# IRMVLab/EfficientLO-Net

Hardware: AMD Instinct MI355X
Metric: frame-pairs/sec (KITTI 64x1800 range image) (higher is better)
Workload: dtype f32 (1x1 convolutions as 3 fp16-MFMA products of hi/lo-split fp32 operands, fp32 accumulate)

## Files before the change

### efficientlo-net_amd/_lib.py

```python
import ctypes
import os

import torch

_PKG = os.path.dirname(os.path.abspath(__file__))
LIB_PATH = os.environ.get("ELO_LIB_PATH") or os.path.join(
    _PKG, "libelo_hip_f32.so" if os.environ.get("ELO_DENSE_F32", "0") == "1" else "libelo_hip.so")

_vp = ctypes.c_void_p


class GroupArgs(ctypes.Structure):
    _fields_ = [("batch", ctypes.c_int), ("H", ctypes.c_int), ("W", ctypes.c_int),
                ("H2", ctypes.c_int), ("W2", ctypes.c_int), ("npoints", ctypes.c_int),
                ("kernel_h", ctypes.c_int), ("kernel_w", ctypes.c_int), ("K", ctypes.c_int),
                ("flag_copy", ctypes.c_int), ("distance", ctypes.c_float),
                ("stride_h", ctypes.c_int), ("stride_w", ctypes.c_int),
                ("xyz1", _vp), ("xyz2", _vp), ("idx_n2", _vp), ("random_hw", _vp),
                ("selected_bhw_idx", _vp), ("valid_idx", _vp), ("valid_in_dis_idx", _vp),
                ("selected_mask", _vp)]


def _struct(name, fields):
    return type(name, (ctypes.Structure,), {"_fields_": fields, "__doc__": "struct %s (include/elo.h)." % name})


_i, _f = ctypes.c_int, ctypes.c_float
GroupConcatArgs = _struct("elo_group_concat_args", [
    ("batch", _i), ("npoints", _i), ("K", _i), ("H2", _i), ("W2", _i), ("C", _i),
    ("centre_xyz", _vp), ("src_xyz", _vp), ("src_feat", _vp), ("idx", _vp), ("mask", _vp), ("out", _vp)])
MaskedMaxpoolArgs = _struct("elo_masked_maxpool_args", [
    ("batch", _i), ("npoints", _i), ("K", _i), ("C", _i), ("x", _vp), ("mask", _vp), ("out", _vp)])
CvEncode1Args = _struct("elo_cv_encode1_args", [
    ("batch", _i), ("npoints", _i), ("K", _i), ("H2", _i), ("W2", _i), ("C", _i),
    ("xyz1", _vp), ("feat1", _vp), ("xyz2", _vp), ("feat2", _vp), ("idx", _vp), ("mask", _vp), ("out", _vp),
    ("dtype", _i)])
CvEncode2Args = _struct("elo_cv_encode2_args", [
    ("batch", _i), ("npoints", _i), ("K", _i), ("H", _i), ("W", _i), ("C", _i), ("Cc", _i),
    ("xyz1", _vp), ("feat1", _vp), ("cost", _vp), ("idx", _vp), ("mask", _vp), ("xyz_cat", _vp), ("rest", _vp),
    ("dtype", _i)])
SoftmaxPoolArgs = _struct("elo_softmax_pool_args", [
    ("batch", _i), ("npoints", _i), ("K", _i), ("C", _i), ("logits", _vp), ("values", _vp),
    ("values_stride", _i), ("mask", _vp), ("out", _vp), ("dtype", _i)])
ELO_F32, ELO_F16 = 0, 1
SoftmaxValidArgs = _struct("elo_softmax_valid_args", [
    ("batch", _i), ("npoints", _i), ("C", _i), ("feature", _vp), ("weight", _vp), ("xyz", _vp), ("out", _vp),
    ("scratch", _vp), ("stats", _vp)])
SV_MAX_PARTS = 512
PermRefreshArgs = _struct("elo_perm_refresh_args", [
    ("pool", _vp), ("versions", _i), ("total", _i), ("cursor", _vp), ("flat", _vp), ("decoded", _vp), ("entry_of", _vp),
    ("table", _vp), ("n_entries", _i)])
PoseHeadArgs = _struct("elo_pose_head_args", [
    ("batch", _i), ("npoints", _i), ("C", _i), ("hidden", _i), ("feature", _vp), ("weight", _vp), ("xyz", _vp),
    ("W_big", _vp), ("b_big", _vp), ("W_q", _vp), ("b_q", _vp), ("W_t", _vp), ("b_t", _vp),
    ("q_coarse", _vp), ("t_coarse", _vp), ("q", _vp), ("t", _vp), ("q_norm", _vp), ("scratch", _vp), ("pose7", _vp),
    ("clear_scratch", _vp), ("clear_xyz", _vp), ("clear_feat", _vp), ("clear_cells", ctypes.c_long), ("clear_C", _i),
    ("feat_dtype", _i), ("pose7_slots", _i), ("pose7_cursor", _vp), ("next_orders", PermRefreshArgs), ("ready_parts", _i)])
WarpProjectArgs = _struct("elo_warp_project_args", [
    ("batch", _i), ("npoints", _i), ("C", _i), ("H", _i), ("W", _i),
    ("az_res", _f), ("vert_res", _f), ("vert_off", _f),
    ("xyz", _vp), ("feat", _vp), ("q", _vp), ("t", _vp), ("warped", _vp), ("out_xyz", _vp), ("out_feat", _vp),
    ("scratch", _vp), ("prepared", _i), ("feat_dtype", _i)])

InputStageArgs = _struct("elo_input_stage_args", [
    ("batch", _i), ("npoints", _i), ("point_stride", _i), ("H", _i), ("W", _i), ("az_res", _f), ("vert_res", _f),
    ("vert_off", _f), ("crop_xy", _f), ("cloud", _vp), ("T_trans", _vp), ("aug_frame", _vp), ("points", _vp),
    ("out_xyz", _vp), ("scratch", _vp)])

GroupConcatBwdArgs = _struct("elo_group_concat_bwd_args", [
    ("batch", _i), ("npoints", _i), ("K", _i), ("H2", _i), ("W2", _i), ("C", _i),
    ("grad_out", _vp), ("idx", _vp), ("mask", _vp), ("grad_centre", _vp), ("grad_src_xyz", _vp), ("grad_src_feat", _vp)])
MaskedMaxpoolBwdArgs = _struct("elo_masked_maxpool_bwd_args", [
    ("batch", _i), ("npoints", _i), ("K", _i), ("C", _i), ("x", _vp), ("mask", _vp), ("grad_out", _vp), ("grad_x", _vp)])
CvEncode1BwdArgs = _struct("elo_cv_encode1_bwd_args", [
    ("batch", _i), ("npoints", _i), ("K", _i), ("H2", _i), ("W2", _i), ("C", _i),
    ("xyz1", _vp), ("xyz2", _vp), ("idx", _vp), ("mask", _vp), ("grad_out", _vp),
    ("grad_xyz1", _vp), ("grad_feat1", _vp), ("grad_xyz2", _vp), ("grad_feat2", _vp)])
CvEncode2BwdArgs = _struct("elo_cv_encode2_bwd_args", [
    ("batch", _i), ("npoints", _i), ("K", _i), ("H", _i), ("W", _i), ("C", _i), ("Cc", _i),
    ("xyz1", _vp), ("idx", _vp), ("mask", _vp), ("grad_xyz_cat", _vp), ("grad_rest", _vp),
    ("grad_xyz1", _vp), ("grad_feat1", _vp), ("grad_cost", _vp)])
SoftmaxPoolBwdArgs = _struct("elo_softmax_pool_bwd_args", [
    ("batch", _i), ("npoints", _i), ("K", _i), ("C", _i), ("logits", _vp), ("values", _vp), ("values_stride", _i),
    ("mask", _vp), ("grad_out", _vp), ("grad_logits", _vp), ("grad_values", _vp)])
SoftmaxValidBwdArgs = _struct("elo_softmax_valid_bwd_args", [
    ("batch", _i), ("npoints", _i), ("C", _i), ("feature", _vp), ("weight", _vp), ("xyz", _vp), ("grad_out", _vp),
    ("grad_feature", _vp), ("grad_weight", _vp), ("out", _vp), ("stats", _vp)])
WarpProjectBwdArgs = _struct("elo_warp_project_bwd_args", [
    ("batch", _i), ("npoints", _i), ("C", _i), ("H", _i), ("W", _i), ("az_res", _f), ("vert_res", _f), ("vert_off", _f),
    ("xyz", _vp), ("q", _vp), ("t", _vp), ("scratch", _vp), ("grad_out_xyz", _vp), ("grad_out_feat", _vp),
    ("grad_warped", _vp), ("grad_xyz", _vp), ("grad_feat", _vp), ("grad_q", _vp), ("grad_t", _vp)])

BnStatsArgs = _struct("elo_bn_stats_args", [
    ("rows", ctypes.c_long), ("C", _i), ("z", _vp), ("scratch", _vp), ("eps", _f), ("momentum", _f), ("mean", _vp), ("invstd", _vp),
    ("running_mean", _vp), ("running_var", _vp), ("groups", _i)])
BnApplyArgs = _struct("elo_bn_apply_args", [
    ("rows", ctypes.c_long), ("C", _i), ("z", _vp), ("mean", _vp), ("invstd", _vp), ("gamma", _vp), ("beta", _vp), ("relu", _i),
    ("y", _vp), ("groups", _i)])
BnBackwardArgs = _struct("elo_bn_backward_args", [
    ("rows", ctypes.c_long), ("C", _i), ("dy", _vp), ("z", _vp), ("mean", _vp), ("invstd", _vp), ("gamma", _vp), ("beta", _vp),
    ("relu", _i), ("scratch", _vp), ("sums", _vp), ("dz", _vp), ("groups", _i)])
AdamFlatArgs = _struct("elo_adam_flat_args", [
    ("n", ctypes.c_long), ("param", _vp), ("grad", _vp), ("exp_avg", _vp), ("exp_avg_sq", _vp), ("hyper", _vp),
    ("beta1", _f), ("beta2", _f), ("one_minus_beta1", _f), ("one_minus_beta2", _f)])
PoseComposeArgs = _struct("elo_pose_compose_args", [
    ("batch", _i), ("q_raw", _vp), ("t_det", _vp), ("q_coarse", _vp), ("t_coarse", _vp), ("q", _vp), ("t", _vp), ("q_norm", _vp),
    ("grad_q", _vp), ("grad_t", _vp), ("grad_q_norm", _vp), ("grad_q_raw", _vp), ("grad_t_det", _vp), ("grad_q_coarse", _vp),
    ("grad_t_coarse", _vp)])
PoseLossArgs = _struct("elo_pose_loss_args", [
    ("batch", _i), ("q", _vp * 4), ("t", _vp * 4), ("q_gt", _vp), ("t_gt", _vp), ("w_x", _vp), ("w_q", _vp), ("loss", _vp),
    ("grad_out", _vp), ("grad_q", _vp * 4), ("grad_t", _vp * 4), ("grad_w_x", _vp), ("grad_w_q", _vp)])
WeightGradArgs = _struct("elo_weight_grad_args", [
    ("rows", ctypes.c_long), ("Cin", _i), ("Cout", _i), ("x", _vp), ("g", _vp), ("dW", _vp), ("db", _vp), ("scratch", _vp)])
DenseRowsArgs = _struct("elo_dense_rows_args", [
    ("rows", ctypes.c_long), ("Cin", _i), ("Cout", _i), ("x", _vp), ("W", _vp), ("transposed", _i), ("bias", _vp), ("out", _vp),
    ("scratch", _vp), ("eps", _f), ("momentum", _f), ("mean", _vp), ("invstd", _vp), ("running_mean", _vp), ("running_var", _vp),
    ("bn_z", _vp), ("bn_mean", _vp), ("bn_invstd", _vp), ("bn_gamma", _vp), ("bn_beta", _vp), ("bn_sums", _vp), ("bn_relu", _i), ("bn_dz", _vp), ("groups", _i)])
Dense = _struct("elo_dense", [("w_packed", _vp), ("bias", _vp), ("K", _i), ("N", _i), ("relu", _i), ("w_plain", _vp),
                              ("products", _i)])
_l = ctypes.c_long
GroupSpec = _struct("elo_group_spec", [
    ("random_hw", _vp), ("kernel_h", _i), ("kernel_w", _i), ("distance", _f), ("stride_h", _i), ("stride_w", _i),
    ("idx_out", _vp), ("mask_out", _vp), ("decoded_hw", _vp)])
SetconvArgs = _struct("elo_setconv_args", [
    ("batch", _i), ("npoints", _i), ("K", _i), ("H", _i), ("W", _i), ("H2", _i), ("W2", _i), ("C", _i),
    ("xyz1_grid", _vp), ("centre_hw", _vp), ("centre_xyz", _vp), ("src_xyz", _vp), ("src_feat", _vp),
    ("idx", _vp), ("mask", _vp), ("n_layers", _i), ("layers", Dense * 3), ("out", _vp), ("new_xyz", _vp), ("group", GroupSpec),
    ("feat_dtype", _i), ("range_counter", _vp)])
MlpArgs = _struct("elo_mlp_args", [
    ("rows", _l), ("n_sources", _i), ("src", _vp * 3), ("src_width", _i * 3), ("n_layers", _i),
    ("layers", Dense * 3), ("out", _vp),
    ("n_layers2", _i), ("layers2", Dense * 3), ("before", _vp), ("w_before", _i), ("after", _vp), ("w_after", _i),
    ("out2", _vp), ("feat_dtype", _i),
    ("clear_scratch", _vp), ("clear_xyz", _vp), ("clear_feat", _vp), ("clear_cells", _l), ("clear_C", _i), ("clear_images", _i),
    ("batch_hint", _i), ("sv_scratch", _vp), ("sv_xyz", _vp), ("sv_feature", _vp), ("sv_npoints", _i),
    ("range_counter", _vp)])
Cv1Args = _struct("elo_cv1_args", [
    ("batch", _i), ("npoints", _i), ("K", _i), ("H2", _i), ("W2", _i), ("C", _i),
    ("xyz1", _vp), ("feat1", _vp), ("xyz2", _vp), ("feat2", _vp), ("idx", _vp), ("mask", _vp),
    ("cv0", Dense), ("cv1", Dense), ("cv2", Dense), ("cv_xyz", Dense), ("sum_cv0", Dense), ("sum_cv1", Dense),
    ("out", _vp), ("group", GroupSpec), ("feat_dtype", _i), ("range_counter", _vp)])
Cv2Args = _struct("elo_cv2_args", [
    ("batch", _i), ("npoints", _i), ("K", _i), ("H", _i), ("W", _i), ("C", _i),
    ("xyz1", _vp), ("feat1", _vp), ("cost", _vp), ("idx", _vp), ("mask", _vp),
    ("xyz_enc", Dense), ("sum_cost0", Dense), ("sum_cost1", Dense), ("out", _vp), ("group", GroupSpec), ("feat_dtype", _i),
    ("range_counter", _vp)])
Tuning = _struct("elo_tuning", [
    ("chain_forms", _i), ("narrow_mfma", _i), ("range_check", _i), ("select_dense_waves", _i), ("random_dense_rows", _i),
    ("setconv_chain_rows", _l), ("mlp_chain_rows", _l), ("small_tile_units", _l), ("pool_wave", _i)])

SYMBOLS = [
    ("elo_abi_version", ctypes.c_int, []),
    ("elo_dense_f32", ctypes.c_int, []),
    ("elo_last_error", ctypes.c_char_p, []),
    ("elo_range_check", ctypes.c_int, [ctypes.c_int]),
    ("elo_range_violations", ctypes.c_int, [ctypes.POINTER(ctypes.c_ulonglong), _vp]),
    ("elo_get_tuning", ctypes.c_int, [ctypes.POINTER(Tuning)]),
    ("elo_set_tuning", ctypes.c_int, [ctypes.POINTER(Tuning)]),
    ("elo_fused_conv_random_k", ctypes.c_int, [ctypes.POINTER(GroupArgs), _vp]),
    ("elo_fused_conv_select_k", ctypes.c_int, [ctypes.POINTER(GroupArgs), _vp]),
    ("elo_fused_conv_random_k_dense", ctypes.c_int, [ctypes.POINTER(GroupArgs), _vp]),
    ("elo_fused_conv_select_k_dense", ctypes.c_int, [ctypes.POINTER(GroupArgs), _vp]),
    ("elo_debug_select_dense_waves", ctypes.c_int, [ctypes.c_int]),
    ("elo_perm_refresh", ctypes.c_int, [ctypes.POINTER(PermRefreshArgs), _vp]),
    ("elo_group_concat", ctypes.c_int, [ctypes.POINTER(GroupConcatArgs), _vp]),
    ("elo_masked_maxpool", ctypes.c_int, [ctypes.POINTER(MaskedMaxpoolArgs), _vp]),
    ("elo_cv_encode1", ctypes.c_int, [ctypes.POINTER(CvEncode1Args), _vp]),
    ("elo_cv_encode2", ctypes.c_int, [ctypes.POINTER(CvEncode2Args), _vp]),
    ("elo_masked_softmax_pool", ctypes.c_int, [ctypes.POINTER(SoftmaxPoolArgs), _vp]),
    ("elo_softmax_valid", ctypes.c_int, [ctypes.POINTER(SoftmaxValidArgs), _vp]),
    ("elo_pose_head", ctypes.c_int, [ctypes.POINTER(PoseHeadArgs), _vp]),
    ("elo_warp_project", ctypes.c_int, [ctypes.POINTER(WarpProjectArgs), _vp]),
    ("elo_input_stage", ctypes.c_int, [ctypes.POINTER(InputStageArgs), _vp]),
    ("elo_pose_head_warp", ctypes.c_int, [ctypes.POINTER(PoseHeadArgs), ctypes.POINTER(WarpProjectArgs), _vp]),
    ("elo_group_concat_backward", ctypes.c_int, [ctypes.POINTER(GroupConcatBwdArgs), _vp]),
    ("elo_masked_maxpool_backward", ctypes.c_int, [ctypes.POINTER(MaskedMaxpoolBwdArgs), _vp]),
    ("elo_cv_encode1_backward", ctypes.c_int, [ctypes.POINTER(CvEncode1BwdArgs), _vp]),
    ("elo_cv_encode2_backward", ctypes.c_int, [ctypes.POINTER(CvEncode2BwdArgs), _vp]),
    ("elo_masked_softmax_pool_backward", ctypes.c_int, [ctypes.POINTER(SoftmaxPoolBwdArgs), _vp]),
    ("elo_softmax_valid_backward", ctypes.c_int, [ctypes.POINTER(SoftmaxValidBwdArgs), _vp]),
    ("elo_warp_project_backward", ctypes.c_int, [ctypes.POINTER(WarpProjectBwdArgs), _vp]),
    ("elo_bn_stats", ctypes.c_int, [ctypes.POINTER(BnStatsArgs), _vp]),
    ("elo_bn_apply", ctypes.c_int, [ctypes.POINTER(BnApplyArgs), _vp]),
    ("elo_bn_backward", ctypes.c_int, [ctypes.POINTER(BnBackwardArgs), _vp]),
    ("elo_dense_weight_grad", ctypes.c_int, [ctypes.POINTER(WeightGradArgs), _vp]),
    ("elo_dense_rows", ctypes.c_int, [ctypes.POINTER(DenseRowsArgs), _vp]),
    ("elo_dense_rows_supported", ctypes.c_int, [ctypes.c_long, ctypes.c_int, ctypes.c_int]),
    ("elo_dense_rows_scratch_floats", ctypes.c_long, [ctypes.c_int, ctypes.c_int]),
    ("elo_bn_scratch_floats", ctypes.c_long, [ctypes.c_int, ctypes.c_int]),
    ("elo_adam_flat", ctypes.c_int, [ctypes.POINTER(AdamFlatArgs), _vp]),
    ("elo_pose_compose", ctypes.c_int, [ctypes.POINTER(PoseComposeArgs), _vp]),
    ("elo_pose_loss", ctypes.c_int, [ctypes.POINTER(PoseLossArgs), _vp]),
    ("elo_weight_grad_slices", ctypes.c_int, [ctypes.c_long, ctypes.c_int, ctypes.c_int]),
    ("elo_setconv_fused", ctypes.c_int, [ctypes.POINTER(SetconvArgs), _vp]),
    ("elo_mlp_fused", ctypes.c_int, [ctypes.POINTER(MlpArgs), _vp]),
    ("elo_setconv_fused2", ctypes.c_int, [ctypes.POINTER(SetconvArgs), ctypes.POINTER(SetconvArgs), _vp]),
    ("elo_mlp_fused2", ctypes.c_int, [ctypes.POINTER(MlpArgs), ctypes.POINTER(MlpArgs), _vp]),
    ("elo_mlp_sv_parts", ctypes.c_int, [ctypes.POINTER(MlpArgs), ctypes.POINTER(MlpArgs)]),
    ("elo_cv_stage1_fused", ctypes.c_int, [ctypes.POINTER(Cv1Args), _vp]),
    ("elo_debug_cv1_rr", ctypes.c_int, [ctypes.c_int]),
    ("elo_debug_rr_rows", ctypes.c_int, [ctypes.c_long, ctypes.c_long]),
    ("elo_debug_rr_launches", ctypes.c_int, [ctypes.POINTER(ctypes.c_ulonglong), ctypes.c_int]),
    ("elo_debug_narrow_mfma", ctypes.c_int, [ctypes.c_int]),
    ("elo_debug_narrow_launches", ctypes.c_int, [ctypes.POINTER(ctypes.c_ulonglong), ctypes.c_int]),
    ("elo_debug_sv_ride_launches", ctypes.c_int, [ctypes.POINTER(ctypes.c_ulonglong), ctypes.c_int]),
    ("elo_get_tuning_base", ctypes.c_int, [ctypes.POINTER(Tuning)]),
    ("elo_graph_submit", ctypes.c_int, [_vp, _vp, _vp, _vp, ctypes.c_ulong, _vp, _vp, ctypes.c_int]),
    ("elo_debug_chain_pair_launches", ctypes.c_int, [ctypes.POINTER(ctypes.c_ulonglong), ctypes.c_int]),
    ("elo_cv_stage1_setconv_chain_form", ctypes.c_int, [ctypes.POINTER(Cv1Args), ctypes.POINTER(SetconvArgs), ctypes.POINTER(SetconvArgs)]),
    ("elo_cv_stage1_setconv_chain", ctypes.c_int, [ctypes.POINTER(Cv1Args), ctypes.POINTER(SetconvArgs), ctypes.POINTER(SetconvArgs), _vp]),
    ("elo_cv_stage2_fused", ctypes.c_int, [ctypes.POINTER(Cv2Args), _vp]),
    ("elo_cv_stage1_setconv_fused", ctypes.c_int, [ctypes.POINTER(Cv1Args), ctypes.POINTER(SetconvArgs), ctypes.POINTER(SetconvArgs), _vp]),
]

_lib = None


class EloError(RuntimeError):
    pass


ABI_VERSION = 26


def lib():
    global _lib
    if _lib is None:
        if not os.path.exists(LIB_PATH):
            raise EloError("libelo_hip.so is not built (%s); run `python -c 'import __graft_entry__ as g; "
                           "g.build()'` -- there is no CPU fallback for the hot path" % LIB_PATH)
        handle = ctypes.CDLL(LIB_PATH)
        for name, restype, argtypes in SYMBOLS:
            fn = getattr(handle, name)
            fn.restype = restype
            fn.argtypes = argtypes
        if handle.elo_abi_version() != ABI_VERSION:
            raise EloError("%s has ABI version %d, this host expects %d: rebuild (python -c 'import __graft_entry__ as g; "
                           "g.build()')" % (LIB_PATH, handle.elo_abi_version(), ABI_VERSION))
        _lib = handle
        from . import tuning
        env = tuning.lib_from_env()
        if env:
            set_tuning(**env)
    return _lib


def get_tuning():
    t = Tuning()
    check(lib().elo_get_tuning(ctypes.byref(t)))
    return {name: int(getattr(t, name)) for name, _ in Tuning._fields_}


def get_tuning_base():
    t = Tuning()
    check(lib().elo_get_tuning_base(ctypes.byref(t)))
    return {name: int(getattr(t, name)) for name, _ in Tuning._fields_}


def set_tuning(**fields):
    t = Tuning()
    check(lib().elo_get_tuning_base(ctypes.byref(t)))
    for name, value in fields.items():
        if not hasattr(t, name):
            raise KeyError("elo_tuning has no field %r" % name)
        setattr(t, name, int(value))
    check(lib().elo_set_tuning(ctypes.byref(t)))
    from . import tuning
    tuning.bump()


def check(rc):
    if rc != 0:
        raise EloError("libelo_hip: %s (status %d)" % (lib().elo_last_error().decode(), rc))


_range_counter = None


def set_range_counter(ptr):
    global _range_counter
    prev, _range_counter = _range_counter, ptr
    return prev


def _stamp(*structs):
    if _range_counter is not None:
        for a in structs:
            if a is not None and hasattr(a, "range_counter"):
                a.range_counter = _range_counter


def call(entry, args, like):
    _stamp(args)
    with torch.cuda.device(like.device):
        check(getattr(lib(), entry)(ctypes.byref(args), stream_ptr(like)))


def call3(entry, a, b, c, like):
    _stamp(a, b, c)
    with torch.cuda.device(like.device):
        check(getattr(lib(), entry)(ctypes.byref(a), ctypes.byref(b), ctypes.byref(c) if c is not None else None, stream_ptr(like)))


def call2(entry, args_a, args_b, like):
    _stamp(args_a, args_b)
    with torch.cuda.device(like.device):
        check(getattr(lib(), entry)(ctypes.byref(args_a), ctypes.byref(args_b), stream_ptr(like)))


def call2n(entry, args_a, args_b, like):
    _stamp(args_a, args_b)
    with torch.cuda.device(like.device):
        check(getattr(lib(), entry)(ctypes.byref(args_a), ctypes.byref(args_b) if args_b is not None else None, stream_ptr(like)))


def stream_ptr(t):
    return ctypes.c_void_p(torch.cuda.current_stream(t.device).cuda_stream)


def require_gpu(*tensors):
    for t in tensors:
        if t is not None and not t.is_cuda:
            raise EloError("the EfficientLO-Net hot path runs on an AMD GPU only (got a %s tensor); "
                           "there is no CPU fallback" % t.device)


def dtype_code(t):
    if t.dtype == torch.float32:
        return ELO_F32
    if t.dtype == torch.float16:
        return ELO_F16
    raise TypeError("feature tensors are float32 or float16 (got %s)" % t.dtype)


def range_check(enable):
    return lib().elo_range_check(1 if enable else 0)


def range_violations(like):
    n = ctypes.c_ulonglong(0)
    with torch.cuda.device(like.device):
        check(lib().elo_range_violations(ctypes.byref(n), stream_ptr(like)))
    return int(n.value)
```

### efficientlo-net_amd/csrc/elo_fused.hip

```cpp
#include "elo_group_device.h"
#include "elo_project_device.h"
#include <atomic>
#include <cstdlib>
#include <type_traits>

namespace elo {
namespace {

typedef float f32x4 __attribute__((ext_vector_type(4)));
typedef _Float16 half4 __attribute__((ext_vector_type(4)));
typedef _Float16 half2v __attribute__((ext_vector_type(2)));

constexpr int FUSED_BLOCK = 256;
constexpr int FUSED_WAVES = 4;
__device__ __forceinline__ int ftid() { return (int)(threadIdx.x & (FUSED_BLOCK - 1)); }

constexpr int MODE_SPLIT = 0;
constexpr int MODE_HALF = 1;
constexpr int MODE_CHECKED = 2;

__device__ unsigned long long g_range_violations;
__device__ unsigned long long g_range_snapshot;
__global__ void range_take_kernel() { g_range_snapshot = atomicExch(&g_range_violations, 0ull); }

// ... 1975 lines not shown
        }
    }
    stage_offsets(lds_off, a.group.random_hw, a.group.kernel_h, a.group.kernel_w, a.group.decoded_hw);
    RR_STAMP(1);
    {
        const float r2 = a.group.distance * a.group.distance;
        const int per_wave = 16 / K > 0 ? 16 / K : 1;
        auto uniform = [](float v) { return __int_as_float(__builtin_amdgcn_readfirstlane(__float_as_int(v))); };
        int pb[2], ph[2], pw[2];
        float pc[2][3];
        bool live[2];
        RawSlot first[2];
#pragma unroll
        for (int j = 0; j < 2; ++j) {
            const int pp = (wave * 16) / K + j;
            const long ptw = first_point + pp;
            live[j] = j < per_wave && pp < P && ptw < total_points;
            if (!live[j]) continue;
            pb[j] = (int)((unsigned)ptw / (unsigned)a.npoints);
            const int hwc = __builtin_amdgcn_readfirstlane(chw[pp]);
            ph[j] = div_stride(hwc >> 16, a.group.stride_h); pw[j] = div_stride(hwc & 0xffff, a.group.stride_w);
#pragma unroll
            for (int e = 0; e < 3; ++e) pc[j][e] = uniform(cxyz[pp * 3 + e]);
            first[j] = fetch_slot(grid_buffer(a.src_xyz + (size_t)pb[j] * a.H2 * a.W2 * 3), a.H2, a.W2, lds_off[lane < KT ? lane : 0], ph[j], pw[j],
                                  lane < KT);
        }
#pragma unroll
        for (int j = 0; j < 2; ++j) {
            if (!live[j]) continue;
            const int pp = (wave * 16) / K + j, b = pb[j];
            const float cx = pc[j][0], cy = pc[j][1], cz = pc[j][2];
            auto emit = [&](int slot, int hw) {
                cell_row[pp * K + slot] = (b * a.H2 + (hw >> 16)) * a.W2 + (hw & 0xffff);
                mask_row[pp * K + slot] = 1.0f;
            };
            int count = 0;
            if (!(pick_max(sq3(cx, cy, cz), ELO_EPS) <= ELO_EPS)) {
                const GridBuf gb = grid_buffer(a.src_xyz + (size_t)b * a.H2 * a.W2 * 3);
                count = wave_random_k_prefetched(gb, a.H2, a.W2, KT, K, lds_off, ph[j], pw[j], cx, cy, cz, r2, first[j], emit);
            }
            if (count + lane < K) { cell_row[pp * K + count + lane] = 0; mask_row[pp * K + count + lane] = 0.0f; }
        }
    }
    RR_STAMP(2);
    __syncthreads();
    RR_STAMP(3);
    const int r = wave * 16 + i16, pi = small_div(r, K);
    const int cell = cell_row[r];
    const bool used = cell >= 0;
    const float mk = mask_row[r];
    const float c0 = cxyz[(pi < P ? pi : 0) * 3 + 0], c1 = cxyz[(pi < P ? pi : 0) * 3 + 1], c2 = cxyz[(pi < P ? pi : 0) * 3 + 2];
    ActPair in0[FPB / 2];
    uint4 dxyz;
    const bool keep = used && mk != 0.0f;
    {
        typedef typename std::conditional<F16, uint2, float4>::type Item;
        Item f[FPB];
        const long cc = used ? cell : 0;
        const Item *rf = reinterpret_cast<const Item *>(a.src_feat) + (cc * C >> 2) + kq;
#pragma unroll
        for (int j = 0; j < FPB; ++j) f[j] = rf[j * 4];
        const float *g = a.src_xyz + cc * 3;
        const float x = g[0], y = g[1], z = g[2];
        ws.prime();
        auto quad = [&](const Item &v) {
            const uint4 zq{0u, 0u, 0u, 0u};
            if constexpr (F16) return keep ? quad_of_halves(v) : zq;
            else return keep ? pack_quad<MODE>(v, bad) : zq;
        };
#pragma unroll
        for (int j = 0; j < FPB; ++j) put_quad(in0[j / 2], j % 2, quad(f[j]));
        const float4 d = kq == 0 ? float4{x * mk - c0, y * mk - c1, z * mk - c2, 0.0f} : float4{0.0f, 0.0f, 0.0f, 0.0f};
        dxyz = used ? pack_quad<MODE>(d, bad) : uint4{0u, 0u, 0u, 0u};
    }
    rr_bias_store(lds, tid, N1 + N2 + N3, bias_word);
    RR_STAMP(4);
    rr_barrier();
    RR_STAMP(5);
    const uint4 none{0u, 0u, 0u, 0u};
    ActPair h1[N1 / 32];
    auto emit0 = [&](int pass, int t, const f32x4 acc) { put_quad(h1[pass], t, pack_quad<MODE>(relu4(acc, a.layers[0].relu), bad)); };
    rr_layer<FPB / 2, true, N1 / 16, 0, MODE, (F16 ? ~0u : 0u)>(in0, dxyz, bt, bt + B1, bias, fetch, advance, emit0);
    RR_STAMP(6);
    float4 last[NOUT / 16];
    if constexpr (N3 == 0) {
        rr_layer<N1 / 32, false, N2 / 16, E0, MODE>(h1, none, bt + B1, nullptr, bias, fetch, advance, [&](int pass, int t, const f32x4 acc) {
            last[2 * pass + t] = relu4(acc, a.layers[1].relu);
        });
    } else {
        ActPair h2[N2 / 32];
        rr_layer<N1 / 32, false, N2 / 16, E0, MODE>(h1, none, bt + B1, bt + B2, bias, fetch, advance, [&](int pass, int t, const f32x4 acc) {
            put_quad(h2[pass], t, pack_quad<MODE>(relu4(acc, a.layers[1].relu), bad));
        });
        rr_layer<N2 / 32, false, NOUT / 16, E1, MODE>(h2, none, bt + B2, nullptr, bias, fetch, advance, [&](int pass, int t, const f32x4 acc) {
            last[2 * pass + t] = relu4(acc, a.layers[2].relu);
        });
    }
    RR_STAMP(7);
    if ((K == 8 || K == 16) && a.layers[N3 ? 2 : 1].relu) rr_pool_max_inwave<NOUT, F16>(last, mk, r, lane, K, first_point, total_points, a.out);
    else rr_pool_max<NOUT, F16>(lds, last, mk, r, wave, lane, K, P, first_point, total_points, a.out);
    RR_STAMP(8);
    report_violations<MODE>(bad, a.range_counter);
}

template <int FPB, int N1, int N2, int N3, bool F16, int MODE = MODE_SPLIT>
__global__ __launch_bounds__(RR_WAVES * 64, 4) void setconv_rr_kernel(const JobPair<elo_setconv_args> jobs)
{
    setconv_rr_body<FPB, N1, N2, N3, F16, MODE>(jobs.job[blockIdx.y], blockIdx.x, gridDim.x);
}

template <int C, bool F16, int MODE>
__global__ __launch_bounds__(RR_WAVES * 64, 4) void cv1_setconv_rr_kernel(const elo_cv1_args a, const JobPair<elo_setconv_args> jobs,
                                                                         const unsigned n_cv, const unsigned n_sc)
{
    if (blockIdx.x < n_cv) {
        cv1_rr_body<C, F16, MODE>(a, blockIdx.x, n_cv);
    } else {
        const unsigned r = blockIdx.x - n_cv, j = r >= n_sc ? 1u : 0u;
        setconv_rr_body<4, 128, 64, 0, F16, MODE>(jobs.job[j], j ? r - n_sc : r, n_sc);
    }
}
template <int CIN, int N1, int N2, int N3, int MODE>
__global__ __launch_bounds__(ELO_BLOCK, 2) void setconv_narrow_kernel(const elo_setconv_args a)
{
    constexpr int G = 32, PER_BLOCK = ELO_BLOCK / G, C = CIN - 3, CB3 = N3 / 16;
    static_assert((C == 16 || C == 3) && N1 <= 16 && N2 <= 16 && (N3 == 16 || N3 == 32), "the pyramid's two narrow set-conv layers");
    __shared__ int slot_hw[PER_BLOCK][G];
    const int tid = threadIdx.x;
    const int l64 = tid & 63, i16 = l64 & 15, kq = l64 >> 4;
    unsigned bad = 0, wbad = 0;
    auto wq = [&](const elo_dense &L, const int LK, const int LN, int k0, int n) {
        const int nc = n < LN ? n : LN - 1;
        float v[4];
#pragma unroll
        for (int e = 0; e < 4; ++e) {
            const int k = k0 + e < LK ? k0 + e : LK - 1;
            v[e] = L.w_plain[k * LN + nc];
        }
#pragma unroll
        for (int e = 0; e < 4; ++e) v[e] = (k0 + e < LK && n < LN) ? v[e] : 0.0f;
        return float4{v[0], v[1], v[2], v[3]};
    };
    auto bq = [&](const elo_dense &L, const int LN, int n0) {
        float v[4];
#pragma unroll
        for (int e = 0; e < 4; ++e) v[e] = L.bias[n0 + e < LN ? n0 + e : LN - 1];
#pragma unroll
        for (int e = 0; e < 4; ++e) v[e] = n0 + e < LN ? v[e] : 0.0f;
        return float4{v[0], v[1], v[2], v[3]};
    };
    const float4 w1a = wq(a.layers[0], CIN, N1, 4 * kq, i16), w1b = C == 16 ? wq(a.layers[0], CIN, N1, 16 + 4 * kq, i16) : float4{0.0f, 0.0f, 0.0f, 0.0f};
    const float4 w2f = wq(a.layers[1], N1, N2, 4 * kq, i16);
    float4 w3f[CB3];
#pragma unroll
    for (int cb = 0; cb < CB3; ++cb) w3f[cb] = wq(a.layers[2], N2, N3, 4 * kq, cb * 16 + i16);
    const float4 b1 = bq(a.layers[0], N1, 4 * kq), b2 = bq(a.layers[1], N2, 4 * kq);
    float4 b3[CB3];
#pragma unroll
    for (int cb = 0; cb < CB3; ++cb) b3[cb] = bq(a.layers[2], N3, cb * 16 + 4 * kq);

    const int g = tid / G, lane = tid % G, shift = (tid & 63) / G * G;
    const elo_group_spec &gs = a.group;
    const int KT = gs.kernel_h * gs.kernel_w, kW = gs.kernel_w, hh = gs.kernel_h / 2, hw2 = gs.kernel_w / 2;
    int off[SMALL_STEPS];
    const int *order = gs.decoded_hw ? gs.decoded_hw : gs.random_hw;
#pragma unroll
    for (int st = 0; st < SMALL_STEPS; ++st) off[st] = order[st * G + lane < KT ? st * G + lane : 0];
    const long total = (long)a.batch * a.npoints;
    const long first = (long)xcd_tile(blockIdx.x, gridDim.x) * PER_BLOCK;
    const long pt = first + g;
    const bool live = pt < total;
    const long ptc = live ? pt : total - 1;
    int b, n, hc, wc;
    split_point(ptc, a.npoints, b, n);
    if (a.centre_hw) {
        const int2 c2 = reinterpret_cast<const int2 *>(a.centre_hw)[ptc];
        hc = c2.x; wc = c2.y;
    } else { hc = n / a.W; wc = n - hc * a.W; }
    if (!gs.decoded_hw) {
#pragma unroll
        for (int st = 0; st < SMALL_STEPS; ++st) off[st] = ((off[st] / kW - hh) << 16) | ((off[st] % kW - hw2) & 0xffff);
    }
    const float *cp = a.xyz1_grid + (((long)b * a.H + hc) * a.W + wc) * 3;
    const float cx = cp[0], cy = cp[1], cz = cp[2];
    const float *grid2 = a.src_xyz + (size_t)b * a.H2 * a.W2 * 3;
    const int base_h = div_stride(hc, gs.stride_h), base_w = div_stride(wc, gs.stride_w);
    RawSlot raw[SMALL_STEPS];
#pragma unroll
    for (int st = 0; st < SMALL_STEPS; ++st) raw[st] = fetch_slot(grid2, a.H2, a.W2, off[st], base_h, base_w, st * G + lane < KT);
    if (live && lane < 3 && a.new_xyz) a.new_xyz[pt * 3 + lane] = lane == 0 ? cx : lane == 1 ? cy : cz;
    const float r2 = gs.distance * gs.distance;
    slot_hw[g][lane] = -1;
    int taken = 0;
    const bool centre_ok = !(pick_max(sq3(cx, cy, cz), ELO_EPS) <= ELO_EPS);
#pragma unroll
    for (int st = 0; st < SMALL_STEPS; ++st) {
        if (st > 0 && (st * G >= KT || __builtin_amdgcn_ballot_w64(taken < G) == 0)) break;
        const Probe pr = judge(raw[st], cx, cy, cz, r2);
        const bool hit = pr.hit && centre_ok && taken < G;
        const unsigned long long mh = group_ballot<G>(hit, shift);
        const int slot = taken + __popcll(mh & ((1ull << lane) - 1ull));
        if (hit && slot < G) slot_hw[g][slot] = pr.hw;
        taken += __popcll(mh);
    }
    __builtin_amdgcn_fence(__ATOMIC_ACQ_REL, "wavefront");
    __builtin_amdgcn_wave_barrier();
    if (gs.idx_out || gs.mask_out) {
        const int hw = slot_hw[g][lane];
        if (live && gs.idx_out) {
            int *o = gs.idx_out + (pt * G + lane) * 3;
            o[0] = hw >= 0 ? b : 0; o[1] = hw >= 0 ? hw >> 16 : 0; o[2] = hw >= 0 ? hw & 0xffff : 0;
        }
        if (live && gs.mask_out) gs.mask_out[pt * G + lane] = hw >= 0 ? 1.0f : 0.0f;
    }

    const int wv = tid >> 6, f16 = a.feat_dtype == ELO_F16;
    auto uni = [](float v, int src) { return __int_as_float(__builtin_amdgcn_readlane(__float_as_int(v), src)); };
    float mrow[4], sx[4][3];
    uint4 ff[4];
#pragma unroll
    for (int rb = 0; rb < 4; ++rb) {
        const int hw = slot_hw[wv * 2 + (rb >> 1)][(rb & 1) * 16 + i16];
        const int bb = __builtin_amdgcn_readlane(b, (rb >> 1) * 32);
        mrow[rb] = hw >= 0 ? 1.0f : 0.0f;
        const long cell = hw >= 0 ? ((long)bb * a.H2 + (hw >> 16)) * a.W2 + (hw & 0xffff) : 0;
        const float *sp = a.src_xyz + cell * 3;
        sx[rb][0] = sp[0]; sx[rb][1] = sp[1]; sx[rb][2] = sp[2];
        if constexpr (C == 16) {
            if (f16) {
                const uint2 h = reinterpret_cast<const uint2 *>(a.src_feat)[cell * 4 + kq];
                ff[rb] = uint4{h.x, h.y, 0u, 0u};
            } else ff[rb] = reinterpret_cast<const uint4 *>(a.src_feat)[cell * 4 + kq];
        } else {
            float v[3];
#pragma unroll
            for (int c = 0; c < 3; ++c) v[c] = feat_load(a.src_feat, cell * 3 + c, f16);
            ff[rb] = uint4{__float_as_uint(v[0]), __float_as_uint(v[1]), __float_as_uint(v[2]), 0u};
        }
    }
    const uint4 q1a = pack_quad<MODE_SPLIT>(w1a, wbad), q1b = pack_quad<MODE_SPLIT>(w1b, wbad), w2t = pack_quad<MODE_SPLIT>(w2f, wbad);
    const WPair w1p{uint4{q1a.x, q1a.y, q1b.x, q1b.y}, uint4{q1a.z, q1a.w, q1b.z, q1b.w}};
    uint4 w3t[CB3];
#pragma unroll
    for (int cb = 0; cb < CB3; ++cb) w3t[cb] = pack_quad<MODE_SPLIT>(w3f[cb], wbad);
    float4 best[CB3];
#pragma unroll
    for (int rb = 0; rb < 4; ++rb) {
        const float m = mrow[rb];
        const float ccx = uni(cx, (rb >> 1) * 32), ccy = uni(cy, (rb >> 1) * 32), ccz = uni(cz, (rb >> 1) * 32);
        const float dx = sx[rb][0] * m - ccx, dy = sx[rb][1] * m - ccy, dz = sx[rb][2] * m - ccz;
        f32x4 acc1[1][1] = {{f32x4{b1.x, b1.y, b1.z, b1.w}}};
        if constexpr (C == 16) {
            uint4 fq;
            const float4 fv = __builtin_bit_cast(float4, ff[rb]);
            if (f16) fq = m != 0.0f ? quad_of_halves(uint2{ff[rb].x, ff[rb].y}) : uint4{0u, 0u, 0u, 0u};
            else fq = pack_quad<MODE>(float4{fv.x * m, fv.y * m, fv.z * m, fv.w * m}, bad);
            const uint4 gq = pack_quad<MODE>(kq == 0 ? float4{dx, dy, dz, 0.0f} : float4{0.0f, 0.0f, 0.0f, 0.0f}, bad);
            const ActPair in[1] = {ActPair{uint4{fq.x, fq.y, gq.x, gq.y}, uint4{fq.z, fq.w, gq.z, gq.w}}};
            const WPair w[1] = {w1p};
            mma_pair<MODE, 1, 1, 1>(acc1, 0, in, w);
        } else {
            const float4 fv = __builtin_bit_cast(float4, ff[rb]);
            const float4 v = kq == 0 ? float4{fv.x * m, fv.y * m, fv.z * m, dx} : kq == 1 ? float4{dy, dz, 0.0f, 0.0f}
                                                                                            : float4{0.0f, 0.0f, 0.0f, 0.0f};
            const uint4 in[1] = {pack_quad<MODE>(v, bad)}, w[1] = {q1a};
            mma_tail<MODE, 1, 1, 1, false>(acc1, 0, in, w);
        }
        f32x4 acc2[1][1] = {{f32x4{b2.x, b2.y, b2.z, b2.w}}};
        {
            const uint4 in[1] = {pack_quad<MODE>(relu4(acc1[0][0], a.layers[0].relu), bad)}, w[1] = {w2t};
            mma_tail<MODE, 1, 1, 1, false>(acc2, 0, in, w);
        }
        const uint4 h2[1] = {pack_quad<MODE>(relu4(acc2[0][0], a.layers[1].relu), bad)};
#pragma unroll
        for (int cb = 0; cb < CB3; ++cb) {
            f32x4 acc3[1][1] = {{f32x4{b3[cb].x, b3[cb].y, b3[cb].z, b3[cb].w}}};
            const uint4 w[1] = {w3t[cb]};
            mma_tail<MODE, 1, 1, 1, false>(acc3, 0, h2, w);
            const float4 y = relu4(acc3[0][0], a.layers[2].relu);
            const float q[4] = {y.x * m, y.y * m, y.z * m, y.w * m};
            float o[4];
#pragma unroll
            for (int e = 0; e < 4; ++e) {
                int v = __float_as_int(q[e]);
                v = dpp_imax_all<0xb1>(v);
                v = dpp_imax_all<0x4e>(v);
                v = dpp_imax_all<0x141>(v);
                v = dpp_imax_all<0x140>(v);
                o[e] = __int_as_float(v);
            }
            if (rb & 1) {
                const long ptg = first + wv * 2 + (rb >> 1);
                const float4 r4{fmaxf(best[cb].x, o[0]), fmaxf(best[cb].y, o[1]), fmaxf(best[cb].z, o[2]), fmaxf(best[cb].w, o[3])};
                if (i16 == 0 && ptg < total) feat_store4(a.out, ptg * N3 + cb * 16 + 4 * kq, r4, f16);
            } else best[cb] = float4{o[0], o[1], o[2], o[3]};
        }
    }
    report_violations<MODE>(bad, a.range_counter);
}

#endif

template <int TILE, int MODE>
__global__ __launch_bounds__(FUSED_BLOCK, TILE == 32 ? ELO_TILE32_WAVES : ELO_TILE_WAVES) void cv2_kernel(const elo_cv2_args a, const int S)
{
    extern __shared__ __align__(16) float lds[];
    float *act = lds;
    const TileMeta meta = tile_meta(lds, TILE, S);
    const int tid = threadIdx.x;
    const int K = a.K, P = TILE / K, C = a.C, f16 = a.feat_dtype == ELO_F16;
    unsigned bad = 0;
    const long total_points = (long)a.batch * a.npoints;
    const long first_point = (long)xcd_tile(blockIdx.x, gridDim.x) * P;
    if (first_point >= total_points) return;
    if (a.group.random_hw) {
        int *lds_off = reinterpret_cast<int *>(meta.cxyz + 128);
        group_tile<TILE, false>(meta, lds_off, nullptr, a.group, first_point, total_points, a.npoints, P, K, a.xyz1, a.H,
                                a.W, nullptr, a.xyz1, a.H, a.W, nullptr);
    } else {
        load_meta<TILE>(meta, first_point, total_points, P, K, a.idx, a.mask, a.H, a.W);
        __syncthreads();
    }
    const int Cp = ceil16(C), XYZ = 192;
    {
        auto cell_of = [&](int row) { return (long)meta.cell[row]; };
        auto centre_of = [&](int row) { return meta.cell[row] >= 0 ? first_point + small_div(row, K) : -1L; };
        uint4 rc[SEG_ITEMS], rf[SEG_ITEMS];
        seg_load<TILE>(rc, a.cost, 64, f16, cell_of);
        seg_load<TILE>(rf, a.feat1, C, f16, centre_of);
        GeoRow gr;
        const bool grow = tid < TILE;
        const int gcell = grow ? meta.cell[tid] : -1;
        if (grow) gr = geo_load(a.xyz1 + (gcell >= 0 ? first_point + small_div(tid, K) : 0) * 3, a.xyz1 + (long)(gcell >= 0 ? gcell : 0) * 3);
        seg_store<TILE, MODE>(act, S, 0, 64, f16, rc, cell_of, [&](int row) { return meta.mask[row] != 0.0f; }, bad);
        seg_store<TILE, MODE>(act, S, 128, C, f16, rf, centre_of, [](int) { return true; }, bad);
        zero_cols<TILE, MODE>(act, S, 128 + C, 128 + Cp);
        if (grow) geo_store<MODE>(act, tid * S + XYZ, gr, meta.mask[tid], gcell >= 0, bad);
    }
    Pre<Sub<TILE, 128>::TPW> p128;
    Pre<Sub<TILE, 64>::TPW> p64;
    prefetch<TILE, Sub<TILE, 64>::TPW, MODE>(a.xyz_enc, p64);
    __syncthreads();
    dense_pf<TILE, 64, 128, MODE>(act, S, XYZ, to_tile(64), a.xyz_enc, p64, &a.sum_cost0, &p128, bad);
    dense_pf<TILE, 128, 64, MODE>(act, S, 0, to_tile(64), a.sum_cost0, p128, &a.sum_cost1, &p64, bad);
    dense_pf<TILE, 64, 0, MODE>(act, S, 64, to_pool(64), a.sum_cost1, p64, nullptr, nullptr, bad);
    pool_masked_softmax(act, S, 64, 0, meta, P, K, first_point, total_points, a.out, f16);
    report_violations<MODE>(bad, a.range_counter);
}

inline long small_tile_threshold() { return tuning().small_tile_units; }
inline bool small_tile(long units_at_32, int K) { return K <= 16 && units_at_32 < small_tile_threshold(); }

int check_dense(const elo_dense &L, int K, int N, const char *who, const char *name)
{
    if (!L.w_packed || !L.bias) return fail(ELO_ERR_ARG, "%s: layer %s has null weights", who, name);
    if (L.K != K || (N > 0 && L.N != N))
        return fail(ELO_ERR_ARG, "%s: layer %s is %dx%d, expected %dx%d", who, name, L.K, L.N, K, N);
    if (L.N <= 0 || L.N > 128) return fail(ELO_ERR_LIMIT, "%s: layer %s width %d outside 1..128", who, name, L.N);
    if (L.products != ELO_PRODUCTS_SPLIT && L.products != ELO_PRODUCTS_HALF)
        return fail(ELO_ERR_ARG, "%s: layer %s: products must be ELO_PRODUCTS_SPLIT or ELO_PRODUCTS_HALF", who, name);
#ifdef ELO_DENSE_F32
    if (L.products != ELO_PRODUCTS_SPLIT) return fail(ELO_ERR_ARG, "%s: this library was built with -DELO_DENSE_F32 (fp32 MFMA only)", who);
#endif
    return ELO_OK;
}

int check_dtype(int feat_dtype, const char *who)
{
    if (feat_dtype != ELO_F32 && feat_dtype != ELO_F16) return fail(ELO_ERR_ARG, "%s: feat_dtype must be ELO_F32 or ELO_F16", who);
    return ELO_OK;
}

int &range_check_flag() { return tuning().range_check; }

template <typename... Rest>
int products_mode(const char *who, int *mode, const elo_dense &first, const Rest &...rest)
{
    const int m = first.products;
    for (const elo_dense *L : {&rest...})
        if (L->products != m) return fail(ELO_ERR_ARG, "%s: the layers of one launch must share one products mode", who);
    *mode = m == ELO_PRODUCTS_HALF ? MODE_HALF : range_check_flag() ? MODE_CHECKED : MODE_SPLIT;
    return ELO_OK;
}

int products_mode(const char *who, int *mode, const elo_dense *layers, int n, const elo_dense *layers2 = nullptr, int n2 = 0)
{
    const int m = layers[0].products;
    for (int l = 0; l < n; ++l)
        if (layers[l].products != m) return fail(ELO_ERR_ARG, "%s: the layers of one launch must share one products mode", who);
    for (int l = 0; l < n2; ++l)
        if (layers2[l].products != m) return fail(ELO_ERR_ARG, "%s: the layers of one launch must share one products mode", who);
    *mode = m == ELO_PRODUCTS_HALF ? MODE_HALF : range_check_flag() ? MODE_CHECKED : MODE_SPLIT;
    return ELO_OK;
}

size_t tile_lds_bytes(int rows, int S, int KT = 0, bool select = false, int K = 0)
{
    return sizeof(float) * ((size_t)rows * S + 64 + 96 + 32 + ((KT + 3) & ~3) + (select ? (size_t)FUSED_WAVES * select_scratch_words(KT, K) : 0));
}

int check_group(const elo_group_spec &g, int H2, int W2, size_t lds_bytes, const char *who)
{
    if (!g.random_hw) return ELO_OK;
    if (g.kernel_h <= 0 || g.kernel_w <= 0 || !(g.distance > 0.0f) || g.stride_h <= 0 || g.stride_w <= 0)
        return fail(ELO_ERR_ARG, "%s: bad grouping attributes", who);
    if (g.kernel_w / 2 > W2)
        return fail(ELO_ERR_LIMIT, "%s: kernel_size_W/2 = %d exceeds the queried width %d (single wrap)", who, g.kernel_w / 2, W2);
    if (H2 >= 32768 || W2 >= 65536) return fail(ELO_ERR_LIMIT, "%s: queried grid larger than 32767 x 65535", who);
    if ((long)H2 * W2 * 12 >= 0x7fffffffL) return fail(ELO_ERR_LIMIT, "%s: queried grid beyond 2 GB per batch element (buffer addressing)", who);
    if (lds_bytes > 64 * 1024)
        return fail(ELO_ERR_LIMIT, "%s: window %dx%d needs %zu bytes of LDS for in-kernel grouping", who, g.kernel_h, g.kernel_w, lds_bytes);
    return ELO_OK;
}

#define ELO_REQUIRE(cond, who, what) \
    do { if (!(cond)) return fail(ELO_ERR_ARG, "%s: %s", who, what); } while (0)

}
}

using namespace elo;

static inline int pad16(int x) { return (x + 15) & ~15; }

#ifdef ELO_DENSE_F32
#define ELO_PICK(KERNEL, tile16, mode, CALL)                                                              \
    do {                                                                                                  \
        if ((mode) == MODE_CHECKED) { if (tile16) CALL((KERNEL<16, MODE_CHECKED>)); else CALL((KERNEL<32, MODE_CHECKED>)); } \
        else { if (tile16) CALL((KERNEL<16, MODE_SPLIT>)); else CALL((KERNEL<32, MODE_SPLIT>)); }         \
    } while (0)
#else
#define ELO_PICK(KERNEL, tile16, mode, CALL)                                                              \
    do {                                                                                                  \
        if ((mode) == MODE_HALF) { if (tile16) CALL((KERNEL<16, MODE_HALF>)); else CALL((KERNEL<32, MODE_HALF>)); } \
        else if ((mode) == MODE_CHECKED) { if (tile16) CALL((KERNEL<16, MODE_CHECKED>)); else CALL((KERNEL<32, MODE_CHECKED>)); } \
        else { if (tile16) CALL((KERNEL<16, MODE_SPLIT>)); else CALL((KERNEL<32, MODE_SPLIT>)); }         \
    } while (0)
#endif

#ifdef ELO_DENSE_F32
#define ELO_PICK_MODE(M_, CALL_T) do { if ((M_) == MODE_CHECKED) CALL_T(MODE_CHECKED); else CALL_T(MODE_SPLIT); } while (0)
#else
#define ELO_PICK_MODE(M_, CALL_T) do { if ((M_) == MODE_HALF) CALL_T(MODE_HALF); else if ((M_) == MODE_CHECKED) CALL_T(MODE_CHECKED); else CALL_T(MODE_SPLIT); } while (0)
#endif

static int chain_cols(const elo_dense *layers, int n_layers, int width)
{
    int cols = pad16(width);
    for (int l = 0; l < n_layers; ++l) cols = cols > pad16(layers[l].N) ? cols : pad16(layers[l].N);
    return cols;
}

static int check_setconv(const elo_setconv_args *a, const char *who)
{
    ELO_REQUIRE(a, who, "null argument block");
    ELO_REQUIRE(a->batch >= 0 && a->npoints > 0 && a->K > 0 && a->H2 > 0 && a->W2 > 0 && a->C >= 0, who, "bad sizes");
    if (a->K > 32) return fail(ELO_ERR_LIMIT, "%s: K = %d exceeds the 32-row tile", who, a->K);
    ELO_REQUIRE(a->n_layers >= 1 && a->n_layers <= ELO_MAX_CHAIN, who, "1..3 layers");
    ELO_REQUIRE(a->src_xyz && (a->src_feat || a->C == 0) && a->out, who, "null tensor pointer");
    ELO_REQUIRE(a->group.random_hw || (a->idx && a->mask), who, "neither idx/mask nor a grouping spec");
    ELO_REQUIRE((a->xyz1_grid && a->H > 0 && a->W > 0 && (a->centre_hw || a->group.random_hw)) || a->centre_xyz, who, "no centre source");
    ELO_REQUIRE(!a->group.random_hw || (a->xyz1_grid && a->H > 0 && a->W > 0), who, "in-kernel grouping needs xyz1_grid");
    if (a->group.random_hw && a->group.stride_h > 0 && a->group.stride_w > 0 &&
        ((a->H - 1) / a->group.stride_h >= a->H2 || (a->W - 1) / a->group.stride_w >= a->W2))
        return fail(ELO_ERR_ARG, "%s: the queried grid %dx%d is smaller than the centres' grid %dx%d over the strides %dx%d", who, a->H2, a->W2,
                    a->H, a->W, a->group.stride_h, a->group.stride_w);
    if (int rc = check_dtype(a->feat_dtype, who)) return rc;
    int width = 3 + a->C;
    for (int l = 0; l < a->n_layers; ++l) {
        if (int rc = check_dense(a->layers[l], width, 0, who, "mlp")) return rc;
        width = a->layers[l].N;
    }
    return ELO_OK;
}

struct TilePlan { int S; bool t16; long units; size_t lds; int mode; };

static bool same_shape(const elo_setconv_args *a, const elo_setconv_args *b)
{
    if (a->batch != b->batch || a->npoints != b->npoints || a->K != b->K || a->C != b->C || a->n_layers != b->n_layers ||
        a->H2 != b->H2 || a->W2 != b->W2 || a->group.kernel_h != b->group.kernel_h || a->group.kernel_w != b->group.kernel_w ||
        (a->group.random_hw == nullptr) != (b->group.random_hw == nullptr) || a->feat_dtype != b->feat_dtype)
        return false;
    for (int l = 0; l < a->n_layers; ++l)
        if (a->layers[l].K != b->layers[l].K || a->layers[l].N != b->layers[l].N) return false;
    return true;
}

static int plan_setconv(const elo_setconv_args *a, const elo_setconv_args *b, TilePlan *p, const char *who)
{
    const long points = (long)a->batch * a->npoints;
    if (points >= 0x7fffffffL) return fail(ELO_ERR_LIMIT, "%s: batch * npoints beyond 2^31", who);
    p->S = row_stride(chain_cols(a->layers, a->n_layers, 3 + a->C));
    const int P32 = 32 / a->K, P16 = a->K <= 16 ? 16 / a->K : 1;
    const long u32 = (points + P32 - 1) / P32, u16 = (points + P16 - 1) / P16;
    int mode_b = 0;
    if (int rc = products_mode(who, &p->mode, a->layers, a->n_layers)) return rc;
    if (b) {
        if (int rc = products_mode(who, &mode_b, b->layers, b->n_layers)) return rc;
        if (p->mode != mode_b) return fail(ELO_ERR_ARG, "%s: the two jobs of a paired launch must share one products mode", who);
    }
    p->t16 = small_tile(u32 * (b ? 2 : 1), a->K);
    p->units = p->t16 ? u16 : u32;
    const int KT = a->group.random_hw ? a->group.kernel_h * a->group.kernel_w : 0;
    p->lds = tile_lds_bytes(p->t16 ? 16 : 32, p->S, KT, false);
    return check_group(a->group, a->H2, a->W2, p->lds, who);
}

extern "C" int elo_dense_f32(void)
{
#ifdef ELO_DENSE_F32
    return 1;
#else
    return 0;
#endif
}

#ifdef ELO_CV1_CLOCK
extern "C" int elo_debug_cv1_clock(unsigned long long *out16)
{
    return hipMemcpyFromSymbol(out16, HIP_SYMBOL(g_cv1_clock), 24 * sizeof(unsigned long long)) == hipSuccess ? 0 : -3;
}
#endif

extern "C" int elo_range_check(int enable)
{
    const int prev = range_check_flag();
    if (enable >= 0) range_check_flag() = enable ? 1 : 0;
    return prev;
}

extern "C" int elo_range_violations(unsigned long long *count, elo_stream_t stream)
{
    const char *who = "elo_range_violations";
    ELO_REQUIRE(count, who, "null count");
    hipStream_t s = (hipStream_t)stream;
    hipLaunchKernelGGL(range_take_kernel, dim3(1), dim3(1), 0, s);
    if (hipMemcpyFromSymbolAsync(count, HIP_SYMBOL(g_range_snapshot), sizeof(*count), 0, hipMemcpyDeviceToHost, s) != hipSuccess ||
        hipStreamSynchronize(s) != hipSuccess)
        return fail(ELO_ERR_LAUNCH, "%s: %s", who, hipGetErrorString(hipGetLastError()));
    return ELO_OK;
}

extern "C" int elo_debug_cv1_rr(int on)
{
    const int prev = tuning().chain_forms;
    tuning().chain_forms = on >= 0 ? (on != 0) : tuning_base().chain_forms;
    return prev;
}
static bool cv1_rr_on() { return tuning().chain_forms != 0; }
extern "C" int elo_debug_rr_rows(long setconv_rows, long mlp_rows)
{
    tuning().setconv_chain_rows = setconv_rows >= 0 ? setconv_rows : tuning_base().setconv_chain_rows;
    tuning().mlp_chain_rows = mlp_rows >= 0 ? mlp_rows : tuning_base().mlp_chain_rows;
    return ELO_OK;
}
static long setconv_rr_rows(int batch)
{
    const long t = tuning().setconv_chain_rows;
    (void)batch;
    return t >= 0 ? t : 20000L;
}
static long mlp_rr_rows(int batch_hint)
{
    const long t = tuning().mlp_chain_rows;
    return t >= 0 ? t : batch_hint >= ELO_THROUGHPUT_BATCH ? 2048L : 8192L;
}
extern "C" int elo_debug_narrow_mfma(int on)
{
    const int prev = tuning().narrow_mfma;
    tuning().narrow_mfma = on >= 0 ? (on ? 1 : 0) : tuning_base().narrow_mfma;
    return prev;
}
static bool narrow_mfma_on() { return tuning().narrow_mfma != 0; }
static std::atomic<unsigned long long> g_rr_launches[4];
extern "C" int elo_debug_rr_launches(unsigned long long *counts4, int reset)
{
    for (int i = 0; i < 4; ++i) {
        if (counts4) counts4[i] = g_rr_launches[i].load();
        if (reset) g_rr_launches[i].store(0);
    }
    return ELO_OK;
}
static std::atomic<unsigned long long> g_chain_pair_launches;
extern "C" int elo_debug_chain_pair_launches(unsigned long long *count, int reset)
{
    if (count) *count = g_chain_pair_launches.load();
    if (reset) g_chain_pair_launches.store(0);
    return ELO_OK;
}
static std::atomic<unsigned long long> g_sv_ride_launches;
extern "C" int elo_debug_sv_ride_launches(unsigned long long *count, int reset)
{
    if (count) *count = g_sv_ride_launches.load();
    if (reset) g_sv_ride_launches.store(0);
    return ELO_OK;
}
static std::atomic<unsigned long long> g_narrow_launches[2];
extern "C" int elo_debug_narrow_launches(unsigned long long *counts2, int reset)
{
    for (int i = 0; i < 2; ++i) {
        if (counts2) counts2[i] = g_narrow_launches[i].load();
        if (reset) g_narrow_launches[i].store(0);
    }
    return ELO_OK;
}

static int setconv_chain_shape(const elo_setconv_args *a, const elo_setconv_args *b, int mode)
{
#ifdef ELO_DENSE_F32
    return 0;
#else
    const long points = (long)a->batch * a->npoints;
    const int nl = a->n_layers, n1 = a->layers[0].N, n2 = nl >= 2 ? a->layers[1].N : 0, n3 = nl == 3 ? a->layers[2].N : 0;
    const int shape = (nl == 2 && n1 == 128 && n2 == 64) ? 1 : (nl == 3 && n1 == 64 && n2 == 64 && n3 == 128) ? 2
                    : (nl == 3 && n1 == 128 && n2 == 64 && n3 == 64) ? 3 : 0;
    const int KT = a->group.kernel_h * a->group.kernel_w;
    const bool narrow = !b && a->K == 32 && nl == 3 && a->layers[0].w_plain && a->layers[1].w_plain && a->layers[2].w_plain;
    if (!shape || narrow || !a->group.random_hw || !(mode == MODE_SPLIT || mode == MODE_HALF) || !cv1_rr_on() || a->C != 64 ||
        !(a->K == 8 || a->K == 16 || a->K == 32) || KT > 512 || a->group.idx_out || a->group.mask_out ||
        points * a->K * (b ? 2 : 1) < setconv_rr_rows(a->batch))
        return 0;
    return shape;
#endif
}

static bool cv_chain(int C, int mode)
{
#ifdef ELO_DENSE_F32
    return false;
#else
    return (mode == MODE_SPLIT || mode == MODE_HALF) && cv1_rr_on() && (C == 16 || C == 32 || C == 64);
#endif
}

extern "C" int elo_setconv_fused2(const elo_setconv_args *a, const elo_setconv_args *b, elo_stream_t stream)
{
    const char *who = "elo_setconv_fused";
    if (int rc = check_setconv(a, who)) return rc;
    if (b) {
        if (int rc = check_setconv(b, who)) return rc;
        if (!same_shape(a, b)) return fail(ELO_ERR_ARG, "%s: the two jobs of a paired launch must have the same shape", who);
    }
    const long points = (long)a->batch * a->npoints;
    if (points >= 0x7fffffffL) return fail(ELO_ERR_LIMIT, "%s: batch * npoints beyond 2^31", who);
    if (points == 0) return ELO_OK;
    hipStream_t s = (hipStream_t)stream;
    if (!b && a->group.random_hw && a->K == 32 && a->n_layers == 3 && a->layers[0].w_plain && a->layers[1].w_plain &&
        a->layers[2].w_plain && a->layers[2].relu && a->group.kernel_h * a->group.kernel_w <= SMALL_STEPS * 32) {
        const int cin = 3 + a->C, n1 = a->layers[0].N, n2 = a->layers[1].N, n3 = a->layers[2].N;
        const unsigned grid = (unsigned)((points + 7) / 8);
        if (int rc = check_group(a->group, a->H2, a->W2, 0, who)) return rc;
#ifndef ELO_DENSE_F32
        if (narrow_mfma_on()) {
            const bool checked = range_check_flag();
            if (cin == 19 && n1 == 16 && n2 == 16 && n3 == 32) {
                if (checked) hipLaunchKernelGGL((setconv_narrow_kernel<19, 16, 16, 32, MODE_CHECKED>), dim3(grid), dim3(ELO_BLOCK), 0, s, *a);
                else hipLaunchKernelGGL((setconv_narrow_kernel<19, 16, 16, 32, MODE_SPLIT>), dim3(grid), dim3(ELO_BLOCK), 0, s, *a);
                ++g_narrow_launches[0];
                return check_launch(who);
            }
        }
#endif
        if (cin == 6 && n1 == 8 && n2 == 8 && n3 == 16) {
            hipLaunchKernelGGL((setconv_small_kernel<6, 8, 8, 16>), dim3(grid), dim3(ELO_BLOCK), 0, s, *a);
            ++g_narrow_launches[1];
            return check_launch(who);
        }
        if (cin == 19 && n1 == 16 && n2 == 16 && n3 == 32) {
            hipLaunchKernelGGL((setconv_small_kernel<19, 16, 16, 32>), dim3(grid), dim3(ELO_BLOCK), 0, s, *a);
            ++g_narrow_launches[1];
            return check_launch(who);
        }
    }
    TilePlan plan;
    if (int rc = plan_setconv(a, b, &plan, who)) return rc;
    JobPair<elo_setconv_args> pair;
    pair.job[0] = *a;
    pair.job[1] = b ? *b : *a;
#ifndef ELO_DENSE_F32
    if (const int shape = setconv_chain_shape(a, b, plan.mode)) {
        const int P = RR_ROWS / a->K;
        const dim3 rgrid((unsigned)((points + P - 1) / P), b ? 2u : 1u);
        const bool f16 = a->feat_dtype == ELO_F16;
#define RRS(N1_, N2_, N3_)                                                                                                              \
        do {                                                                                                                        \
            if (f16 && plan.mode == MODE_HALF) hipLaunchKernelGGL((setconv_rr_kernel<4, N1_, N2_, N3_, true, MODE_HALF>), rgrid, dim3(RR_WAVES * 64), RR_LDS_BYTES, s, pair);  \
            else if (f16) hipLaunchKernelGGL((setconv_rr_kernel<4, N1_, N2_, N3_, true, MODE_SPLIT>), rgrid, dim3(RR_WAVES * 64), RR_LDS_BYTES, s, pair);  \
            else if (plan.mode == MODE_HALF) hipLaunchKernelGGL((setconv_rr_kernel<4, N1_, N2_, N3_, false, MODE_HALF>), rgrid, dim3(RR_WAVES * 64), RR_LDS_BYTES, s, pair);     \
            else hipLaunchKernelGGL((setconv_rr_kernel<4, N1_, N2_, N3_, false, MODE_SPLIT>), rgrid, dim3(RR_WAVES * 64), RR_LDS_BYTES, s, pair);     \
        } while (0)
        if (shape == 1) RRS(128, 64, 0);
        else if (shape == 2) RRS(64, 64, 128);
        else RRS(128, 64, 64);
#undef RRS
        ++g_rr_launches[2];
        return check_launch(who);
    }
#endif
    const dim3 grid((unsigned)plan.units, b ? 2u : 1u);
    const size_t lds = plan.lds;
    const int S = plan.S;
#define CALL(k) hipLaunchKernelGGL(k, grid, dim3(FUSED_BLOCK), lds, s, pair, S)
    ELO_PICK(setconv_kernel, plan.t16, plan.mode, CALL);
#undef CALL
    return check_launch(who);
}

extern "C" int elo_setconv_fused(const elo_setconv_args *a, elo_stream_t stream)
{
    return elo_setconv_fused2(a, nullptr, stream);
}

static int check_mlp(const elo_mlp_args *a, const char *who, int *in_width)
{
    ELO_REQUIRE(a, who, "null argument block");
    ELO_REQUIRE(a->rows >= 0 && a->n_sources >= 1 && a->n_sources <= 3, who, "bad sizes");
    ELO_REQUIRE(a->n_layers >= 1 && a->n_layers <= ELO_MAX_CHAIN && a->out, who, "1..3 layers and an output");
    if (int rc = check_dtype(a->feat_dtype, who)) return rc;
    int width = 0;
    for (int s = 0; s < a->n_sources; ++s) {
        ELO_REQUIRE(a->src[s] && a->src_width[s] > 0, who, "null / empty source");
        width += a->src_width[s];
    }
    *in_width = width;
    for (int l = 0; l < a->n_layers; ++l) {
        if (int rc = check_dense(a->layers[l], width, 0, who, "mlp")) return rc;
        width = a->layers[l].N;
    }
    ELO_REQUIRE(!a->clear_scratch || (a->clear_xyz && a->clear_cells > 0 && a->clear_images > 0 && a->clear_C >= 0 &&
                                      (a->clear_feat || a->clear_C == 0) && (a->feat_dtype != ELO_F16 || a->clear_C % 2 == 0)),
                who, "incomplete clear_* side job");
    ELO_REQUIRE(!a->clear_scratch || a->clear_cells * (a->clear_C > 3 ? a->clear_C : 3) < (1l << 31), who, "clear_* side job: more than 2^31 words");
    ELO_REQUIRE(a->n_layers2 >= 0 && a->n_layers2 <= ELO_MAX_CHAIN, who, "0..3 second-stage layers");
    if (a->n_layers2 > 0) {
        ELO_REQUIRE(a->out2 && a->w_before >= 0 && a->w_after >= 0 && (a->before || a->w_before == 0) &&
                    (a->after || a->w_after == 0), who, "incomplete second stage");
        ELO_REQUIRE(width % 4 == 0, who, "a second stage needs a first-stage output width that is a multiple of 4");
        width += a->w_before + a->w_after;
        for (int l = 0; l < a->n_layers2; ++l) {
            if (int rc = check_dense(a->layers2[l], width, 0, who, "mlp stage 2")) return rc;
            width = a->layers2[l].N;
        }
    }
    return ELO_OK;
}

static int mlp_cols(const elo_mlp_args *a, int in_width)
{
    int cols = chain_cols(a->layers, a->n_layers, in_width);
    if (a->n_layers2 > 0) {
        const int n1 = a->layers[a->n_layers - 1].N, in2 = a->w_before + n1 + a->w_after;
        const int c2 = chain_cols(a->layers2, a->n_layers2, in2);
        cols = cols > c2 ? cols : c2;
    }
    return cols;
}

struct MlpPlan { int S, mode, C; bool t16, chain; int sv_tiles; };

static int plan_mlp(const elo_mlp_args *a, const elo_mlp_args *b, MlpPlan *p, const char *who)
{
    int in_width = 0, in_width_b = 0;
    if (int rc = check_mlp(a, who, &in_width)) return rc;
    if (b) {
        if (int rc = check_mlp(b, who, &in_width_b)) return rc;
        bool same = a->rows == b->rows && in_width == in_width_b && a->n_layers == b->n_layers &&
                    a->n_layers2 == b->n_layers2 && a->w_before == b->w_before && a->w_after == b->w_after &&
                    a->feat_dtype == b->feat_dtype;
        for (int l = 0; same && l < a->n_layers; ++l) same = a->layers[l].N == b->layers[l].N;
        for (int l = 0; same && l < a->n_layers2; ++l) same = a->layers2[l].N == b->layers2[l].N;
        if (!same) return fail(ELO_ERR_ARG, "%s: the two jobs of a paired launch must have the same shape", who);
    }
    if (b && b->clear_scratch) return fail(ELO_ERR_ARG, "%s: the clear_* side job belongs to the first job of a pair", who);
    if (b && (b->sv_scratch || b->sv_feature)) return fail(ELO_ERR_ARG, "%s: the sv_* fields belong to the first job of a pair", who);
    p->S = row_stride(mlp_cols(a, in_width));
    const long u32 = (a->rows + 31) / 32;
    p->mode = 0;
    int mode_b = 0;
    if (int rc = products_mode(who, &p->mode, a->layers, a->n_layers, a->layers2, a->n_layers2)) return rc;
    if (b) {
        if (int rc = products_mode(who, &mode_b, b->layers, b->n_layers, b->layers2, b->n_layers2)) return rc;
        if (p->mode != mode_b) return fail(ELO_ERR_ARG, "%s: the two jobs of a paired launch must share one products mode", who);
    }
    p->t16 = small_tile(u32 * (b ? 2 : 1), 1);
    p->chain = false;
    p->C = a->n_sources == 2 ? a->src_width[1] : 0;
#ifndef ELO_DENSE_F32
    {
        const long min_rows = mlp_rr_rows(a->batch_hint);
        const int C = p->C;
        const bool aligned = ((uintptr_t)a->src[0] | (uintptr_t)a->src[1] | (uintptr_t)a->before | (uintptr_t)a->after | (uintptr_t)a->out |
                              (uintptr_t)a->out2) % 16 == 0 &&
                             (!b || ((uintptr_t)b->src[0] | (uintptr_t)b->src[1] | (uintptr_t)b->before | (uintptr_t)b->after | (uintptr_t)b->out |
                                     (uintptr_t)b->out2) % 16 == 0);
        p->chain = (p->mode == MODE_SPLIT || p->mode == MODE_HALF) && cv1_rr_on() && a->n_sources == 2 && a->src_width[0] == 64 &&
                   (C == 16 || C == 32 || C == 64) && a->n_layers == 2 && a->layers[0].N == 128 && a->layers[1].N == 64 && a->n_layers2 == 2 &&
                   a->layers2[0].N == 128 && a->layers2[1].N == 64 && a->w_before == C && a->w_after == 64 && aligned &&
                   a->rows * (b ? 2 : 1) >= min_rows;
    }
#endif
    p->sv_tiles = 0;
    const int final_n = a->n_layers2 > 0 ? a->layers2[a->n_layers2 - 1].N : a->layers[a->n_layers - 1].N;
    if (!p->chain && final_n == 64 && a->sv_npoints > 0 && a->rows > 0 && a->rows % a->sv_npoints == 0) {
        const bool t16 = small_tile((a->rows / a->sv_npoints) * (((long)a->sv_npoints + 31) / 32), 1);
        const int tile = t16 ? 16 : 32, groups = b ? 2 : 1;
        const long tiles = ((long)a->sv_npoints + tile - 1) / tile;
        const size_t lds = sizeof(float) * ((size_t)groups * tile * p->S + (b ? 0 : (size_t)tile * 64));
        if (tiles <= ELO_SV_MAX_PARTS && lds <= 64 * 1024) {
            p->sv_tiles = (int)tiles;
            p->t16 = t16;
        }
    }
    return ELO_OK;
}

extern "C" int elo_mlp_sv_parts(const elo_mlp_args *a, const elo_mlp_args *b)
{
    MlpPlan p;
    if (plan_mlp(a, b, &p, "elo_mlp_sv_parts")) return 0;
    return p.sv_tiles;
}

extern "C" int elo_mlp_fused2(const elo_mlp_args *a, const elo_mlp_args *b, elo_stream_t stream)
{
    const char *who = "elo_mlp_fused";
    MlpPlan plan;
    if (int rc = plan_mlp(a, b, &plan, who)) return rc;
    if (a->rows == 0)
        return a->clear_scratch || a->sv_scratch ? fail(ELO_ERR_ARG, "%s: a clear_* / sv_* side job needs rows to ride on", who) : ELO_OK;
    const int S = plan.S, mode = plan.mode;
    const bool t16 = plan.t16;
    const long u32 = (a->rows + 31) / 32, u16 = (a->rows + 15) / 16;
    JobPair<elo_mlp_args> pair;
    pair.job[0] = *a;
    pair.job[1] = b ? *b : *a;
    if (a->sv_scratch) {
        if (!plan.sv_tiles)
            return fail(ELO_ERR_ARG, "%s: sv_scratch is set but this launch cannot compute softmax_valid's partial sums "
                                     "(elo_mlp_sv_parts returns 0: chain-kernel regime, final width != 64, rows %% sv_npoints != 0 or too many tiles)", who);
        if (!a->sv_xyz) return fail(ELO_ERR_ARG, "%s: sv_scratch without sv_xyz", who);
        if ((b != nullptr) == (a->sv_feature != nullptr))
            return fail(ELO_ERR_ARG, "%s: a paired launch takes its features from job b (sv_feature NULL), a single launch from sv_feature", who);
        if (!b && ((uintptr_t)a->sv_feature & 15)) return fail(ELO_ERR_ARG, "%s: unaligned sv_feature", who);
        const int tile = t16 ? 16 : 32, groups = b ? 2 : 1;
        const size_t lds = sizeof(float) * ((size_t)groups * tile * S + (b ? 0 : (size_t)tile * 64));
        const dim3 grid((unsigned)(a->rows / a->sv_npoints) * (unsigned)plan.sv_tiles);
        hipStream_t s = (hipStream_t)stream;
#define CALL_SV(T_, M_)                                                                                                         \
        do {                                                                                                                    \
            if (b) hipLaunchKernelGGL((mlp_sv_kernel<T_, M_, true>), grid, dim3(2 * FUSED_BLOCK), lds, s, pair, S, plan.sv_tiles); \
            else hipLaunchKernelGGL((mlp_sv_kernel<T_, M_, false>), grid, dim3(FUSED_BLOCK), lds, s, pair, S, plan.sv_tiles);     \
        } while (0)
#define CALL_SV_T(M_) do { if (t16) CALL_SV(16, M_); else CALL_SV(32, M_); } while (0)
        ELO_PICK_MODE(mode, CALL_SV_T);
#undef CALL_SV_T
#undef CALL_SV
        ++g_sv_ride_launches;
        return check_launch(who);
    }
    const size_t lds = tile_lds_bytes(t16 ? 16 : 32, S);
#ifndef ELO_DENSE_F32
    if (plan.chain) {
        const int C = plan.C;
        const dim3 rgrid((unsigned)((a->rows + RR_ROWS - 1) / RR_ROWS), b ? 2u : 1u);
        const bool f16 = a->feat_dtype == ELO_F16;
        hipStream_t rs = (hipStream_t)stream;
#define RRM(C_)                                                                                                                      \
        do {                                                                                                                    \
            if (f16 && mode == MODE_HALF) hipLaunchKernelGGL((mlp2_rr_kernel<C_, true, MODE_HALF>), rgrid, dim3(RR_WAVES * 64), RR_LDS_BYTES, rs, pair);             \
            else if (f16) hipLaunchKernelGGL((mlp2_rr_kernel<C_, true, MODE_SPLIT>), rgrid, dim3(RR_WAVES * 64), RR_LDS_BYTES, rs, pair);             \
            else if (mode == MODE_HALF) hipLaunchKernelGGL((mlp2_rr_kernel<C_, false, MODE_HALF>), rgrid, dim3(RR_WAVES * 64), RR_LDS_BYTES, rs, pair);                \
            else hipLaunchKernelGGL((mlp2_rr_kernel<C_, false, MODE_SPLIT>), rgrid, dim3(RR_WAVES * 64), RR_LDS_BYTES, rs, pair);                \
        } while (0)
        if (C == 16) RRM(16);
        else if (C == 32) RRM(32);
        else RRM(64);
#undef RRM
        ++g_rr_launches[3];
        return check_launch(who);
    }
#endif
    const dim3 grid((unsigned)(t16 ? u16 : u32), b ? 2u : 1u);
    hipStream_t s = (hipStream_t)stream;
#define CALL(k) hipLaunchKernelGGL(k, grid, dim3(FUSED_BLOCK), lds, s, pair, S)
    ELO_PICK(mlp_kernel, t16, mode, CALL);
#undef CALL
    return check_launch(who);
}

extern "C" int elo_mlp_fused(const elo_mlp_args *a, elo_stream_t stream) { return elo_mlp_fused2(a, nullptr, stream); }

static int check_cv_features(const char *who, int C, int f16, std::initializer_list<const void *> tensors)
{
    const int per = f16 ? 8 : 4;
    if (C % per != 0) return fail(ELO_ERR_LIMIT, "%s: C = %d must be a multiple of %d (%s feature storage)", who, C, per, f16 ? "fp16" : "fp32");
    if (32 * (C / per) > SEG_ITEMS * FUSED_BLOCK) return fail(ELO_ERR_LIMIT, "%s: C = %d too wide for the tile gather", who, C);
    for (const void *p : tensors)
        if ((uintptr_t)p & 15) return fail(ELO_ERR_ARG, "%s: feature tensors must be 16-byte aligned", who);
    return ELO_OK;
}

static int plan_cv1(const elo_cv1_args *a, TilePlan *p, const char *who)
{
    ELO_REQUIRE(a, who, "null argument block");
    ELO_REQUIRE(a->batch >= 0 && a->npoints > 0 && a->K > 0 && a->H2 > 0 && a->W2 > 0 && a->C > 0, who, "bad sizes");
    if (a->K > 32) return fail(ELO_ERR_LIMIT, "%s: K = %d exceeds the 32-row tile", who, a->K);
    ELO_REQUIRE(a->xyz1 && a->feat1 && a->xyz2 && a->feat2 && a->out, who, "null tensor pointer");
    ELO_REQUIRE(a->group.random_hw || (a->idx && a->mask), who, "neither idx/mask nor a grouping spec");
    ELO_REQUIRE(!a->group.random_hw || a->npoints == a->H2 * a->W2, who, "in-kernel grouping needs npoints == H2*W2");
    if (int rc = check_dtype(a->feat_dtype, who)) return rc;
    if (int rc = check_cv_features(who, a->C, a->feat_dtype == ELO_F16, {a->feat1, a->feat2})) return rc;
    const int CT = 10 + 2 * a->C;
    if (int rc = check_dense(a->cv0, CT, 128, who, "CV_0")) return rc;
    if (int rc = check_dense(a->cv1, 128, 64, who, "CV_1")) return rc;
    if (int rc = check_dense(a->cv2, 64, 64, who, "CV_2")) return rc;
    if (int rc = check_dense(a->cv_xyz, 10, 64, who, "CV_xyz")) return rc;
    if (int rc = check_dense(a->sum_cv0, 128, 128, who, "sum_CV_0")) return rc;
    if (int rc = check_dense(a->sum_cv1, 128, 64, who, "sum_CV_1")) return rc;
    const long points = (long)a->batch * a->npoints;
    if (points >= 0x7fffffffL) return fail(ELO_ERR_LIMIT, "%s: batch * npoints beyond 2^31", who);
    const int cols = 128 + cv1_feat_cols(a->C);
    p->S = row_stride(cols > 192 ? cols : 192);
    const int P32 = 32 / a->K, P16 = a->K <= 16 ? 16 / a->K : 1;
    const long u32 = (points + P32 - 1) / P32, u16 = (points + P16 - 1) / P16;
    if (int rc = products_mode(who, &p->mode, a->cv0, a->cv1, a->cv2, a->cv_xyz, a->sum_cv0, a->sum_cv1)) return rc;
    p->t16 = small_tile(u32, a->K);
    p->units = p->t16 ? u16 : u32;
    const int KT = a->group.random_hw ? a->group.kernel_h * a->group.kernel_w : 0;
    p->lds = tile_lds_bytes(p->t16 ? 16 : 32, p->S);
    if (sizeof(float) * (((size_t)KT + 3) / 4 * 4 + (size_t)FUSED_WAVES * select_scratch_words(KT, a->K)) > sizeof(float) * (p->t16 ? 16 : 32) * p->S)
        return fail(ELO_ERR_LIMIT, "%s: window %dx%d does not fit the tile for in-kernel grouping", who, a->group.kernel_h, a->group.kernel_w);
    return check_group(a->group, a->H2, a->W2, p->lds, who);
}

extern "C" int elo_cv_stage1_fused(const elo_cv1_args *a, elo_stream_t stream)
{
    const char *who = "elo_cv_stage1_fused";
    TilePlan plan;
    if (int rc = plan_cv1(a, &plan, who)) return rc;
    if ((long)a->batch * a->npoints == 0) return ELO_OK;
#ifndef ELO_DENSE_F32
    if (!a->group.random_hw && cv_chain(a->C, plan.mode)) {
        const int P = RR_ROWS / a->K;
        const dim3 grid((unsigned)(((long)a->batch * a->npoints + P - 1) / P));
        const size_t lds = RR_LDS_BYTES;
        hipStream_t s = (hipStream_t)stream;
        const bool f16 = a->feat_dtype == ELO_F16;
        static_assert(RR_LDS_BYTES <= 64 * 1024, "dynamic LDS within the default limit");
#define RR(CC)                                                                                                      \
        do {                                                                                                        \
            if (f16 && plan.mode == MODE_HALF) hipLaunchKernelGGL((cv1_rr_kernel<CC, true, MODE_HALF>), grid, dim3(RR_WAVES * 64), lds, s, *a);          \
            else if (f16) hipLaunchKernelGGL((cv1_rr_kernel<CC, true, MODE_SPLIT>), grid, dim3(RR_WAVES * 64), lds, s, *a);          \
            else if (plan.mode == MODE_HALF) hipLaunchKernelGGL((cv1_rr_kernel<CC, false, MODE_HALF>), grid, dim3(RR_WAVES * 64), lds, s, *a);             \
            else hipLaunchKernelGGL((cv1_rr_kernel<CC, false, MODE_SPLIT>), grid, dim3(RR_WAVES * 64), lds, s, *a);             \
        } while (0)
        if (a->C == 16) RR(16);
        else if (a->C == 32) RR(32);
        else RR(64);
#undef RR
        ++g_rr_launches[0];
        return check_launch(who);
    }
#endif
    const dim3 grid((unsigned)plan.units);
    const size_t lds = plan.lds;
    const int S = plan.S;
    hipStream_t s = (hipStream_t)stream;
#define CALL(k) hipLaunchKernelGGL(k, grid, dim3(FUSED_BLOCK), lds, s, *a, S)
    if (a->group.random_hw) ELO_PICK(cv1_kernel, plan.t16, plan.mode, CALL);
    else ELO_PICK(cv1_meta_kernel, plan.t16, plan.mode, CALL);
#undef CALL
    return check_launch(who);
}


extern "C" int elo_cv_stage1_setconv_fused(const elo_cv1_args *a, const elo_setconv_args *ja, const elo_setconv_args *jb,
                                           elo_stream_t stream)
{
    const char *who = "elo_cv_stage1_setconv_fused";
    TilePlan pc, ps;
    if (int rc = plan_cv1(a, &pc, who)) return rc;
    if (int rc = check_setconv(ja, who)) return rc;
    if (jb) {
        if (int rc = check_setconv(jb, who)) return rc;
        if (!same_shape(ja, jb)) return fail(ELO_ERR_ARG, "%s: the two set-conv jobs must have the same shape", who);
    }
    if (int rc = plan_setconv(ja, jb, &ps, who)) return rc;
    if (ps.mode != pc.mode) return fail(ELO_ERR_ARG, "%s: the cost volume and the set-conv jobs must share one products mode", who);
    if ((long)a->batch * a->npoints == 0 || (long)ja->batch * ja->npoints == 0)
        return fail(ELO_ERR_ARG, "%s: empty batch (call the separate entry points)", who);
    SideJobs side;
    side.job[0] = *ja;
    side.job[1] = jb ? *jb : *ja;
    side.njobs = jb ? 2 : 1;
    side.S = ps.S;
    side.blocks_per_job = (int)ps.units;
    const unsigned n_cv = (unsigned)pc.units;
    const dim3 grid(n_cv + (unsigned)(ps.units * side.njobs));
    const size_t lds = pc.lds > ps.lds ? pc.lds : ps.lds;
    const int S = pc.S;
    hipStream_t s = (hipStream_t)stream;
#define CALL_T(M) do {                                                                                                  \
        if (pc.t16 && ps.t16) hipLaunchKernelGGL((cv1_setconv_kernel<16, 16, M>), grid, dim3(FUSED_BLOCK), lds, s, *a, S, n_cv, side);      \
        else if (pc.t16) hipLaunchKernelGGL((cv1_setconv_kernel<16, 32, M>), grid, dim3(FUSED_BLOCK), lds, s, *a, S, n_cv, side);           \
        else if (ps.t16) hipLaunchKernelGGL((cv1_setconv_kernel<32, 16, M>), grid, dim3(FUSED_BLOCK), lds, s, *a, S, n_cv, side);           \
        else hipLaunchKernelGGL((cv1_setconv_kernel<32, 32, M>), grid, dim3(FUSED_BLOCK), lds, s, *a, S, n_cv, side);                        \
    } while (0)
    ELO_PICK_MODE(pc.mode, CALL_T);
#undef CALL_T
    return check_launch(who);
}

static int chain_pair_form(const elo_cv1_args *a, const elo_setconv_args *ja, const elo_setconv_args *jb, int *mode_out, const char *who)
{
#ifdef ELO_DENSE_F32
    (void)a; (void)ja; (void)jb; (void)mode_out; (void)who;
    return 0;
#else
    if (!a || !ja || !jb) return 0;
    int mode = 0, mode_sc = 0, mode_sb = 0;
    if (products_mode(who, &mode, a->cv0, a->cv1, a->cv2, a->cv_xyz, a->sum_cv0, a->sum_cv1)) return 0;
    if (ja->n_layers != 2 || jb->n_layers != 2 || products_mode(who, &mode_sc, ja->layers, 2) || products_mode(who, &mode_sb, jb->layers, 2)) return 0;
    if (mode != mode_sc || mode != mode_sb || !same_shape(ja, jb) || ja->feat_dtype != a->feat_dtype) return 0;
    if (!cv_chain(a->C, mode) || setconv_chain_shape(ja, jb, mode) != 1) return 0;
    if (a->K <= 0 || a->K > 32) return 0;
    *mode_out = mode;
    return 1;
#endif
}

extern "C" int elo_cv_stage1_setconv_chain_form(const elo_cv1_args *a, const elo_setconv_args *ja, const elo_setconv_args *jb)
{
    int mode = 0;
    return chain_pair_form(a, ja, jb, &mode, "elo_cv_stage1_setconv_chain_form");
}

extern "C" int elo_cv_stage1_setconv_chain(const elo_cv1_args *a, const elo_setconv_args *ja, const elo_setconv_args *jb,
                                           elo_stream_t stream)
{
    const char *who = "elo_cv_stage1_setconv_chain";
#ifdef ELO_DENSE_F32
    (void)a; (void)ja; (void)jb; (void)stream;
    return fail(ELO_ERR_LIMIT, "%s: the fp32-MFMA comparison build has no register-resident kernels", who);
#else
    TilePlan pc, ps;
    if (int rc = plan_cv1(a, &pc, who)) return rc;
    ELO_REQUIRE(jb, who, "two set-conv jobs");
    if (int rc = check_setconv(ja, who)) return rc;
    if (int rc = check_setconv(jb, who)) return rc;
    if (!same_shape(ja, jb)) return fail(ELO_ERR_ARG, "%s: the two set-conv jobs must have the same shape", who);
    if (int rc = plan_setconv(ja, jb, &ps, who)) return rc;
    if (a->group.random_hw || !a->idx || !a->mask) return fail(ELO_ERR_ARG, "%s: the cost volume comes pre-grouped (idx / mask of the select-k pre-pass)", who);
    int mode = 0;
    if (!chain_pair_form(a, ja, jb, &mode, who) || mode != pc.mode || mode != ps.mode)
        return fail(ELO_ERR_ARG, "%s: not a chain-form launch (elo_cv_stage1_setconv_chain_form returns 0)", who);
    const long pts_cv = (long)a->batch * a->npoints, pts_sc = (long)ja->batch * ja->npoints;
    if (pts_cv == 0 || pts_sc == 0) return fail(ELO_ERR_ARG, "%s: empty batch (call the separate entry points)", who);
    const int Pc = RR_ROWS / a->K, Ps = RR_ROWS / ja->K;
    const unsigned n_cv = (unsigned)((pts_cv + Pc - 1) / Pc), n_sc = (unsigned)((pts_sc + Ps - 1) / Ps);
    const dim3 grid(n_cv + 2u * n_sc);
    JobPair<elo_setconv_args> pair;
    pair.job[0] = *ja;
    pair.job[1] = *jb;
    hipStream_t s = (hipStream_t)stream;
    const bool f16 = a->feat_dtype == ELO_F16;
#define RRP(CC)                                                                                                                              \
    do {                                                                                                                                    \
        if (f16 && mode == MODE_HALF) hipLaunchKernelGGL((cv1_setconv_rr_kernel<CC, true, MODE_HALF>), grid, dim3(RR_WAVES * 64), RR_LDS_BYTES, s, *a, pair, n_cv, n_sc);   \
        else if (f16) hipLaunchKernelGGL((cv1_setconv_rr_kernel<CC, true, MODE_SPLIT>), grid, dim3(RR_WAVES * 64), RR_LDS_BYTES, s, *a, pair, n_cv, n_sc);                 \
        else if (mode == MODE_HALF) hipLaunchKernelGGL((cv1_setconv_rr_kernel<CC, false, MODE_HALF>), grid, dim3(RR_WAVES * 64), RR_LDS_BYTES, s, *a, pair, n_cv, n_sc);   \
        else hipLaunchKernelGGL((cv1_setconv_rr_kernel<CC, false, MODE_SPLIT>), grid, dim3(RR_WAVES * 64), RR_LDS_BYTES, s, *a, pair, n_cv, n_sc);                          \
    } while (0)
    if (a->C == 16) RRP(16);
    else if (a->C == 32) RRP(32);
    else RRP(64);
#undef RRP
    ++g_rr_launches[0];
    ++g_rr_launches[2];
    ++g_chain_pair_launches;
    return check_launch(who);
#endif
}

extern "C" int elo_cv_stage2_fused(const elo_cv2_args *a, elo_stream_t stream)
{
    const char *who = "elo_cv_stage2_fused";
    ELO_REQUIRE(a, who, "null argument block");
    ELO_REQUIRE(a->batch >= 0 && a->npoints > 0 && a->K > 0 && a->H > 0 && a->W > 0 && a->C > 0, who, "bad sizes");
    ELO_REQUIRE(a->npoints == a->H * a->W, who, "npoints must equal H*W (every pixel is a centre)");
    if (a->K > 32) return fail(ELO_ERR_LIMIT, "%s: K = %d exceeds the 32-row tile", who, a->K);
    if (a->C > 64) return fail(ELO_ERR_LIMIT, "%s: C = %d exceeds 64", who, a->C);
    ELO_REQUIRE(a->xyz1 && a->feat1 && a->cost && a->out, who, "null tensor pointer");
    ELO_REQUIRE(a->group.random_hw || (a->idx && a->mask), who, "neither idx/mask nor a grouping spec");
    if (int rc = check_dtype(a->feat_dtype, who)) return rc;
    if (int rc = check_cv_features(who, a->C, a->feat_dtype == ELO_F16, {a->feat1, a->cost})) return rc;
    if (int rc = check_dense(a->xyz_enc, 10, 64, who, "sum_xyz_encoding")) return rc;
    if (int rc = check_dense(a->sum_cost0, 128 + a->C, 128, who, "sum_cost_volume_0")) return rc;
    if (int rc = check_dense(a->sum_cost1, 128, 64, who, "sum_cost_volume_1")) return rc;
    const long points = (long)a->batch * a->npoints;
    if (points >= 0x7fffffffL) return fail(ELO_ERR_LIMIT, "%s: batch * npoints beyond 2^31", who);
    if (points == 0) return ELO_OK;
    const int S = row_stride(208);
    const int P32 = 32 / a->K, P16 = a->K <= 16 ? 16 / a->K : 1;
    const long u32 = (points + P32 - 1) / P32, u16 = (points + P16 - 1) / P16;
    int mode = 0;
    if (int rc = products_mode(who, &mode, a->xyz_enc, a->sum_cost0, a->sum_cost1)) return rc;
    const bool t16 = small_tile(u32, a->K);
    const int KT = a->group.random_hw ? a->group.kernel_h * a->group.kernel_w : 0;
    const size_t lds = tile_lds_bytes(t16 ? 16 : 32, S, KT, false);
    if (int rc = check_group(a->group, a->H, a->W, lds, who)) return rc;
    hipStream_t s = (hipStream_t)stream;
#ifndef ELO_DENSE_F32
    if (!a->group.random_hw && cv_chain(a->C, mode)) {
        const int P = RR_ROWS / a->K;
        const dim3 rgrid((unsigned)((points + P - 1) / P));
        const bool f16 = a->feat_dtype == ELO_F16;
#define RR(CC)                                                                                                           \
        do {                                                                                                             \
            if (f16 && mode == MODE_HALF) hipLaunchKernelGGL((cv2_rr_kernel<CC, true, MODE_HALF>), rgrid, dim3(RR_WAVES * 64), RR_LDS_BYTES, s, *a);     \
            else if (f16) hipLaunchKernelGGL((cv2_rr_kernel<CC, true, MODE_SPLIT>), rgrid, dim3(RR_WAVES * 64), RR_LDS_BYTES, s, *a);     \
            else if (mode == MODE_HALF) hipLaunchKernelGGL((cv2_rr_kernel<CC, false, MODE_HALF>), rgrid, dim3(RR_WAVES * 64), RR_LDS_BYTES, s, *a);        \
            else hipLaunchKernelGGL((cv2_rr_kernel<CC, false, MODE_SPLIT>), rgrid, dim3(RR_WAVES * 64), RR_LDS_BYTES, s, *a);        \
        } while (0)
        if (a->C == 16) RR(16);
        else if (a->C == 32) RR(32);
        else RR(64);
#undef RR
        ++g_rr_launches[1];
        return check_launch(who);
    }
#endif
    const dim3 grid((unsigned)(t16 ? u16 : u32));
#define CALL(k) hipLaunchKernelGGL(k, grid, dim3(FUSED_BLOCK), lds, s, *a, S)
    ELO_PICK(cv2_kernel, t16, mode, CALL);
#undef CALL
    return check_launch(who);
}
```

### efficientlo-net_amd/fused.py

```python
import ctypes
import os

import torch

from . import _lib as L
from . import tf_util, tuning


def fp32_mfma():
    return bool(L.lib().elo_dense_f32())


PRODUCTS_SPLIT, PRODUCTS_HALF = 0, 1
_products = PRODUCTS_SPLIT


def products_mode():
    return _products


class products:

    def __init__(self, mode):
        self.mode = {"split": PRODUCTS_SPLIT, "half": PRODUCTS_HALF, PRODUCTS_SPLIT: PRODUCTS_SPLIT,
                     PRODUCTS_HALF: PRODUCTS_HALF}[mode]
        if self.mode == PRODUCTS_HALF and fp32_mfma():
            raise RuntimeError("libelo_hip.so was built with -DELO_DENSE_F32: no fp16 products")

    def __enter__(self):
        global _products
        self.prev, _products = _products, self.mode
        return self

    def __exit__(self, *exc):
        global _products
        _products = self.prev


_storage = torch.float32


def storage_dtype():
    return _storage


class storage:

    def __init__(self, dtype):
        if dtype not in (torch.float32, torch.float16):
            raise TypeError("feature storage is torch.float32 or torch.float16")
        self.dtype = dtype

    def __enter__(self):
        global _storage
        self.prev, _storage = _storage, self.dtype
        return self

    def __exit__(self, *exc):
        global _storage
        _storage = self.prev


def _features(*ts):
    live = [t for t in ts if t is not None]
    dt = live[0].dtype
    if dt not in (torch.float32, torch.float16) or any(t.dtype != dt for t in live):
        raise TypeError("the feature tensors of a call are all float32 or all float16 (got %s)" % [str(t.dtype) for t in live])
    return [None if t is None else t.contiguous() for t in ts], dt, L.dtype_code(live[0])


class PackedDense:

    def __init__(self, W, b, relu=True, row_order=None, half=False):
        if row_order is not None:
            W = W[row_order]
        K, N = W.shape
        if not fp32_mfma():
            peak = float(W.abs().max()) if W.numel() else 0.0
            if not peak < 65504.0:
                raise ValueError("a folded weight of magnitude %g does not fit the fp16 hi/lo split of the fused kernels "
                                 "(|w| < 65504): rescale the layer or run the fp32-MFMA build (ELO_DENSE_F32=1)" % peak)
        Kp, Np = (K + 15) // 16 * 16, (N + 15) // 16 * 16
        Wp = torch.zeros((Kp, Np), dtype=torch.float32, device=W.device)
        Wp[:K, :N] = W
        CB, KS, NP = Np // 16, Kp // 16, Kp // 32
        frag = Wp.reshape(KS, 4, 4, CB, 16).permute(3, 0, 1, 4, 2).reshape(CB, KS, 64, 4).contiguous()
        self.products = PRODUCTS_HALF if half else PRODUCTS_SPLIT

        def paired(h4):
            parts = []
            if NP:
                parts.append(torch.cat([h4[:, 0:2 * NP:2], h4[:, 1:2 * NP:2]], -1))
            return parts, (h4[:, KS - 1] if KS % 2 else None)

        if fp32_mfma():
            self.w = frag
        elif half:
            pairs, tail = paired(frag.to(torch.float16))
            flat = [p.reshape(CB, -1) for p in pairs] + ([tail.reshape(CB, -1)] if tail is not None else [])
            self.w = torch.cat(flat, 1).contiguous()
        else:
            hi = frag.to(torch.float16)
            lo = (frag - hi.to(torch.float32)).to(torch.float16)
            (ph, th), (pl, tl) = paired(hi), paired(lo)
            flat = []
            if ph:
                flat.append(torch.stack([ph[0], pl[0]], 2).reshape(CB, -1))
            if th is not None:
                flat.append(torch.cat([th, tl], -1).reshape(CB, -1))
            self.w = torch.cat(flat, 1).contiguous()
        self.b = torch.zeros((Np,), dtype=torch.float32, device=W.device)
        self.b[:N] = b
        self.K, self.N, self.relu = K, N, relu
        self.plain = W.contiguous() if max(K, N) <= 32 else None

    def struct(self):
        return L.Dense(self.w.data_ptr(), self.b.data_ptr(), self.K, self.N, 1 if self.relu else 0,
                       self.plain.data_ptr() if self.plain is not None else None, self.products)


def packed_layer(scope, cin, cout, bn=True, relu=True, row_order=None, tf_kernel_dims=(1, 1)):
    store = tf_util.get_store()
    name, W, b, bn_vars = tf_util.dense_variables(scope, cin, cout, tf_kernel_dims, bn)
    half = _products == PRODUCTS_HALF
    key = ("packed", name, None if row_order is None else tuple(row_order), relu, half)
    hit = store._folded.get(key)
    if hit is None:
        Wf, bf = store.folded(name, W, b, bn_vars)
        order = None if row_order is None else torch.as_tensor(row_order, device=Wf.device)
        hit = PackedDense(Wf, bf, relu, order, half)
        store._folded[key] = hit
    return hit


def setconv_row_order(C):
    return list(range(3, 3 + C)) + [0, 1, 2]


def cv0_row_order(C):
    return list(range(10, 10 + 2 * C)) + list(range(10))


def stage2_row_order(w_before, n_out, w_after):
    return (list(range(w_before, w_before + n_out)) + list(range(w_before)) +
            list(range(w_before + n_out, w_before + n_out + w_after)))


def _f32c(t):
    if t.dtype != torch.float32:
        raise TypeError("geometry tensors (xyz, masks) are float32")
    return t.contiguous()


def _chain(layers):
    arr = (L.Dense * 3)()
    for i, p in enumerate(layers):
        arr[i] = p.struct()
    return arr


class Grouping:

    def __init__(self, random_hw, kernel_size, distance, stride_h=1, stride_w=1, want_indices=False):
        self.random_hw = random_hw.contiguous()
        self.kernel_h, self.kernel_w = int(kernel_size[0]), int(kernel_size[1])
        self.distance, self.stride_h, self.stride_w = float(distance), int(stride_h), int(stride_w)
        self.want_indices = want_indices
        self.idx = self.mask = None

    def struct(self, B, N, K, device):
        if self.random_hw.dtype != torch.int32 or self.random_hw.numel() != self.kernel_h * self.kernel_w:
            raise ValueError("FusedConv expects (kernel_size_h * kernel_size_w) random_hw shape.")
        if self.want_indices:
            self.idx = torch.empty((B, N, K, 3), dtype=torch.int32, device=device)
            self.mask = torch.empty((B, N, K), dtype=torch.float32, device=device)
        return L.GroupSpec(self.random_hw.data_ptr(), self.kernel_h, self.kernel_w, self.distance, self.stride_h,
                           self.stride_w, self.idx.data_ptr() if self.want_indices else None,
                           self.mask.data_ptr() if self.want_indices else None,
                           _decoded_order(self.random_hw, self.kernel_h, self.kernel_w))


_DECODED = {}


def _decoded_order(random_hw, kH, kW):
    from . import perm
    pooled = perm.pooled_decoded(random_hw)
    if pooled is not None:
        return pooled.data_ptr()
    key = (random_hw.data_ptr(), kH, kW)
    hit = _DECODED.get(key)
    if hit is not None and hit[0] is random_hw and hit[1] == random_hw._version:
        return hit[2].data_ptr()
    if random_hw.is_cuda and torch.cuda.is_current_stream_capturing():
        return None
    p = random_hw.to(torch.int64)
    dec = ((((p // kW) - kH // 2) << 16) | (((p % kW) - kW // 2) & 0xffff)).to(torch.int32).contiguous()
    if len(_DECODED) >= 512:
        _DECODED.clear()
    _DECODED[key] = (random_hw, random_hw._version, dec)
    return dec.data_ptr()


_NO_GROUP = L.GroupSpec(None, 0, 0, 0.0, 0, 0, None, None, None)


def _setconv_args(src_xyz, src_feat, idx, mask, layers, centre_xyz=None, xyz1_grid=None, centre_hw=None, group=None,
                  K=None):
    L.require_gpu(src_xyz, src_feat, idx, mask, centre_xyz, xyz1_grid, centre_hw)
    src_xyz = _f32c(src_xyz)
    (src_feat,), dt, code = _features(src_feat)
    _, H2, W2, C = src_feat.shape
    dev = src_xyz.device
    ptr = lambda x: x.data_ptr() if x is not None else None
    H = W = 0
    if xyz1_grid is not None:
        xyz1_grid = _f32c(xyz1_grid)
        H, W = xyz1_grid.shape[1:3]
    if group is None:
        idx, mask = idx.contiguous(), _f32c(mask)
        B, n, K, _ = idx.shape
    else:
        B = src_xyz.shape[0]
        n = centre_hw.shape[1] if centre_hw is not None else H * W
    new_xyz = None
    if centre_hw is not None:
        centre_hw = centre_hw.contiguous()
        new_xyz = torch.empty((B, n, 3), dtype=torch.float32, device=dev)
    elif centre_xyz is not None:
        centre_xyz = _f32c(centre_xyz)
    out = torch.empty((B, n, layers[-1].N), dtype=dt, device=dev)
    a = L.SetconvArgs(B, n, K, H, W, H2, W2, C, ptr(xyz1_grid), ptr(centre_hw), ptr(centre_xyz), src_xyz.data_ptr(),
                      src_feat.data_ptr(), ptr(idx), ptr(mask), len(layers), _chain(layers), out.data_ptr(), ptr(new_xyz),
                      group.struct(B, n, K, dev) if group is not None else _NO_GROUP, code)
    keep = (src_xyz, src_feat, idx, mask, centre_xyz, xyz1_grid, centre_hw, layers, group)
    return a, out, new_xyz, keep


def setconv(src_xyz, src_feat, idx, mask, layers, centre_xyz=None, xyz1_grid=None, centre_hw=None, group=None, K=None):
    job = _setconv_args(src_xyz, src_feat, idx, mask, layers, centre_xyz, xyz1_grid, centre_hw, group, K)
    L.call("elo_setconv_fused", job[0], job[1])
    return job[1], job[2]


def setconv_pair(job_a, job_b):
    ja, jb = _setconv_args(**job_a), _setconv_args(**job_b)
    L.call2("elo_setconv_fused2", ja[0], jb[0], ja[1])
    return (ja[1], ja[2]), (jb[1], jb[2])


def _mlp_args(sources, layers):
    L.require_gpu(*sources)
    batch_hint = sources[0].shape[0] if sources[0].dim() >= 3 else 0
    srcs, dt, code = _features(*sources)
    srcs = [s.reshape(-1, s.shape[-1]) for s in srcs]
    rows = srcs[0].shape[0]
    out = torch.empty((rows, layers[-1].N), dtype=dt, device=srcs[0].device)
    a = L.MlpArgs()
    a.rows, a.n_sources, a.n_layers, a.layers, a.out = rows, len(srcs), len(layers), _chain(layers), out.data_ptr()
    a.feat_dtype, a.batch_hint = code, batch_hint
    for i, s in enumerate(srcs):
        a.src[i], a.src_width[i] = s.data_ptr(), s.shape[1]
    return a, out, (srcs, layers)


def _ride_clear(a, clear, dt):
    if clear is None:
        return
    if clear.out_feat is not None and clear.out_feat.dtype != dt:
        raise TypeError("the projection buffers and the MLP's features must share one storage dtype")
    B, _N, H, W, C = clear.shape
    a.clear_scratch, a.clear_xyz = clear.scratch.data_ptr(), clear.out_xyz.data_ptr()
    a.clear_feat = clear.out_feat.data_ptr() if clear.out_feat is not None else None
    a.clear_cells, a.clear_C, a.clear_images = B * H * W, C, B
    clear.cleared = True


def _ride_sv(a, b, sv, dt):
    if sv is None:
        return False
    B, N, _ = sv.xyz.shape
    if a.rows != B * N:
        raise ValueError("the SvPartials cloud (%d x %d points) does not match the MLP's %d rows" % (B, N, a.rows))
    a.sv_npoints = N
    parts = L.lib().elo_mlp_sv_parts(ctypes.byref(a), ctypes.byref(b) if b is not None else None)
    if parts <= 0:
        a.sv_npoints = 0
        return False
    a.sv_scratch, a.sv_xyz = sv.scratch.data_ptr(), sv.xyz.data_ptr()
    if b is None:
        feat = sv.feature
        if feat is None or feat.shape != (B, N, 64) or feat.dtype != dt:
            raise ValueError("a single launch takes its (B, N, 64) features of the MLP's storage dtype from SvPartials.feature")
        sv.feature = feat = feat.contiguous()
        a.sv_feature = feat.data_ptr()
    sv.parts = parts
    return True


def mlp(sources, layers, clear=None, sv=None):
    a, out, _keep = _mlp_args(sources, layers)
    if _ride_sv(a, None, sv, out.dtype) or sv is None:
        _ride_clear(a, clear, out.dtype)
    L.call("elo_mlp_fused", a, out)
    return out.reshape(sources[0].shape[:-1] + (layers[-1].N,))


def mlp_pair(sources_a, layers_a, sources_b, layers_b):
    a, out_a, _ka = _mlp_args(sources_a, layers_a)
    b, out_b, _kb = _mlp_args(sources_b, layers_b)
    L.call2("elo_mlp_fused2", a, b, out_a)
    lead = sources_a[0].shape[:-1]
    return out_a.reshape(lead + (layers_a[-1].N,)), out_b.reshape(lead + (layers_b[-1].N,))


def _mlp2_args(sources, layers, before, after, layers2):
    a, out, keep = _mlp_args(sources, layers)
    rows = out.shape[0]
    before, after = _features(before, after, out)[0][:2]
    flat = lambda t: None if t is None else t.reshape(rows, t.shape[-1])
    before, after = flat(before), flat(after)
    out2 = torch.empty((rows, layers2[-1].N), dtype=out.dtype, device=out.device)
    a.n_layers2, a.layers2, a.out2 = len(layers2), _chain(layers2), out2.data_ptr()
    a.before, a.w_before = (before.data_ptr(), before.shape[1]) if before is not None else (None, 0)
    a.after, a.w_after = (after.data_ptr(), after.shape[1]) if after is not None else (None, 0)
    return a, out, out2, (keep, before, after, layers2)


def mlp2_pair(job_a, job_b, clear=None, sv=None):
    a, out_a, out2_a, _ka = _mlp2_args(**job_a)
    b, out_b, out2_b, _kb = _mlp2_args(**job_b)
    if _ride_sv(a, b, sv, out_a.dtype) or sv is None:
        _ride_clear(a, clear, out_a.dtype)
    L.call2("elo_mlp_fused2", a, b, out_a)
    lead = job_a["sources"][0].shape[:-1]
    shape = lambda t: t.reshape(lead + (t.shape[-1],))
    return (shape(out_a), shape(out2_a)), (shape(out_b), shape(out2_b))


THROUGHPUT_BATCH = 4


def _prepass_rows(stage=1, batch=1):
    e = tuning.get("cv_prepass")
    if e is None:
        return 8192 if batch >= THROUGHPUT_BATCH else (20000 if stage == 1 else 65536)
    return (1 << 60) if e == 0 else 0 if e == 1 else int(e)


_HW = {}


def _all_pixels(B, H, W, device):
    key = (B, H, W, str(device))
    hit = _HW.get(key)
    if hit is None:
        hh = torch.arange(H, dtype=torch.int32, device=device).view(1, H, 1, 1).expand(B, H, W, 1)
        ww = torch.arange(W, dtype=torch.int32, device=device).view(1, 1, W, 1).expand(B, H, W, 1)
        hit = torch.cat([hh, ww], -1).reshape(B, H * W, 2).contiguous()
        if hit.is_cuda and torch.cuda.is_current_stream_capturing():
            return hit
        if len(_HW) >= 64:
            _HW.clear()
        _HW[key] = hit
    return hit




def group_prepass(kind, xyz1_grid, xyz2_grid, group, K):
    B, H, W, _ = xyz1_grid.shape
    _, H2, W2, _ = xyz2_grid.shape
    N, kH, kW = H * W, group.kernel_h, group.kernel_w
    idx = torch.empty((B, N, K, 3), dtype=torch.int32, device=xyz1_grid.device)
    mask = torch.empty((B, N, K), dtype=torch.float32, device=xyz1_grid.device)
    if kind == "select":
        from .fused_conv import _select_dense_fits
        dense = -(-W // 64) * H * B >= tuning.get("select_dense_tiles") and _select_dense_fits(kH, kW, K, 0, group.stride_h, group.stride_w)
        entry = "elo_fused_conv_select_k_dense" if dense else "elo_fused_conv_select_k"
    else:
        RH, RW = 1 // group.stride_h + kH, 63 // group.stride_w + kW
        dense = 4 * ((kH * kW + 7) & ~7) + 16 * RH * RW + 4 * (129 * K + 256) <= 64 * 1024
        entry = "elo_fused_conv_random_k_dense" if dense else "elo_fused_conv_random_k"
    hw = None if dense else _all_pixels(B, H, W, xyz1_grid.device)
    a = L.GroupArgs(B, H, W, H2, W2, N, kH, kW, K, 0, group.distance, group.stride_h, group.stride_w,
                    xyz1_grid.data_ptr(), xyz2_grid.data_ptr(), None if dense else hw.data_ptr(), group.random_hw.data_ptr(),
                    idx.data_ptr(), None, None, mask.data_ptr())
    L.call(entry, a, idx)
    return idx, mask


def _rr_path(group, B, N, K, C, stage=1):
    return (group is not None and not group.want_indices and K <= 32 and B * N * K >= _prepass_rows(stage, B)
            and group.stride_h == 1 and group.stride_w == 1 and not fp32_mfma()
            and C in (16, 32, 64))


_RECORD = None


class recording:

    def __enter__(self):
        global _RECORD
        self.prev, _RECORD = _RECORD, []
        return _RECORD

    def __exit__(self, *exc):
        global _RECORD
        _RECORD = self.prev


def _record(stage, args, kwargs):
    keep = lambda v: v.detach().clone() if torch.is_tensor(v) else v
    kw = {k: keep(v) for k, v in kwargs.items() if k != "side"}
    if kwargs.get("group") is not None:
        g = kwargs["group"]
        kw["group"] = Grouping(g.random_hw.clone(), [g.kernel_h, g.kernel_w], g.distance, g.stride_h, g.stride_w)
    _RECORD.append((stage, tuple(keep(v) for v in args), kw, bool(kwargs.get("side"))))


def cv_stage1(xyz1, feat1, xyz2_proj, feat2_proj, idx, mask, cv0, cv1, cv2, cv_xyz, sum_cv0, sum_cv1, group=None, K=None,
              side=None, side_chain=False):
    L.require_gpu(xyz1, feat1, xyz2_proj, feat2_proj, idx, mask)
    if _RECORD is not None:
        _record(1, (xyz1, feat1, xyz2_proj, feat2_proj, idx, mask, cv0, cv1, cv2, cv_xyz, sum_cv0, sum_cv1), dict(group=group, K=K, side=side))
    xyz1, xyz2_proj = _f32c(xyz1), _f32c(xyz2_proj)
    (feat1, feat2_proj), dt, code = _features(feat1, feat2_proj)
    _, H2, W2, C = feat2_proj.shape
    B, N = xyz1.shape[0], xyz1.shape[1]
    ptr = lambda x: x.data_ptr() if x is not None else None
    chain_jobs = None
    if side and side_chain:
        rr = len(side) == 2 and N == H2 * W2 and _rr_path(group, B, N, K, C)
        if rr:
            chain_jobs = [_setconv_args(**job) for job in side]
            probe = L.Cv1Args(B, N, K, H2, W2, C, None, None, None, None, None, None, cv0.struct(), cv1.struct(), cv2.struct(),
                              cv_xyz.struct(), sum_cv0.struct(), sum_cv1.struct(), None, _NO_GROUP, code)
            if L.lib().elo_cv_stage1_setconv_chain_form(ctypes.byref(probe), ctypes.byref(chain_jobs[0][0]), ctypes.byref(chain_jobs[1][0])) != 1:
                chain_jobs = None
        if chain_jobs is None:
            return cv_stage1_alone(xyz1, feat1, xyz2_proj, feat2_proj, idx, mask, cv0, cv1, cv2, cv_xyz, sum_cv0, sum_cv1, group, K), None
    if (not side or chain_jobs) and N == H2 * W2 and _rr_path(group, B, N, K, C):
        idx, mask = group_prepass("select", xyz1.reshape(B, H2, W2, 3), xyz2_proj, group, K)
        group = None
    if group is None:
        idx, mask = idx.contiguous(), _f32c(mask)
        K = idx.shape[2]
    out = torch.empty((B, N, 64), dtype=dt, device=xyz1.device)
    a = L.Cv1Args(B, N, K, H2, W2, C, xyz1.data_ptr(), feat1.data_ptr(), xyz2_proj.data_ptr(), feat2_proj.data_ptr(),
                  ptr(idx), ptr(mask), cv0.struct(), cv1.struct(), cv2.struct(), cv_xyz.struct(),
                  sum_cv0.struct(), sum_cv1.struct(), out.data_ptr(),
                  group.struct(B, N, K, xyz1.device) if group is not None else _NO_GROUP, code)
    if chain_jobs:
        L.call3("elo_cv_stage1_setconv_chain", a, chain_jobs[0][0], chain_jobs[1][0], out)
        return out, [(j[1], j[2]) for j in chain_jobs]
    if side:
        jobs = [_setconv_args(**job) for job in side]
        L.call3("elo_cv_stage1_setconv_fused", a, jobs[0][0], jobs[1][0] if len(jobs) > 1 else None, out)
        return out, [(j[1], j[2]) for j in jobs]
    L.call("elo_cv_stage1_fused", a, out)
    return out


def cv_stage1_alone(xyz1, feat1, xyz2_proj, feat2_proj, idx, mask, cv0, cv1, cv2, cv_xyz, sum_cv0, sum_cv1, group, K):
    global _RECORD
    keep, _RECORD = _RECORD, None
    try:
        return cv_stage1(xyz1, feat1, xyz2_proj, feat2_proj, idx, mask, cv0, cv1, cv2, cv_xyz, sum_cv0, sum_cv1, group=group, K=K)
    finally:
        _RECORD = keep


def cv_stage2(xyz1_proj, feat1_proj, cost_proj, idx, mask, xyz_enc, sum_cost0, sum_cost1, group=None, K=None):
    L.require_gpu(xyz1_proj, feat1_proj, cost_proj, idx, mask)
    if _RECORD is not None:
        _record(2, (xyz1_proj, feat1_proj, cost_proj, idx, mask, xyz_enc, sum_cost0, sum_cost1), dict(group=group, K=K))
    xyz1_proj = _f32c(xyz1_proj)
    (feat1_proj, cost_proj), dt, code = _features(feat1_proj, cost_proj)
    B, H, W, C = feat1_proj.shape
    N = H * W
    ptr = lambda x: x.data_ptr() if x is not None else None
    if _rr_path(group, B, N, K, C, stage=2):
        idx, mask = group_prepass("random", xyz1_proj, xyz1_proj, group, K)
        group = None
    if group is None:
        idx, mask = idx.contiguous(), _f32c(mask)
        K = idx.shape[2]
    out = torch.empty((B, N, 64), dtype=dt, device=xyz1_proj.device)
    a = L.Cv2Args(B, N, K, H, W, C, xyz1_proj.data_ptr(), feat1_proj.data_ptr(), cost_proj.data_ptr(), ptr(idx),
                  ptr(mask), xyz_enc.struct(), sum_cost0.struct(), sum_cost1.struct(), out.data_ptr(),
                  group.struct(B, N, K, xyz1_proj.device) if group is not None else _NO_GROUP, code)
    L.call("elo_cv_stage2_fused", a, out)
    return out
```

### efficientlo-net_amd/pointnet_util.py

```python
import os

import torch

from . import _ops, fused, tf_util, tuning
from .fused_conv import fused_conv_random_k, fused_conv_select_k, register_dense_index
from .perm import random_shuffle


def use_fused(flag):
    tuning.set_host("fused", bool(flag))


def _fused_path(is_training):
    return tuning.get("fused") and not is_training


def _store_round(x):
    return x.half().float() if fused.storage_dtype() == torch.float16 else x


def _storage_boundary(*feature_args, tuple_out=False):
    import functools
    import inspect

    def deco(fn):
        sig = inspect.signature(fn)

        @functools.wraps(fn)
        def wrapped(*args, **kw):
            b = sig.bind(*args, **kw)
            b.apply_defaults()
            if _fused_path(b.arguments["is_training"]):
                return fn(*args, **kw)
            halves = [n for n in feature_args if torch.is_tensor(b.arguments.get(n)) and b.arguments[n].dtype == torch.float16]
            if not halves:
                return fn(*args, **kw)
            if b.arguments["is_training"]:
                raise NotImplementedError("training stores its features in fp32")
            for n in halves:
                b.arguments[n] = b.arguments[n].float()
            with fused.storage(torch.float16):
                out = fn(*b.args, **b.kwargs)
            return ((out[0].half(),) + tuple(out[1:])) if tuple_out else out.half()
        return wrapped
    return deco


def warping_layers(xyz1, upsampled_flow):
    return xyz1 + upsampled_flow


_hw_cache = {}
_centre_hw_cache = {}


def _centre_hw(selected_idx):
    key = (selected_idx.data_ptr(), tuple(selected_idx.shape), str(selected_idx.device))
    hit = _centre_hw_cache.get(key)
    if hit is None or hit[0] is not selected_idx:
        B = selected_idx.shape[0]
        hit = (selected_idx, selected_idx.reshape(B, -1, 3)[:, :, 1:].contiguous())
        if len(_centre_hw_cache) > 64:
            _centre_hw_cache.clear()
        _centre_hw_cache[key] = hit
    return hit[1]


def get_hw_idx(B, H, W, device="cuda"):
    key = (B, H, W, str(device))
    if key not in _hw_cache:
        hh = torch.arange(H, dtype=torch.int32, device=device).view(1, H, 1, 1).expand(B, H, W, 1)
        ww = torch.arange(W, dtype=torch.int32, device=device).view(1, 1, W, 1).expand(B, H, W, 1)
        grid = torch.cat([hh, ww], -1).reshape(B, H * W, 2).contiguous()
        if grid.is_cuda and torch.cuda.is_current_stream_capturing():
            return grid
        if len(_hw_cache) >= 256:
            _hw_cache.clear()
        _hw_cache[key] = register_dense_index(grid)
    return _hw_cache[key]


def _split_conv(parts, num_output_channels, scope, is_training, bn_decay, bn=True):
    if is_training:
        return tf_util.conv2d(torch.cat(parts, -1), num_output_channels, [1, 1], padding='VALID', stride=[1, 1],
                              bn=bn, is_training=is_training, scope=scope, bn_decay=bn_decay)
    cin = sum(p.shape[-1] for p in parts)
    lead = parts[0].shape[:-1]
    W, b = tf_util.folded_variables(scope, cin, num_output_channels, (1, 1), bn)
    y, row = None, 0
    for i, p in enumerate(parts):
        c = p.shape[-1]
        x2 = p.reshape(-1, c)
        if y is None:
            y = torch.addmm(b, x2, W[row:row + c])
        elif i + 1 < len(parts):
            y = y.addmm_(x2, W[row:row + c])
        else:
            y = torch._addmm_activation(y, x2, W[row:row + c])
        row += c
    return y.reshape(lead + (num_output_channels,))


@_storage_boundary("points1_proj", "points2_proj")
def cost_volume(warped_xyz1_proj, xyz2_proj, points1_proj, points2_proj, kernel_size1, kernel_size2, nsample,
                nsample_q, distance, mlp1, mlp2, is_training, bn_decay, scope, bn=True, pooling='max', knn=True,
                corr_func='elementwise_product', side_jobs=None, side_chain=False):
    with tf_util.variable_scope(scope):
        B, H, W, _ = warped_xyz1_proj.shape
        N = H * W
        warped_xyz1 = warped_xyz1_proj.reshape(B, N, 3)
        points1 = points1_proj.reshape(B, N, -1)
        dev = warped_xyz1_proj.device

        C = points1.shape[-1]
        random_HW_q = random_shuffle(tf_util.scope_name(), "random_HW_q", kernel_size2[0] * kernel_size2[1], dev, kernel_size2)
        random_HW_p = random_shuffle(tf_util.scope_name(), "random_HW_p", kernel_size1[0] * kernel_size1[1], dev, kernel_size1)
        if _fused_path(is_training) and nsample_q <= 32 and nsample <= 32:
            if list(mlp1) != [128, 64, 64] or list(mlp2) != [128, 64]:
                raise NotImplementedError("the fused cost volume is built for mlp1=[128,64,64], mlp2=[128,64]")
            P = fused.packed_layer
            stage1 = fused.cv_stage1(
                warped_xyz1, points1, xyz2_proj, points2_proj, None, None,
                P('CV_0', 10 + 2 * C, 128, row_order=fused.cv0_row_order(C)), P('CV_1', 128, 64), P('CV_2', 64, 64),
                P('CV_xyz', 10, 64),
                P('sum_CV_0', 128, 128, row_order=list(range(64, 128)) + list(range(64))),
                P('sum_CV_1', 128, 64),
                group=fused.Grouping(random_HW_q, kernel_size2, 1000), K=nsample_q, side=side_jobs, side_chain=side_chain)
            pi_feat1_new, side_out = stage1 if side_jobs else (stage1, None)
            pi_feat1_new = pi_feat1_new.reshape(B, H, W, -1)
            order = list(range(64 + C, 128 + C)) + list(range(64)) + list(range(64, 64 + C))
            cost = fused.cv_stage2(warped_xyz1_proj, points1_proj, pi_feat1_new, None, None,
                                   P('sum_xyz_encoding', 10, 64), P('sum_cost_volume_0', 128 + C, 128, row_order=order),
                                   P('sum_cost_volume_1', 128, 64),
                                   group=fused.Grouping(random_HW_p, kernel_size1, distance), K=nsample)
            return (cost, side_out) if side_jobs else cost
        if side_jobs:
            raise NotImplementedError("side_jobs ride on the fused cost-volume launch only")

        idx_hw = get_hw_idx(B, H, W, dev)
        qi_idx, _, _, valid_mask = fused_conv_select_k(
            warped_xyz1_proj, xyz2_proj, idx_hw, random_HW_q, H, W, N, kernel_size2[0], kernel_size2[1], nsample_q,
            flag_copy=0, distance=1000, stride_h=1, stride_w=1, want_valid=False)
        mask = valid_mask.reshape(B, N, nsample_q)
        pi_feat1_new = _store_round(_cost_volume_stage1(warped_xyz1, points1, xyz2_proj, points2_proj, qi_idx, mask, mlp1, mlp2,
                                                        is_training, bn_decay)).reshape(B, H, W, -1)

        pc_idx, _, _, valid_mask2 = fused_conv_random_k(
            warped_xyz1_proj, warped_xyz1_proj, idx_hw, random_HW_p, H, W, N, kernel_size1[0], kernel_size1[1],
            nsample, flag_copy=0, distance=distance, stride_h=1, stride_w=1, want_valid=False)
        mask2 = valid_mask2.reshape(B, N, nsample)
        return _cost_volume_stage2(warped_xyz1_proj, points1_proj, pi_feat1_new, pc_idx, mask2, mlp1, mlp2, is_training,
                                   bn_decay)


def _cost_volume_stage1(warped_xyz1, points1, xyz2_proj, points2_proj, qi_idx, mask, mlp1, mlp2, is_training, bn_decay):
    B, N, nsample_q = mask.shape
    feat_cat = _ops.cv_encode1(warped_xyz1, points1, xyz2_proj, points2_proj, qi_idx, mask)
    xyz_cat = feat_cat.reshape(-1, feat_cat.shape[-1])[:, :10]
    x = feat_cat
    for j, num_out_channel in enumerate(mlp1):
        x = tf_util.conv2d(x, num_out_channel, [1, 1], padding='VALID', stride=[1, 1], bn=True,
                           is_training=is_training, scope='CV_%d' % j, bn_decay=bn_decay)
    enc = tf_util.conv2d(xyz_cat, mlp1[-1], [1, 1], padding='VALID', stride=[1, 1], bn=True,
                         is_training=is_training, scope='CV_xyz', bn_decay=bn_decay)
    enc = enc.reshape(B, N, nsample_q, -1)
    cat = None
    for j, num_out_channel in enumerate(mlp2):
        if j == 0:
            cat = _split_conv([enc, x], num_out_channel, 'sum_CV_0', is_training, bn_decay)
        else:
            cat = tf_util.conv2d(cat, num_out_channel, [1, 1], padding='VALID', stride=[1, 1], bn=True,
                                 is_training=is_training, scope='sum_CV_%d' % j, bn_decay=bn_decay)
    return _ops.masked_softmax_pool(cat, x, mask)


def _cost_volume_stage2(warped_xyz1_proj, points1_proj, pi_feat1_new, pc_idx, mask2, mlp1, mlp2, is_training, bn_decay):
    C = points1_proj.shape[-1]
    pc_xyz_cat, rest = _ops.cv_encode2(warped_xyz1_proj, points1_proj, pi_feat1_new, pc_idx, mask2)
    pc_enc = tf_util.conv2d(pc_xyz_cat, mlp1[-1], [1, 1], padding='VALID', stride=[1, 1], bn=True,
                            is_training=is_training, scope='sum_xyz_encoding', bn_decay=bn_decay)
    pc_cat = None
    for j, num_out_channel in enumerate(mlp2):
        if j == 0:
            pc_cat = _split_conv([pc_enc, rest], num_out_channel, 'sum_cost_volume_0', is_training, bn_decay)
        else:
            pc_cat = tf_util.conv2d(pc_cat, num_out_channel, [1, 1], padding='VALID', stride=[1, 1], bn=True,
                                    is_training=is_training, scope='sum_cost_volume_%d' % j, bn_decay=bn_decay)
    pc_points_grouped = rest[..., C:]
    return _ops.masked_softmax_pool(pc_cat, pc_points_grouped, mask2)


@_storage_boundary("points_f1", "upsampled_feat", "cost_volume")
def flow_predictor(points_f1, upsampled_feat, cost_volume, mlp, is_training, bn_decay, scope, bn=True, clear=None, sv=None):
    with tf_util.variable_scope(scope):
        parts = [points_f1]
        if upsampled_feat is not None:
            parts.append(upsampled_feat)
        if cost_volume is not None:
            parts.append(cost_volume)
        if _fused_path(is_training) and len(mlp) <= 3:
            widths = [sum(p.shape[-1] for p in parts)] + list(mlp)
            layers = [fused.packed_layer('conv_predictor%d' % i, widths[i], widths[i + 1], bn=bn)
                      for i in range(len(mlp))]
            return fused.mlp(parts, layers, clear=clear, sv=sv)
        parts = [p.unsqueeze(2) for p in parts]
        x = None
        for i, num_out_channel in enumerate(mlp):
            if i == 0:
                x = _split_conv(parts, num_out_channel, 'conv_predictor0', is_training, bn_decay, bn=bn)
            else:
                x = tf_util.conv2d(x, num_out_channel, [1, 1], padding='VALID', stride=[1, 1], bn=bn,
                                   is_training=is_training, scope='conv_predictor%d' % i, bn_decay=bn_decay)
        return x.squeeze(2)


def fused_pairs_available(is_training):
    return _fused_path(is_training)




def merge_branches(is_training, finest_points, level_points=0):
    return (_fused_path(is_training) and finest_points <= tuning.get("merge_points") and
            level_points <= tuning.get("merge_level_points"))


def flow_predictor_pair(call_a, call_b):
    specs = []
    for c in (call_a, call_b):
        with tf_util.variable_scope(c["scope"]):
            parts = [p for p in (c["points_f1"], c["upsampled_feat"], c["cost_volume"]) if p is not None]
            widths = [sum(p.shape[-1] for p in parts)] + list(c["mlp"])
            layers = [fused.packed_layer('conv_predictor%d' % i, widths[i], widths[i + 1], bn=c.get("bn", True))
                      for i in range(len(c["mlp"]))]
        specs.append((parts, layers))
    return fused.mlp_pair(specs[0][0], specs[0][1], specs[1][0], specs[1][1])


def up_conv_pair(call_a, call_b):
    jobs, stage2 = [], []
    for c in (call_a, call_b):
        with tf_util.variable_scope(c["scope"]):
            xyz1_proj, feat1_proj, feat2_proj = c["xyz1_proj"], c["feat1_proj"], c["feat2_proj"]
            B, H, W, _ = xyz1_proj.shape
            ks, mlp, mlp2 = c["kernel_size"], c["mlp"], c["mlp2"]
            random_HW = random_shuffle(tf_util.scope_name(), "random_HW", ks[0] * ks[1], xyz1_proj.device, ks)
            P = fused.packed_layer
            w1 = [3 + feat2_proj.shape[-1]] + list(mlp)
            jobs.append(dict(src_xyz=c["xyz2_proj"], src_feat=feat2_proj, idx=None, mask=None,
                             layers=[P('up_1_%d' % j, w1[j], w1[j + 1],
                                       row_order=fused.setconv_row_order(w1[0] - 3) if j == 0 else None)
                                     for j in range(len(mlp))],
                             xyz1_grid=xyz1_proj, K=c["nsample"],
                             group=fused.Grouping(random_HW, ks, c["distance"], c["stride_h"], c["stride_w"])))
            points1 = feat1_proj.reshape(B, H * W, -1)
            w2 = [mlp[-1] + points1.shape[-1]] + list(mlp2)
            stage2.append((points1, [P('up_2_%d' % i, w2[i], w2[i + 1]) for i in range(len(mlp2))]))
    (up_a, _), (up_b, _) = fused.setconv_pair(jobs[0], jobs[1])
    return fused.mlp_pair([up_a, stage2[0][0]], stage2[0][1], [up_b, stage2[1][0]], stage2[1][1])


def up_conv_predict_pair(up_a, up_b, fp_a, fp_b):
    jobs = up_conv_stage1_jobs(up_a, up_b)
    (up_a_pooled, _), (up_b_pooled, _) = fused.setconv_pair(jobs[0], jobs[1])
    return up_conv_predict_finish(up_a, up_b, fp_a, fp_b, up_a_pooled, up_b_pooled)


def up_conv_stage1_jobs(up_a, up_b):
    jobs = []
    for up in (up_a, up_b):
        P = fused.packed_layer
        with tf_util.variable_scope(up["scope"]):
            feat2_proj, ks, mlp = up["feat2_proj"], up["kernel_size"], up["mlp"]
            random_HW = random_shuffle(tf_util.scope_name(), "random_HW", ks[0] * ks[1], up["xyz1_proj"].device, ks)
            w1 = [3 + feat2_proj.shape[-1]] + list(mlp)
            jobs.append(dict(src_xyz=up["xyz2_proj"], src_feat=feat2_proj, idx=None, mask=None,
                             layers=[P('up_1_%d' % j, w1[j], w1[j + 1],
                                       row_order=fused.setconv_row_order(w1[0] - 3) if j == 0 else None)
                                     for j in range(len(mlp))],
                             xyz1_grid=up["xyz1_proj"], K=up["nsample"],
                             group=fused.Grouping(random_HW, ks, up["distance"], up["stride_h"], up["stride_w"])))
    return jobs


def up_conv_predict_finish(up_a, up_b, fp_a, fp_b, up_a_pooled, up_b_pooled, clear=None, sv=None):
    stage2 = []
    for up, fp, pooled in ((up_a, fp_a, up_a_pooled), (up_b, fp_b, up_b_pooled)):
        P = fused.packed_layer
        with tf_util.variable_scope(up["scope"]):
            feat1_proj, mlp, mlp2 = up["feat1_proj"], up["mlp"], up["mlp2"]
            B, H, W, _ = up["xyz1_proj"].shape
            points1 = feat1_proj.reshape(B, H * W, -1)
            w2 = [mlp[-1] + points1.shape[-1]] + list(mlp2)
            layers = [P('up_2_%d' % i, w2[i], w2[i + 1]) for i in range(len(mlp2))]
        with tf_util.variable_scope(fp["scope"]):
            before, after = fp["points_f1"], fp["cost_volume"]
            wp = [sum(p.shape[-1] for p in (before, after) if p is not None) + mlp2[-1]] + list(fp["mlp"])
            w_before = before.shape[-1] if before is not None else 0
            w_after = after.shape[-1] if after is not None else 0
            layers2 = [P('conv_predictor%d' % i, wp[i], wp[i + 1], bn=fp.get("bn", True),
                         row_order=fused.stage2_row_order(w_before, mlp2[-1], w_after) if i == 0 else None)
                       for i in range(len(fp["mlp"]))]
        stage2.append(dict(sources=[pooled, points1], layers=layers, before=before, after=after, layers2=layers2))
    (out_a, pred_a), (out_b, pred_b) = fused.mlp2_pair(stage2[0], stage2[1], clear=clear, sv=sv)
    return out_a, pred_a, out_b, pred_b


def down_conv_job(xyz_proj, points_proj, selected_idx, K_sample, kernel_size, distance, mlp, scope, bn=True):
    with tf_util.variable_scope(scope):
        random_HW = random_shuffle(tf_util.scope_name(), "random_HW", kernel_size[0] * kernel_size[1], xyz_proj.device, kernel_size)
        widths = [3 + points_proj.shape[-1]] + list(mlp)
        layers = [fused.packed_layer('conv%d' % i, widths[i], widths[i + 1], bn=bn,
                                     row_order=fused.setconv_row_order(widths[0] - 3) if i == 0 else None)
                  for i in range(len(mlp))]
    job = dict(src_xyz=xyz_proj, src_feat=points_proj, idx=None, mask=None, layers=layers, xyz1_grid=xyz_proj,
               centre_hw=_centre_hw(selected_idx), K=K_sample, group=fused.Grouping(random_HW, kernel_size, distance))
    return job, lambda out, new_xyz: (out, new_xyz.reshape(selected_idx.shape[:-1] + (3,)))


@_storage_boundary("points_proj", tuple_out=True)
def down_conv(xyz_proj, points_proj, selected_idx, K_sample, kernel_size, distance, mlp, mlp2, flag_add, is_training,
              bn_decay, scope, bn=True, pooling='max', knn=False, use_xyz=True, use_nchw=False):
    if use_nchw or pooling != 'max' or mlp2 is not None:
        raise NotImplementedError("the model uses NHWC, max pooling and mlp2=None (pwclo_model.py:126-177)")
    with tf_util.variable_scope(scope):
        B, H, W, _ = xyz_proj.shape
        idx_n2 = selected_idx.reshape(B, -1, 3)
        n_sampled = idx_n2.shape[1]
        dev = xyz_proj.device
        random_HW = random_shuffle(tf_util.scope_name(), "random_HW", kernel_size[0] * kernel_size[1], dev, kernel_size)
        centre_hw = _centre_hw(selected_idx)
        if _fused_path(is_training) and len(mlp) <= 3 and K_sample <= 32:
            widths = [3 + points_proj.shape[-1]] + list(mlp)
            layers = [fused.packed_layer('conv%d' % i, widths[i], widths[i + 1], bn=bn,
                                         row_order=fused.setconv_row_order(widths[0] - 3) if i == 0 else None)
                      for i in range(len(mlp))]
            out, new_xyz = fused.setconv(xyz_proj, points_proj, None, None, layers, xyz1_grid=xyz_proj,
                                         centre_hw=centre_hw, K=K_sample,
                                         group=fused.Grouping(random_HW, kernel_size, distance))
            return out, new_xyz.reshape(selected_idx.shape[:-1] + (3,))
        sel, _, _, valid_mask = fused_conv_random_k(
            xyz_proj, xyz_proj, centre_hw, random_HW, H, W, n_sampled, kernel_size[0],
            kernel_size[1], K_sample, flag_copy=0, distance=distance, stride_h=1, stride_w=1, want_valid=False)
        mask = valid_mask.reshape(B, n_sampled, K_sample)
        li = selected_idx.reshape(-1, 3).long()
        new_xyz_proj = xyz_proj[li[:, 0], li[:, 1], li[:, 2]].reshape(selected_idx.shape[:-1] + (3,))
        new_xyz = new_xyz_proj.reshape(B, -1, 3)
        x = _ops.group_concat(new_xyz, xyz_proj, points_proj, sel, mask)
        for i, num_out_channel in enumerate(mlp):
            x = tf_util.conv2d(x, num_out_channel, [1, 1], padding='VALID', stride=[1, 1], bn=bn,
                               is_training=is_training, scope='conv%d' % i, bn_decay=bn_decay)
        return _ops.masked_maxpool(x, mask), new_xyz_proj


@_storage_boundary("feat1_proj", "feat2_proj")
def up_conv(xyz1_proj, xyz2_proj, feat1_proj, feat2_proj, kernel_size, stride_h, stride_w, nsample, distance, mlp,
            mlp2, is_training, scope, bn_decay=None, bn=True, pooling='max', radius=None, knn=True):
    with tf_util.variable_scope(scope):
        B, H, W, _ = xyz1_proj.shape
        N = H * W
        dev = xyz1_proj.device
        xyz1 = xyz1_proj.reshape(B, N, 3)
        points1 = feat1_proj.reshape(B, N, -1)
        random_HW = random_shuffle(tf_util.scope_name(), "random_HW", kernel_size[0] * kernel_size[1], dev, kernel_size)
        if _fused_path(is_training) and len(mlp) <= 3 and len(mlp2) <= 3 and nsample <= 32:
            P = fused.packed_layer
            w1 = [3 + feat2_proj.shape[-1]] + list(mlp)
            up_feat, _ = fused.setconv(xyz2_proj, feat2_proj, None, None,
                                       [P('up_1_%d' % j, w1[j], w1[j + 1],
                                          row_order=fused.setconv_row_order(w1[0] - 3) if j == 0 else None)
                                        for j in range(len(mlp))],
                                       xyz1_grid=xyz1_proj, K=nsample,
                                       group=fused.Grouping(random_HW, kernel_size, distance, stride_h, stride_w))
            w2 = [mlp[-1] + points1.shape[-1]] + list(mlp2)
            return fused.mlp([up_feat, points1], [P('up_2_%d' % i, w2[i], w2[i + 1]) for i in range(len(mlp2))])
        idx_hw = get_hw_idx(B, H, W, dev)
        sel, _, _, valid_mask = fused_conv_random_k(
            xyz1_proj, xyz2_proj, idx_hw, random_HW, H, W, N, kernel_size[0], kernel_size[1], nsample,
            flag_copy=0, distance=distance, stride_h=stride_h, stride_w=stride_w, want_valid=False)
        mask = valid_mask.reshape(B, N, nsample)
        x = _ops.group_concat(xyz1, xyz2_proj, feat2_proj, sel, mask)
        for j, num_out_channel in enumerate(mlp):
            x = tf_util.conv2d(x, num_out_channel, [1, 1], padding='VALID', stride=[1, 1], bn=True,
                               is_training=is_training, scope='up_1_%d' % j, bn_decay=bn_decay)
        up_feat = _store_round(_ops.masked_maxpool(x, mask))
        y = None
        for i, num_out_channel in enumerate(mlp2):
            if i == 0:
                y = _split_conv([up_feat.unsqueeze(2), points1.unsqueeze(2)], num_out_channel, 'up_2_0',
                                is_training, bn_decay)
            else:
                y = tf_util.conv2d(y, num_out_channel, [1, 1], padding='VALID', stride=[1, 1], bn=True,
                                   is_training=is_training, scope='up_2_%d' % i, bn_decay=bn_decay)
        return y.squeeze(2)
```

### efficientlo-net_amd/pwclo_model.py

```python
import math
import os

import numpy as np
import torch

from . import _ops, fused, tf_util, tuning
from .model_util import (PreProcess, ProjectPC2SphericalRing, input_stage, preprocess_gt, get_selected_idx, inv_q, mul_point_q, mul_q_point,
                         softmax_valid, warp_and_project)
from .pointnet_util import (cost_volume, down_conv, down_conv_job, flow_predictor, fused_pairs_available, merge_branches,
                            up_conv, up_conv_predict_finish, up_conv_stage1_jobs)

Down_conv_dis = [0.5, 3.0, 6.0, 12.0]
Up_conv_dis = [3.0, 6.0, 9.0]
Cost_volume_dis = [1.0, 2.0, 4.0]
stride_h_list = [1, 1, 4, 2, 2, 1]
stride_w_list = [1, 1, 8, 2, 2, 2]


def pyramid_sizes(H_input, W_input):
    out_h = [math.ceil(H_input / stride_h_list[0])]
    out_w = [math.ceil(W_input / stride_w_list[0])]
    for i in range(1, 6):
        out_h.append(math.ceil(out_h[i - 1] / stride_h_list[i]))
        out_w.append(math.ceil(out_w[i - 1] / stride_w_list[i]))
    return out_h, out_w


def variable_specs():
    specs = []

    def chain(prefix, names, cin, couts, bn=True, dims=(1, 1)):
        for n, cout in zip(names, couts):
            specs.append((prefix + n, cin, cout, dims, bn))
            cin = cout

    conv3 = ['conv0', 'conv1', 'conv2']
    chain('sa1/layer0/', conv3, 3 + 3, [8, 8, 16])
    chain('sa1/layer1/', conv3, 3 + 16, [16, 16, 32])
    chain('sa1/layer2/', conv3, 3 + 32, [32, 32, 64])
    chain('sa1/layer3/', conv3, 3 + 64, [64, 64, 128])
    for scope, C in (('flow_embedding_l2_origin', 64), ('flow_embedding_l2', 64), ('flow_embedding_l1', 32),
                     ('flow_embedding_l0', 16)):
        chain(scope + '/', ['CV_0', 'CV_1', 'CV_2'], 10 + 2 * C, [128, 64, 64])
        chain(scope + '/', ['CV_xyz'], 10, [64])
        chain(scope + '/', ['sum_CV_0', 'sum_CV_1'], 128, [128, 64])
        chain(scope + '/', ['sum_xyz_encoding'], 10, [64])
        chain(scope + '/', ['sum_cost_volume_0', 'sum_cost_volume_1'], 64 + C + 64, [128, 64])
    chain('new_layer3/', conv3, 3 + 64, [128, 64, 64])
    pred = ['conv_predictor0', 'conv_predictor1']
    chain('l3_costvolume_predict_ww/', pred, 128 + 64, [128, 64])
    for level, C in ((2, 64), (1, 32), (0, 16)):
        for kind in ('w', 'costvolume'):
            chain('up_sa_layer_layer_l%d%s/' % (level, kind), ['up_1_0', 'up_1_1'], 3 + 64, [128, 64])
            chain('up_sa_layer_layer_l%d%s/' % (level, kind), ['up_2_0', 'up_2_1'], 64 + C, [128, 64])
        chain('l%d_costvolume_predict/' % level, pred, C + 64 + 64, [128, 64])
        chain('l%d_w_predict/' % level, pred, C + 64 + 64, [128, 64])
    for level in (3, 2, 1, 0):
        heads = ('q_coarse', 't_coarse') if level == 3 else ('q_det', 't_det')
        specs.append(('l%d_big' % level, 64, 256, (1,), False))
        specs.append(('l%d_%s' % (level, heads[0]), 256, 4, (1,), False))
        specs.append(('l%d_%s' % (level, heads[1]), 256, 3, (1,), False))
    return specs


def create_variables(store=None):
    store = store if store is not None else tf_util.get_store()
    with tf_util.default_store(store):
        for scope, cin, cout, dims, bn in variable_specs():
            tf_util.dense_variables(scope, cin, cout, dims, bn)
    return store


def placeholder_inputs(batch_size, NUM_POINTS, device="cuda"):
    z = lambda *s: torch.zeros(s, dtype=torch.float32, device=device)
    return z(batch_size, NUM_POINTS * 2, 6), z(batch_size, 4, 4), z(batch_size, 4, 4), z(batch_size, 4, 4)


def _parallel(branches, is_training=False):
    return [b() for b in branches]


def _adjacent_frames(a, b):
    if (a.shape == b.shape and a.dtype == b.dtype and a.device == b.device and a.is_contiguous() and b.is_contiguous()
            and b.data_ptr() == a.data_ptr() + a.numel() * a.element_size()
            and a.untyped_storage().data_ptr() == b.untyped_storage().data_ptr()):
        return torch.as_strided(a, (2 * a.shape[0],) + tuple(a.shape[1:]), a.stride())
    return None


PROJECTION_TAP = None

_ZEROS = {}


def _zero_features(like):
    dtype = fused.storage_dtype()
    key = (tuple(like.shape), like.device, dtype)
    if key not in _ZEROS:
        if like.is_cuda and torch.cuda.is_current_stream_capturing():
            return torch.zeros_like(like, dtype=dtype)
        _ZEROS[key] = torch.zeros_like(like, dtype=dtype)
    return _ZEROS[key]


def _normalise_q(q):
    return q / (torch.sqrt((q * q).sum(-1, keepdim=True) + 1e-10) + 1e-10)


def _pose_head(feat_b1c, level, coarse, is_training, raw=False):
    big = tf_util.conv1d(feat_b1c, 256, 1, padding='VALID', activation_fn=None, scope='l%d_big' % level, is_training=is_training)
    if is_training:
        big = torch.nn.functional.dropout(big, p=0.5, training=True)
    qn, tn = ('l%d_q_coarse', 'l%d_t_coarse') if coarse else ('l%d_q_det', 'l%d_t_det')
    q = tf_util.conv1d(big, 4, 1, padding='VALID', activation_fn=None, scope=qn % level, is_training=is_training)
    t = tf_util.conv1d(big, 3, 1, padding='VALID', activation_fn=None, scope=tn % level, is_training=is_training)
    return (q if raw else _normalise_q(q)), t


def _estimate_pose(predict, weight, xyz, level, q_coarse, t_coarse, is_training, pose7=None, clear=None, warp=None, partials=None):
    batch_size = predict.shape[0]
    coarse = q_coarse is None
    if not is_training:
        qn, tn = ('l%d_q_coarse', 'l%d_t_coarse') if coarse else ('l%d_q_det', 'l%d_t_det')
        W_big, b_big = tf_util.folded_variables('l%d_big' % level, predict.shape[-1], 256, (1,), bn=False)
        W_q, b_q = tf_util.folded_variables(qn % level, 256, 4, (1,), bn=False)
        W_t, b_t = tf_util.folded_variables(tn % level, 256, 3, (1,), bn=False)
        from . import perm
        nxt = perm.tail_refresh_args() if level == 0 else None
        return _ops.pose_head(predict, weight, xyz, W_big, b_big, W_q, b_q, W_t, b_t, q_coarse, t_coarse, pose7, clear, warp, nxt, partials)
    summed = softmax_valid(feature_bnc=predict, weight_bnc=weight, mask_valid=xyz)
    if predict.is_cuda and pose7 is None:
        q_raw, t_det = _pose_head(summed, level, coarse, is_training, raw=True)
        return _ops.pose_compose(q_raw, t_det, q_coarse, t_coarse)
    q_det, t_det = _pose_head(summed, level, coarse, is_training)
    if coarse:
        q = q_det.squeeze(1)
        return q, t_det.squeeze(1), _normalise_q(q)
    dev = predict.device
    t_coarse_trans = torch.cat([torch.zeros((batch_size, 1, 1), dtype=torch.float32, device=dev), t_coarse], -1)
    t_coarse_trans = mul_q_point(q_det, t_coarse_trans, batch_size)
    t_coarse_trans = mul_point_q(t_coarse_trans, inv_q(q_det, batch_size), batch_size)[:, :, 1:]
    q = mul_point_q(q_det, q_coarse, batch_size).squeeze(1)
    t = (t_coarse_trans + t_det).squeeze(1)
    q_norm = _normalise_q(q)
    if pose7 is not None:
        pose7.copy_(torch.cat([q_norm, t], -1).detach())
    return q, t, q_norm


def get_model_from_projection(xyz_f1_input_proj, xyz_f2_input_proj, is_training, bn_decay=None, pose_out=None):
    batch_size, H_input, W_input, _ = xyz_f1_input_proj.shape
    dev = xyz_f1_input_proj.device
    out_h_list, out_w_list = pyramid_sizes(H_input, W_input)

    zero_features = _zero_features
    finest_points = batch_size * out_h_list[2] * out_w_list[2]

    pre2 = xyz_f1_input_proj
    l0_selected_idx = get_selected_idx(pre2, stride_h_list[2], stride_w_list[2], out_h_list[2], out_w_list[2])
    l1_selected_idx = get_selected_idx(pre2, stride_h_list[3], stride_w_list[3], out_h_list[3], out_w_list[3])
    l2_selected_idx = get_selected_idx(pre2, stride_h_list[4], stride_w_list[4], out_h_list[4], out_w_list[4])
    l3_selected_idx = get_selected_idx(pre2, stride_h_list[5], stride_w_list[5], out_h_list[5], out_w_list[5])

    def feature_pyramid(xyz_in, points_in, sel):
        l0_selected_idx, l1_selected_idx, l2_selected_idx, l3_selected_idx = sel
        batch_size = xyz_in.shape[0]
        l0_points, l0_xyz_proj = down_conv(xyz_in, points_in, l0_selected_idx, K_sample=32, kernel_size=[9, 15],
                                           distance=Down_conv_dis[0], mlp=[8, 8, 16], mlp2=None, flag_add=False,
                                           is_training=is_training, bn_decay=bn_decay, scope='layer0')
        l0_points_proj = l0_points.reshape(batch_size, out_h_list[2], out_w_list[2], -1)
        l1_points, l1_xyz_proj = down_conv(l0_xyz_proj, l0_points_proj, l1_selected_idx, K_sample=32,
                                           kernel_size=[7, 11], distance=Down_conv_dis[1], mlp=[16, 16, 32], mlp2=None,
                                           flag_add=False, is_training=is_training, bn_decay=bn_decay, scope='layer1')
        l1_points_proj = l1_points.reshape(batch_size, out_h_list[3], out_w_list[3], -1)
        l2_points, l2_xyz_proj = down_conv(l1_xyz_proj, l1_points_proj, l2_selected_idx, K_sample=16,
                                           kernel_size=[5, 9], distance=Down_conv_dis[2], mlp=[32, 32, 64], mlp2=None,
                                           flag_add=False, is_training=is_training, bn_decay=bn_decay, scope='layer2')
        l2_points_proj = l2_points.reshape(batch_size, out_h_list[4], out_w_list[4], -1)
        if merge_branches(is_training, finest_points, batch_size * out_h_list[4] * out_w_list[4]):
            deferred.append(down_conv_job(l2_xyz_proj, l2_points_proj, l3_selected_idx, K_sample=16, kernel_size=[5, 9],
                                          distance=Down_conv_dis[3], mlp=[64, 64, 128], scope='layer3'))
            l3_points = l3_xyz_proj = None
        else:
            l3_points, l3_xyz_proj = down_conv(l2_xyz_proj, l2_points_proj, l3_selected_idx, K_sample=16,
                                               kernel_size=[5, 9], distance=Down_conv_dis[3], mlp=[64, 64, 128], mlp2=None,
                                               flag_add=False, is_training=is_training, bn_decay=bn_decay, scope='layer3')
        return ([l0_points, l1_points, l2_points, l3_points],
                [l0_points_proj, l1_points_proj, l2_points_proj, None],
                [l0_xyz_proj, l1_xyz_proj, l2_xyz_proj, l3_xyz_proj])

    deferred = []
    with tf_util.variable_scope('sa1') as scope:
        both = _adjacent_frames(xyz_f1_input_proj, xyz_f2_input_proj) if not is_training else None
        siamese_train = (is_training and tuning.get("train_siamese_batch") and tuning.get("train_kernels")
                         and xyz_f1_input_proj.shape == xyz_f2_input_proj.shape)
        if siamese_train:
            both_t = torch.cat([xyz_f1_input_proj, xyz_f2_input_proj], 0)
            sel2 = [get_selected_idx(both_t, stride_h_list[i], stride_w_list[i], out_h_list[i], out_w_list[i])
                    for i in (2, 3, 4, 5)]
            with tf_util.bn_groups(2):
                pts, pts_proj, xyz_proj = feature_pyramid(both_t, zero_features(both_t), sel2)
            B = batch_size
            two = lambda t: (None, None) if t is None else t.split(B)
            pts_s = [two(p) for p in pts]
            pts_f1, pts_f2 = [a for a, _ in pts_s], [b for _, b in pts_s]
            shape_like = lambda t, ref: None if t is None or ref is None else t.reshape((B,) + tuple(ref.shape[1:]))
            pts_proj_f1 = [shape_like(a, ref) for a, ref in zip(pts_f1, pts_proj)]
            pts_proj_f2 = [shape_like(b, ref) for b, ref in zip(pts_f2, pts_proj)]
            xyz_s = [two(x) for x in xyz_proj]
            xyz_proj_f1, xyz_proj_f2 = [a for a, _ in xyz_s], [b for _, b in xyz_s]
        elif both is not None:
            sel2 = [get_selected_idx(both, stride_h_list[i], stride_w_list[i], out_h_list[i], out_w_list[i])
                    for i in (2, 3, 4, 5)]
            pts, pts_proj, xyz_proj = feature_pyramid(both, zero_features(both), sel2)
            B = batch_size
            half = lambda t, lo, hi: None if t is None else t[lo:hi]
            pts_f1, pts_f2 = [half(p, 0, B) for p in pts], [half(p, B, 2 * B) for p in pts]
            pts_proj_f1 = [half(p, 0, B) for p in pts_proj]
            pts_proj_f2 = [half(p, B, 2 * B) for p in pts_proj]
            xyz_proj_f1, xyz_proj_f2 = [half(x, 0, B) for x in xyz_proj], [half(x, B, 2 * B) for x in xyz_proj]
        else:
            sel1 = [l0_selected_idx, l1_selected_idx, l2_selected_idx, l3_selected_idx]
            points_input_proj = zero_features(xyz_f1_input_proj)
            pts_f1, pts_proj_f1, xyz_proj_f1 = feature_pyramid(xyz_f1_input_proj, points_input_proj, sel1)
            scope.reuse_variables()
            pts_f2, pts_proj_f2, xyz_proj_f2 = feature_pyramid(xyz_f2_input_proj, points_input_proj, sel1)

    l2_points_f1_new = cost_volume(xyz_proj_f1[2], xyz_proj_f2[2], pts_proj_f1[2], pts_proj_f2[2],
                                   kernel_size1=[3, 5], kernel_size2=[5, 35], nsample=4, nsample_q=32,
                                   distance=Cost_volume_dis[2], mlp1=[128, 64, 64], mlp2=[128, 64],
                                   is_training=is_training, bn_decay=bn_decay, scope='flow_embedding_l2_origin',
                                   bn=True, pooling='max', knn=True, corr_func='concat',
                                   side_jobs=[job for job, _ in deferred] or None)
    if deferred:
        l2_points_f1_new, side = l2_points_f1_new
        for f, ((_job, finish), (out, new_xyz)) in enumerate(zip(deferred, side)):
            l3_points, l3_xyz_proj = finish(out, new_xyz)
            if len(deferred) == 1 and l3_points.shape[0] == 2 * batch_size:
                pts_f1[3], pts_f2[3] = l3_points[:batch_size], l3_points[batch_size:]
                xyz_proj_f1[3], xyz_proj_f2[3] = l3_xyz_proj[:batch_size], l3_xyz_proj[batch_size:]
            else:
                (pts_f1 if f == 0 else pts_f2)[3] = l3_points
                (xyz_proj_f1 if f == 0 else xyz_proj_f2)[3] = l3_xyz_proj
    l2_points_new_proj_f1 = l2_points_f1_new.reshape(batch_size, out_h_list[4], out_w_list[4], -1)
    l3_points_f1_cost_volume, _ = down_conv(xyz_proj_f1[2], l2_points_new_proj_f1, l3_selected_idx, K_sample=16,
                                            kernel_size=[5, 9], distance=Down_conv_dis[3], mlp=[128, 64, 64], mlp2=None,
                                            flag_add=False, is_training=is_training, bn_decay=bn_decay,
                                            scope='new_layer3')

    l3_points_predict = l3_points_f1_cost_volume
    l3_points_predict_proj = l3_points_predict.reshape(batch_size, out_h_list[5], out_w_list[5], -1)
    l3_xyz_f1 = xyz_proj_f1[3].reshape(batch_size, -1, 3)
    inference = not is_training

    def projection_buffers(level, g):
        if not inference:
            return None
        return _ops.ProjectionBuffers(batch_size, xyz_proj_f1[level].shape[1] * xyz_proj_f1[level].shape[2],
                                      out_h_list[g], out_w_list[g], pts_f1[level].shape[-1], dev, pts_f1[level].dtype)
    def sv_ride(xyz_bn3, feature=None):
        if inference and fused_pairs_available(is_training) and tuning.get("sv_ride"):
            return _ops.SvPartials(xyz_bn3, feature)
        return None
    def next_warp(level):
        return (xyz_proj_f1[level].reshape(batch_size, -1, 3), pts_f1[level]) if inference else None
    next_buffers = projection_buffers(2, 4)
    sv3 = sv_ride(l3_xyz_f1, l3_points_predict)
    l3_cost_volume_w = flow_predictor(pts_f1[3], None, l3_points_predict, mlp=[128, 64], is_training=is_training,
                                      bn_decay=bn_decay, scope='l3_costvolume_predict_ww',
                                      clear=next_buffers if sv3 is not None else None,
                                      **({"sv": sv3} if sv3 is not None else {}))
    l3_cost_volume_w_proj = l3_cost_volume_w.reshape(batch_size, out_h_list[5], out_w_list[5], -1)
    l3_q, l3_t, l3_q_norm = _estimate_pose(l3_points_predict, l3_cost_volume_w, l3_xyz_f1, 3, None, None,
                                           is_training, clear=next_buffers, warp=next_warp(2), partials=sv3)

    cv_kernel2 = {2: [5, 15], 1: [7, 25], 0: [11, 41]}
    poses = {3: (l3_q_norm, l3_t)}
    q_prev, t_prev = l3_q, l3_t
    coarse_w_proj, coarse_predict_proj, coarse_xyz_proj = l3_cost_volume_w_proj, l3_points_predict_proj, xyz_proj_f1[3]
    for level, g in ((2, 4), (1, 3), (0, 2)):
        q_coarse = q_prev.reshape(batch_size, 1, -1)
        t_coarse = t_prev.reshape(batch_size, 1, -1)
        xyz_f1 = xyz_proj_f1[level].reshape(batch_size, -1, 3)
        _warped, xyz_warp_proj_f1, points_warp_proj_f1 = warp_and_project(
            xyz_f1, pts_f1[level], q_coarse, t_coarse, out_h_list[g], out_w_list[g], next_buffers)
        if PROJECTION_TAP is not None and next_buffers is not None:
            PROJECTION_TAP.append((level, next_buffers.scratch, batch_size, xyz_f1.shape[1], out_h_list[g], out_w_list[g], xyz_warp_proj_f1, _warped))
        next_buffers = projection_buffers(level - 1, g - 1) if level > 0 else None
        xyz_warp_f1 = xyz_warp_proj_f1.reshape(batch_size, -1, 3)
        points_warp_f1 = points_warp_proj_f1.reshape(batch_size, out_h_list[g] * out_w_list[g], -1)

        def branch_cost(side_jobs=None, side_chain=False):
            return cost_volume(xyz_warp_proj_f1, xyz_proj_f2[level], points_warp_proj_f1, pts_proj_f2[level],
                               kernel_size1=[3, 5], kernel_size2=cv_kernel2[level], nsample=4, nsample_q=6,
                               distance=Cost_volume_dis[level], mlp1=[128, 64, 64], mlp2=[128, 64],
                               is_training=is_training, bn_decay=bn_decay, scope='flow_embedding_l%d' % level,
                               bn=True, pooling='max', knn=True, corr_func='concat', side_jobs=side_jobs,
                               **({"side_chain": True} if side_chain else {}))

        def branch_up(kind, coarse_feat_proj):
            return up_conv(xyz_warp_proj_f1, coarse_xyz_proj, points_warp_proj_f1, coarse_feat_proj,
                           kernel_size=[7, 15], stride_h=stride_h_list[g + 1], stride_w=stride_w_list[g + 1],
                           nsample=8, distance=Up_conv_dis[level], mlp=[128, 64], mlp2=[128, 64],
                           scope='up_sa_layer_layer_l%d%s' % (level, kind), is_training=is_training,
                           bn_decay=bn_decay, knn=True)

        if fused_pairs_available(is_training):
            up = dict(xyz1_proj=xyz_warp_proj_f1, xyz2_proj=coarse_xyz_proj, feat1_proj=points_warp_proj_f1,
                      kernel_size=[7, 15], stride_h=stride_h_list[g + 1], stride_w=stride_w_list[g + 1], nsample=8,
                      distance=Up_conv_dis[level], mlp=[128, 64], mlp2=[128, 64])
            up_w = dict(up, feat2_proj=coarse_w_proj, scope='up_sa_layer_layer_l%dw' % level)
            up_c = dict(up, feat2_proj=coarse_predict_proj, scope='up_sa_layer_layer_l%dcostvolume' % level)
            jobs = up_conv_stage1_jobs(up_w, up_c)
            if merge_branches(is_training, finest_points, batch_size * out_h_list[g] * out_w_list[g]):
                cost, ((up_w_pooled, _), (up_c_pooled, _)) = branch_cost(side_jobs=jobs)
            else:
                pair = tuning.get("chain_pair") and finest_points <= tuning.get("merge_points")
                cost, sides = branch_cost(side_jobs=jobs, side_chain=True) if pair else (branch_cost(), None)
                (up_w_pooled, _), (up_c_pooled, _) = sides if sides is not None else fused.setconv_pair(jobs[0], jobs[1])
            fp = dict(points_f1=points_warp_f1, cost_volume=cost, mlp=[128, 64])
            sv = sv_ride(xyz_warp_f1)
            w_up_sample, weight, cost_up_sample, predict = up_conv_predict_finish(
                up_w, up_c, dict(fp, scope='l%d_w_predict' % level), dict(fp, scope='l%d_costvolume_predict' % level),
                up_w_pooled, up_c_pooled, clear=next_buffers if sv is not None else None, sv=sv)
        else:
            cost, w_up_sample, cost_up_sample = _parallel([branch_cost, lambda: branch_up('w', coarse_w_proj),
                                                           lambda: branch_up('costvolume', coarse_predict_proj)], is_training)
            sv = None
            predict, weight = _parallel([
                lambda: flow_predictor(points_warp_f1, cost_up_sample, cost, mlp=[128, 64], is_training=is_training,
                                       bn_decay=bn_decay, scope='l%d_costvolume_predict' % level),
                lambda: flow_predictor(points_warp_f1, w_up_sample, cost, mlp=[128, 64], is_training=is_training,
                                       bn_decay=bn_decay, scope='l%d_w_predict' % level)], is_training)
        q_prev, t_prev, q_norm = _estimate_pose(predict, weight, xyz_warp_f1, level, q_coarse, t_coarse,
                                                is_training, pose_out if level == 0 else None,
                                                clear=next_buffers,
                                                warp=next_warp(level - 1) if level > 0 else None, partials=sv)
        poses[level] = (q_norm, t_prev)

        coarse_w_proj = weight.reshape(batch_size, out_h_list[g], out_w_list[g], -1)
        coarse_predict_proj = predict.reshape(batch_size, out_h_list[g], out_w_list[g], -1)
        coarse_xyz_proj = xyz_warp_proj_f1

    l0_xyz_f1 = xyz_proj_f1[0].reshape(batch_size, -1, 3)
    return (poses[0][0], poses[0][1], poses[1][0], poses[1][1], poses[2][0], poses[2][1], poses[3][0], poses[3][1],
            l0_xyz_f1)


def get_model(point_cloud, H_input, W_input, T_gt, T_trans, T_trans_inv, is_training, bn_decay=None, aug_frame=None):
    batch_size = point_cloud.shape[0]
    if aug_frame is None:
        aug_frame = np.random.choice([1, 2], size=batch_size, replace=True)
    with torch.no_grad():
        _points, both = input_stage(point_cloud, T_trans, aug_frame, H_input, W_input)
        xyz_f1_proj, xyz_f2_proj = both[:batch_size], both[batch_size:]
        q_gt, t_gt = preprocess_gt(T_gt, T_trans, T_trans_inv, aug_frame)
    out = get_model_from_projection(xyz_f1_proj, xyz_f2_proj, is_training, bn_decay)
    return out + (q_gt, t_gt)


def get_loss(l0_q, l0_t, l1_q, l1_t, l2_q, l2_t, l3_q, l3_t, q_gt, t_gt, w_x, w_q):
    if l0_q.is_cuda and w_x.is_cuda and w_x.dim() == 0:
        return _ops.pose_loss(l0_q, l0_t, l1_q, l1_t, l2_q, l2_t, l3_q, l3_t, q_gt, t_gt, w_x, w_q)
    t_gt = t_gt.squeeze(-1)

    def level(q, t):
        q_norm = _normalise_q(q)
        loss_q = torch.sqrt(((q_gt - q_norm) * (q_gt - q_norm)).sum(-1, keepdim=True) + 1e-10).mean()
        loss_x = torch.sqrt((t - t_gt) * (t - t_gt) + 1e-10).mean()
        return loss_x * torch.exp(-w_x) + w_x + loss_q * torch.exp(-w_q) + w_q

    return 1.6 * level(l3_q, l3_t) + 0.8 * level(l2_q, l2_t) + 0.4 * level(l1_q, l1_t) + 0.2 * level(l0_q, l0_t)
```

### efficientlo-net_amd/tf_util.py

```python
import contextlib
import math
import os

import torch
import torch.nn.functional as Fnn

from . import _ops, tuning

BN_EPS = 1e-3
_DEFAULT_BN_DECAY = 0.9


class VariableStore:

    def __init__(self, device="cuda", seed=0):
        self.device = torch.device(device)
        self.params = {}
        self.buffers = {}
        self.tf_shapes = {}
        self._scope = []
        self._folded = {}
        self.generation = 0
        self._gen = torch.Generator(device="cpu")
        self._gen.manual_seed(seed)

    @contextlib.contextmanager
    def variable_scope(self, name):
        self._scope.append(name)
        try:
            yield _Scope(self)
        finally:
            self._scope.pop()

    def full_name(self, name):
        return "/".join(self._scope + [name])

    def get_variable(self, name, shape, init, tf_shape=None, trainable=True):
        full = self.full_name(name)
        table = self.params if trainable else self.buffers
        if full in table:
            if tuple(table[full].shape) != tuple(shape):
                raise ValueError("variable %s exists with shape %s, requested %s"
                                 % (full, tuple(table[full].shape), tuple(shape)))
            return table[full]
        value = init(shape).to(self.device)
        table[full] = torch.nn.Parameter(value) if trainable else value
        self.tf_shapes[full] = tuple(tf_shape if tf_shape is not None else shape)
        return table[full]

    def xavier(self, fan_in, fan_out):
        limit = math.sqrt(6.0 / (fan_in + fan_out))
        return lambda shape: (torch.rand(shape, generator=self._gen, dtype=torch.float32) * 2 - 1) * limit

    def parameters(self):
        return list(self.params.values())

    def state_dict(self):
        out = {k: v.detach() for k, v in self.params.items()}
        out.update(self.buffers)
        return out

    def load_state_dict(self, state):
        with torch.no_grad():
            for k, v in state.items():
                target = self.params.get(k, self.buffers.get(k))
                if target is None:
                    raise KeyError("unknown variable " + k)
                target.copy_(torch.as_tensor(v).reshape(target.shape))
        self.invalidate()

    def invalidate(self):
        self._folded.clear()
        self.generation += 1

    def folded(self, scope_name, W, b, bn):
        key = scope_name
        hit = self._folded.get(key)
        if hit is None:
            with torch.no_grad():
                if bn is None:
                    hit = (W.detach().contiguous(), b.detach().contiguous())
                else:
                    gamma, beta, mean, var = bn
                    s = gamma / torch.sqrt(var + BN_EPS)
                    hit = ((W * s).contiguous(), ((b - mean) * s + beta).contiguous())
            self._folded[key] = hit
        return hit


class _Scope:
    def __init__(self, store):
        self.store = store

    def reuse_variables(self):
        """No-op: variables are always get-or-create (pwclo_model.py:143)."""


_current = []


@contextlib.contextmanager
def default_store(store):
    _current.append(store)
    try:
        yield store
    finally:
        _current.pop()


def get_store():
    if not _current:
        raise RuntimeError("no VariableStore is active: wrap the model in `with tf_util.default_store(store):`")
    return _current[-1]


def variable_scope(name):
    return get_store().variable_scope(name)


def scope_name():
    return "/".join(get_store()._scope)


def relu(x):
    return torch.relu(x)


def dense_variables(scope, cin, num_output_channels, tf_kernel_dims=(1, 1), bn=True):
    store = get_store()
    with store.variable_scope(scope):
        name = store.full_name("")[:-1]
        W = store.get_variable("weights", (cin, num_output_channels), store.xavier(cin, num_output_channels),
                               tf_shape=tuple(tf_kernel_dims) + (cin, num_output_channels))
        b = store.get_variable("biases", (num_output_channels,), torch.zeros)
        bn_vars = None
        if bn:
            with store.variable_scope("bn"):
                gamma = store.get_variable("gamma", (num_output_channels,), torch.ones)
                beta = store.get_variable("beta", (num_output_channels,), torch.zeros)
                mean = store.get_variable("moving_mean", (num_output_channels,), torch.zeros, trainable=False)
                var = store.get_variable("moving_variance", (num_output_channels,), torch.ones, trainable=False)
            bn_vars = (gamma, beta, mean, var)
    return name, W, b, bn_vars


def folded_variables(scope, cin, num_output_channels, tf_kernel_dims=(1, 1), bn=True):
    name, W, b, bn_vars = dense_variables(scope, cin, num_output_channels, tf_kernel_dims, bn)
    return get_store().folded(name, W, b, bn_vars)


_bn_groups = 1


@contextlib.contextmanager
def bn_groups(n):
    global _bn_groups
    prev, _bn_groups = _bn_groups, int(n)
    try:
        yield
    finally:
        _bn_groups = prev


def _dense(inputs, num_output_channels, scope, tf_kernel_dims, activation_fn, bn, bn_decay, is_training):
    cin = inputs.shape[-1]
    name, W, b, bn_vars = dense_variables(scope, cin, num_output_channels, tf_kernel_dims, bn)
    x2 = inputs.reshape(-1, cin)
    training = bool(is_training) if is_training is not None else False
    if training:
        decay = _DEFAULT_BN_DECAY if bn_decay is None else float(bn_decay)
        if (bn and tuning.get("train_kernels") and (activation_fn is relu or activation_fn is None)
                and _ops.dense_bn_supported(x2, num_output_channels)):
            y = _ops.dense_bn(x2, W, b, bn_vars[0], bn_vars[1], bn_vars[2], bn_vars[3], 1.0 - decay, BN_EPS,
                              activation_fn is relu, groups=_bn_groups)
            return y.reshape(inputs.shape[:-1] + (num_output_channels,))
        y = torch.addmm(b, x2, W)
        if bn:
            y = torch.cat([Fnn.batch_norm(part, bn_vars[2], bn_vars[3], bn_vars[0], bn_vars[1], training=training,
                                          momentum=1.0 - decay, eps=BN_EPS) for part in y.chunk(_bn_groups)]) if _bn_groups > 1 else \
                Fnn.batch_norm(y, bn_vars[2], bn_vars[3], bn_vars[0], bn_vars[1], training=training, momentum=1.0 - decay, eps=BN_EPS)
        if activation_fn is not None:
            y = activation_fn(y)
    else:
        Wf, bf = get_store().folded(name, W, b, bn_vars)
        if activation_fn is relu:
            y = torch._addmm_activation(bf, x2, Wf)
        else:
            y = torch.addmm(bf, x2, Wf)
            if activation_fn is not None:
                y = activation_fn(y)
    return y.reshape(inputs.shape[:-1] + (num_output_channels,))


def conv2d(inputs, num_output_channels, kernel_size, scope, stride=[1, 1], padding='SAME', data_format='NHWC',
           use_xavier=True, stddev=1e-3, weight_decay=None, activation_fn=relu, bn=False, bn_decay=None,
           is_training=None):
    if list(kernel_size) != [1, 1] or list(stride) != [1, 1] or data_format != 'NHWC':
        raise NotImplementedError("only 1x1, stride 1, NHWC convolutions are on the hot path")
    if not use_xavier or weight_decay is not None:
        raise NotImplementedError("the model uses xavier init without weight decay")
    return _dense(inputs, num_output_channels, scope, (1, 1), activation_fn, bn, bn_decay, is_training)


def conv1d(inputs, num_output_channels, kernel_size, scope, stride=1, padding='SAME', data_format='NHWC',
           use_xavier=True, stddev=1e-3, weight_decay=None, activation_fn=relu, bn=False, bn_decay=None,
           is_training=None):
    if kernel_size != 1 or stride != 1 or data_format != 'NHWC':
        raise NotImplementedError("only kernel 1, stride 1, NHWC 1-D convolutions are on the hot path")
    return _dense(inputs, num_output_channels, scope, (1,), activation_fn, bn, bn_decay, is_training)
```

### efficientlo-net_amd/tuning.py

```python
import contextlib
import hashlib
import json
import os

def _prepass(spec):
    return None if spec in (None, "") else int(spec)


_HOST = {
    "fused": ("ELO_FUSED", lambda v: v != "0", True),
    "cv_prepass": ("ELO_CV_PREPASS", _prepass, None),
    "select_dense_tiles": ("ELO_SELECT_DENSE_TILES", int, 1024),
    "merge_points": ("ELO_MERGE_POINTS", int, 8192),
    "merge_level_points": ("ELO_MERGE_LEVEL_POINTS", int, 2000),
    "chain_pair": ("ELO_CHAIN_PAIR", lambda v: v != "0", True),
    "native_submit": ("ELO_NATIVE_SUBMIT", lambda v: v != "0", True),
    "sv_ride": ("ELO_SV_RIDE", lambda v: v != "0", True),
    "train_kernels": ("ELO_TRAIN_KERNELS", lambda v: v != "0", True),
    "train_dense": ("ELO_TRAIN_DENSE", lambda v: v != "0", True),
    "train_dense_rows": ("ELO_TRAIN_DENSE_ROWS", int, 25000),
    "train_siamese_batch": ("ELO_TRAIN_SIAMESE_BATCH", lambda v: v != "0", True),
    "train_dense_fused_dz": ("ELO_TRAIN_DENSE_FUSED_DZ", lambda v: v != "0", True),
    "train_dense_dx_rows": ("ELO_TRAIN_DENSE_DX_ROWS", int, 100000),
}
_LIB = {
    "chain_forms": ("ELO_CV1_RR", 1), "narrow_mfma": ("ELO_SETCONV_NARROW_MFMA", 1), "range_check": ("ELO_RANGE_CHECK", 0),
    "select_dense_waves": ("ELO_SELECT_DENSE_WAVES", 0), "random_dense_rows": ("ELO_DENSE_ROWS", 0),
    "setconv_chain_rows": ("ELO_SETCONV_RR_ROWS", -1), "mlp_chain_rows": ("ELO_MLP_RR_ROWS", -1), "small_tile_units": ("ELO_SMALL_TILE_UNITS", 64),
    "pool_wave": ("ELO_POOL_WAVE", 1),
}


_LIB_BOOLEAN = ("chain_forms", "narrow_mfma", "range_check", "pool_wave")


def _host_from_env():
    out = {}
    for name, (var, parse, default) in _HOST.items():
        raw = os.environ.get(var)
        out[name] = default if raw is None else parse(raw)
    return out


def lib_from_env():
    out = {}
    for name, (var, _default) in _LIB.items():
        raw = os.environ.get(var)
        if raw is not None:
            value = int(raw)
            out[name] = (1 if value else 0) if name in _LIB_BOOLEAN else value
    return out


_host = _host_from_env()
_version = 0


def version():
    return _version


def bump():
    global _version
    _version += 1


def get(name):
    return _host[name]


def set_host(name, value):
    if name not in _HOST:
        raise KeyError(name)
    prev, _host[name] = _host[name], value
    bump()
    return prev


@contextlib.contextmanager
def override(**fields):
    from . import _lib
    host = {k: v for k, v in fields.items() if k in _HOST}
    lib = {k: v for k, v in fields.items() if k in _LIB}
    unknown = set(fields) - set(host) - set(lib)
    if unknown:
        raise KeyError("unknown tuning field(s): %s" % sorted(unknown))
    prev_host = {k: _host[k] for k in host}
    prev_lib = _lib.get_tuning_base() if lib else None
    try:
        _host.update(host)
        bump()
        if lib:
            _lib.set_tuning(**lib)
        yield
    finally:
        _host.update(prev_host)
        bump()
        if prev_lib is not None:
            _lib.set_tuning(**prev_lib)


def snapshot():
    from . import _lib, fused
    snap = {k: (dict(v) if isinstance(v, dict) else v) for k, v in _host.items()}
    snap["lib"] = _lib.get_tuning()
    snap["products"] = "half" if fused.products_mode() == fused.PRODUCTS_HALF else "split"
    snap["storage"] = str(fused.storage_dtype()).replace("torch.", "")
    snap["build"] = "fp32-mfma" if fused.fp32_mfma() else "fp16-split"
    return snap


def digest():
    snap = snapshot()
    forms = {k: v for k, v in snap.items() if k not in ("products", "storage", "build")}
    return hashlib.sha256(json.dumps(forms, sort_keys=True).encode()).hexdigest()[:16]
```

### include/elo.h

```cpp
#ifndef ELO_H_
#define ELO_H_

#ifdef __cplusplus
extern "C" {
#endif

typedef void *elo_stream_t;

typedef enum elo_status {
    ELO_OK = 0,
    ELO_ERR_ARG = -1,
    ELO_ERR_LIMIT = -2,
    ELO_ERR_LAUNCH = -3
} elo_status;

int elo_abi_version(void);
int elo_dense_f32(void);
const char *elo_last_error(void);
int elo_range_check(int enable);
int elo_range_violations(unsigned long long *count, elo_stream_t stream);

int elo_graph_submit(void *graph_exec, elo_stream_t stream, void *dst, const void *src, unsigned long bytes,
                     elo_stream_t producer, void *order_event, int device);

// ... 169 lines not shown
    int point_stride;
    int H, W;
    float az_res, vert_res, vert_off;
    float crop_xy;
    const float *cloud;
    const float *T_trans;
    const int *aug_frame;
    float *points;
    float *out_xyz;
    unsigned *scratch;
} elo_input_stage_args;
int elo_input_stage(const elo_input_stage_args *a, elo_stream_t stream);

int elo_pose_head_warp(const elo_pose_head_args *a, const elo_warp_project_args *w, elo_stream_t stream);

typedef struct elo_group_concat_bwd_args {
    int batch, npoints, K;
    int H2, W2, C;
    const float *grad_out;
    const int *idx;
    const float *mask;
    float *grad_centre;
    float *grad_src_xyz;
    float *grad_src_feat;
} elo_group_concat_bwd_args;
int elo_group_concat_backward(const elo_group_concat_bwd_args *a, elo_stream_t stream);

typedef struct elo_masked_maxpool_bwd_args {
    int batch, npoints, K, C;
    const float *x;
    const float *mask;
    const float *grad_out;
    float *grad_x;
} elo_masked_maxpool_bwd_args;
int elo_masked_maxpool_backward(const elo_masked_maxpool_bwd_args *a, elo_stream_t stream);

typedef struct elo_cv_encode1_bwd_args {
    int batch, npoints, K;
    int H2, W2, C;
    const float *xyz1;
    const float *xyz2;
    const int *idx;
    const float *mask;
    const float *grad_out;
    float *grad_xyz1;
    float *grad_feat1;
    float *grad_xyz2;
    float *grad_feat2;
} elo_cv_encode1_bwd_args;
int elo_cv_encode1_backward(const elo_cv_encode1_bwd_args *a, elo_stream_t stream);

typedef struct elo_cv_encode2_bwd_args {
    int batch, npoints, K;
    int H, W, C, Cc;
    const float *xyz1;
    const int *idx;
    const float *mask;
    const float *grad_xyz_cat;
    const float *grad_rest;
    float *grad_xyz1;
    float *grad_feat1;
    float *grad_cost;
} elo_cv_encode2_bwd_args;
int elo_cv_encode2_backward(const elo_cv_encode2_bwd_args *a, elo_stream_t stream);

typedef struct elo_softmax_pool_bwd_args {
    int batch, npoints, K, C;
    const float *logits;
    const float *values;
    int values_stride;
    const float *mask;
    const float *grad_out;
    float *grad_logits;
    float *grad_values;
} elo_softmax_pool_bwd_args;
int elo_masked_softmax_pool_backward(const elo_softmax_pool_bwd_args *a, elo_stream_t stream);

typedef struct elo_softmax_valid_bwd_args {
    int batch, npoints, C;
    const float *feature, *weight, *xyz;
    const float *grad_out;
    float *grad_feature;
    float *grad_weight;
    const float *out, *stats;
} elo_softmax_valid_bwd_args;
int elo_softmax_valid_backward(const elo_softmax_valid_bwd_args *a, elo_stream_t stream);

typedef struct elo_warp_project_bwd_args {
    int batch, npoints, C;
    int H, W;
    float az_res, vert_res, vert_off;
    const float *xyz;
    const float *q, *t;
    const unsigned *scratch;
    const float *grad_out_xyz;
    const float *grad_out_feat;
    const float *grad_warped;
    float *grad_xyz;
    float *grad_feat;
    float *grad_q;
    float *grad_t;
} elo_warp_project_bwd_args;
int elo_warp_project_backward(const elo_warp_project_bwd_args *a, elo_stream_t stream);

#define ELO_BN_MAX_PARTS 512
typedef struct elo_bn_stats_args {
    long rows; int C;
    const float *z;
    float *scratch;
    float eps, momentum;
    float *mean, *invstd;
    float *running_mean, *running_var;
    int groups;
} elo_bn_stats_args;
int elo_bn_stats(const elo_bn_stats_args *a, elo_stream_t stream);
long elo_bn_scratch_floats(int C, int groups);

typedef struct elo_bn_apply_args {
    long rows; int C;
    const float *z, *mean, *invstd, *gamma, *beta;
    int relu;
    float *y;
    int groups;
} elo_bn_apply_args;
int elo_bn_apply(const elo_bn_apply_args *a, elo_stream_t stream);

typedef struct elo_bn_backward_args {
    long rows; int C;
    const float *dy, *z, *mean, *invstd, *gamma, *beta;
    int relu;
    float *scratch;
    float *sums;
    float *dz;
    int groups;
} elo_bn_backward_args;
int elo_bn_backward(const elo_bn_backward_args *a, elo_stream_t stream);

typedef struct elo_weight_grad_args {
    long rows; int Cin, Cout;
    const float *x;
    const float *g;
    float *dW;
    float *db;
    float *scratch;
} elo_weight_grad_args;
int elo_weight_grad_slices(long rows, int Cin, int Cout);
int elo_dense_weight_grad(const elo_weight_grad_args *a, elo_stream_t stream);

#define ELO_DENSE_MAX_PARTS 2048
typedef struct elo_dense_rows_args {
    long rows; int Cin, Cout;
    const float *x;
    const float *W;
    int transposed;
    const float *bias;
    float *out;
    float *scratch;
    float eps, momentum;
    float *mean, *invstd;
    float *running_mean, *running_var;
    const float *bn_z, *bn_mean, *bn_invstd, *bn_gamma, *bn_beta, *bn_sums;
    int bn_relu;
    float *bn_dz;
    int groups;
} elo_dense_rows_args;
int elo_dense_rows_supported(long rows, int Cin, int Cout);
long elo_dense_rows_scratch_floats(int Cout, int groups);
int elo_dense_rows(const elo_dense_rows_args *a, elo_stream_t stream);

typedef struct elo_adam_flat_args {
    long n;
    float *param;
    const float *grad;
    float *exp_avg;
    float *exp_avg_sq;
    const float *hyper;
    float beta1, beta2;
    float one_minus_beta1, one_minus_beta2;
} elo_adam_flat_args;
int elo_adam_flat(const elo_adam_flat_args *a, elo_stream_t stream);

typedef struct elo_pose_compose_args {
    int batch;
    const float *q_raw, *t_det, *q_coarse, *t_coarse;
    float *q, *t, *q_norm;
    const float *grad_q, *grad_t, *grad_q_norm;
    float *grad_q_raw, *grad_t_det, *grad_q_coarse, *grad_t_coarse;
} elo_pose_compose_args;
int elo_pose_compose(const elo_pose_compose_args *a, elo_stream_t stream);

typedef struct elo_pose_loss_args {
    int batch;
    const float *q[4], *t[4];
    const float *q_gt, *t_gt;
    const float *w_x, *w_q;
    float *loss;
    const float *grad_out;
    float *grad_q[4], *grad_t[4];
    float *grad_w_x, *grad_w_q;
} elo_pose_loss_args;
int elo_pose_loss(const elo_pose_loss_args *a, elo_stream_t stream);

enum { ELO_PRODUCTS_SPLIT = 0,
       ELO_PRODUCTS_HALF = 1 };

typedef struct elo_dense {
    const float *w_packed;
    const float *bias;
    int K, N;
    int relu;
    const float *w_plain;
    int products;
} elo_dense;

#define ELO_MAX_CHAIN 3

typedef struct elo_group_spec {
    const int *random_hw;
    int kernel_h, kernel_w;
    float distance;
    int stride_h, stride_w;
    int *idx_out;
    float *mask_out;
    const int *decoded_hw;
} elo_group_spec;

typedef struct elo_setconv_args {
    int batch, npoints, K;
    int H, W;
    int H2, W2, C;
    const float *xyz1_grid;
    const int *centre_hw;
    const float *centre_xyz;
    const float *src_xyz;
    const void *src_feat;
    const int *idx;
    const float *mask;
    int n_layers;
    elo_dense layers[ELO_MAX_CHAIN];
    void *out;
    float *new_xyz;
    elo_group_spec group;
    int feat_dtype;
    unsigned long long *range_counter;
} elo_setconv_args;
int elo_setconv_fused(const elo_setconv_args *a, elo_stream_t stream);
int elo_setconv_fused2(const elo_setconv_args *a, const elo_setconv_args *b, elo_stream_t stream);

typedef struct elo_mlp_args {
    long rows;
    int n_sources;
    const void *src[3];
    int src_width[3];
    int n_layers;
    elo_dense layers[ELO_MAX_CHAIN];
    void *out;
    int n_layers2;
    elo_dense layers2[ELO_MAX_CHAIN];
    const void *before;
    int w_before;
    const void *after;
    int w_after;
    void *out2;
    int feat_dtype;
    unsigned *clear_scratch;
    float *clear_xyz;
    void *clear_feat;
    long clear_cells;
    int clear_C;
    int clear_images;
    int batch_hint;
    float *sv_scratch;
    const float *sv_xyz;
    const void *sv_feature;
    int sv_npoints;
    unsigned long long *range_counter;
} elo_mlp_args;
#define ELO_THROUGHPUT_BATCH 4
int elo_mlp_fused(const elo_mlp_args *a, elo_stream_t stream);
int elo_mlp_fused2(const elo_mlp_args *a, const elo_mlp_args *b, elo_stream_t stream);
int elo_mlp_sv_parts(const elo_mlp_args *a, const elo_mlp_args *b);

typedef struct elo_cv1_args {
    int batch, npoints, K;
    int H2, W2, C;
    const float *xyz1;
    const void *feat1;
    const float *xyz2;
    const void *feat2;
    const int *idx;
    const float *mask;
    elo_dense cv0, cv1, cv2, cv_xyz, sum_cv0, sum_cv1;
    void *out;
    elo_group_spec group;
    int feat_dtype;
    unsigned long long *range_counter;
} elo_cv1_args;
int elo_cv_stage1_fused(const elo_cv1_args *a, elo_stream_t stream);
int elo_debug_cv1_rr(int on);
int elo_debug_rr_rows(long setconv_rows, long mlp_rows);
int elo_debug_rr_launches(unsigned long long *counts4, int reset);
int elo_debug_sv_ride_launches(unsigned long long *count, int reset);
int elo_debug_chain_pair_launches(unsigned long long *count, int reset);
int elo_debug_narrow_mfma(int on);
int elo_debug_narrow_launches(unsigned long long *counts2, int reset);
int elo_cv_stage1_setconv_fused(const elo_cv1_args *a, const elo_setconv_args *ja, const elo_setconv_args *jb, elo_stream_t stream);
int elo_cv_stage1_setconv_chain_form(const elo_cv1_args *a, const elo_setconv_args *ja, const elo_setconv_args *jb);
int elo_cv_stage1_setconv_chain(const elo_cv1_args *a, const elo_setconv_args *ja, const elo_setconv_args *jb, elo_stream_t stream);

typedef struct elo_cv2_args {
    int batch, npoints, K;
    int H, W, C;
    const float *xyz1;
    const void *feat1;
    const void *cost;
    const int *idx;
    const float *mask;
    elo_dense xyz_enc, sum_cost0, sum_cost1;
    void *out;
    elo_group_spec group;
    int feat_dtype;
    unsigned long long *range_counter;
} elo_cv2_args;
int elo_cv_stage2_fused(const elo_cv2_args *a, elo_stream_t stream);

#ifdef __cplusplus
}
#endif
#endif
```

Before: 11980.

## Ride set-upconv stage-2 MLPs on the cost-volume stage-2 launch

Adds a combined kernel in which the first blocks run cost-volume stage 2 and the remaining blocks run the two set-upconv stage-2 MLPs. The predictor MLPs are then run as a separate pair. The goal is to cut kernel launches and fill the GPU better at small batch by running independent work in one grid. This reorders the model's upconv/predictor path, enabled by default through the upconv_ride tuning flag. The combined kernel is sized for the larger of the two LDS footprints and register bounds, which may lower occupancy for the cost-volume blocks.

```diff
diff --git a/efficientlo-net_amd/_lib.py b/efficientlo-net_amd/_lib.py
--- a/efficientlo-net_amd/_lib.py
+++ b/efficientlo-net_amd/_lib.py
@@ -210,6 +210,9 @@
     ("elo_cv_stage1_setconv_chain_form", ctypes.c_int, [ctypes.POINTER(Cv1Args), ctypes.POINTER(SetconvArgs), ctypes.POINTER(SetconvArgs)]),
     ("elo_cv_stage1_setconv_chain", ctypes.c_int, [ctypes.POINTER(Cv1Args), ctypes.POINTER(SetconvArgs), ctypes.POINTER(SetconvArgs), _vp]),
     ("elo_cv_stage2_fused", ctypes.c_int, [ctypes.POINTER(Cv2Args), _vp]),
+    ("elo_debug_upconv_ride_launches", ctypes.c_int, [ctypes.POINTER(ctypes.c_ulonglong), ctypes.c_int]),
+    ("elo_cv_stage2_upconv_form", ctypes.c_int, [ctypes.POINTER(Cv2Args), ctypes.POINTER(MlpArgs), ctypes.POINTER(MlpArgs)]),
+    ("elo_cv_stage2_upconv_fused", ctypes.c_int, [ctypes.POINTER(Cv2Args), ctypes.POINTER(MlpArgs), ctypes.POINTER(MlpArgs), _vp]),
     ("elo_cv_stage1_setconv_fused", ctypes.c_int, [ctypes.POINTER(Cv1Args), ctypes.POINTER(SetconvArgs), ctypes.POINTER(SetconvArgs), _vp]),
 ]
 
diff --git a/efficientlo-net_amd/csrc/elo_fused.hip b/efficientlo-net_amd/csrc/elo_fused.hip
--- a/efficientlo-net_amd/csrc/elo_fused.hip
+++ b/efficientlo-net_amd/csrc/elo_fused.hip
@@ -2301,16 +2301,15 @@
 #endif
 
 template <int TILE, int MODE>
-__global__ __launch_bounds__(FUSED_BLOCK, TILE == 32 ? ELO_TILE32_WAVES : ELO_TILE_WAVES) void cv2_kernel(const elo_cv2_args a, const int S)
-{
-    extern __shared__ __align__(16) float lds[];
+__device__ __forceinline__ void cv2_tile(const elo_cv2_args &a, const int S, float *lds, unsigned block, unsigned nblocks)
+{
     float *act = lds;
     const TileMeta meta = tile_meta(lds, TILE, S);
     const int tid = threadIdx.x;
     const int K = a.K, P = TILE / K, C = a.C, f16 = a.feat_dtype == ELO_F16;
     unsigned bad = 0;
     const long total_points = (long)a.batch * a.npoints;
-    const long first_point = (long)xcd_tile(blockIdx.x, gridDim.x) * P;
+    const long first_point = (long)xcd_tile(block, nblocks) * P;
     if (first_point >= total_points) return;
     if (a.group.random_hw) {
         int *lds_off = reinterpret_cast<int *>(meta.cxyz + 128);
@@ -2345,6 +2344,37 @@
     dense_pf<TILE, 64, 0, MODE>(act, S, 64, to_pool(64), a.sum_cost1, p64, nullptr, nullptr, bad);
     pool_masked_softmax(act, S, 64, 0, meta, P, K, first_point, total_points, a.out, f16);
     report_violations<MODE>(bad, a.range_counter);
+}
+
+template <int TILE, int MODE>
+__global__ __launch_bounds__(FUSED_BLOCK, TILE == 32 ? ELO_TILE32_WAVES : ELO_TILE_WAVES) void cv2_kernel(const elo_cv2_args a, const int S)
+{
+    extern __shared__ __align__(16) float lds[];
+    cv2_tile<TILE, MODE>(a, S, lds, blockIdx.x, gridDim.x);
+}
+
+struct MlpSideJobs {
+    elo_mlp_args job[2];
+    int S, blocks_per_job;
+};
+
+template <int TILE_CV, int TILE_MLP, int MODE>
+__global__ __launch_bounds__(FUSED_BLOCK, TILE_CV == 32 || TILE_MLP == 32 ? ELO_TILE32_WAVES : ELO_TILE_WAVES)
+void cv2_upconv_kernel(const elo_cv2_args a, const int S, const unsigned n_cv, const MlpSideJobs side)
+{
+    extern __shared__ __align__(16) float lds[];
+    if (blockIdx.x < n_cv) {
+        cv2_tile<TILE_CV, MODE>(a, S, lds, blockIdx.x, n_cv);
+    } else {
+        const unsigned r = blockIdx.x - n_cv;
+        const unsigned j = r / (unsigned)side.blocks_per_job;
+        const elo_mlp_args &m = side.job[j];
+        const long first = (long)xcd_tile(r - j * (unsigned)side.blocks_per_job, (unsigned)side.blocks_per_job) * TILE_MLP;
+        if (first >= m.rows) return;
+        unsigned bad = 0;
+        mlp_tile<TILE_MLP, MODE>(m, lds, side.S, first, m.rows, false, bad);
+        report_violations<MODE>(bad, m.range_counter);
+    }
 }
 
 inline long small_tile_threshold() { return tuning().small_tile_units; }
@@ -2586,6 +2616,13 @@
 {
     if (count) *count = g_chain_pair_launches.load();
     if (reset) g_chain_pair_launches.store(0);
+    return ELO_OK;
+}
+static std::atomic<unsigned long long> g_upconv_ride_launches;
+extern "C" int elo_debug_upconv_ride_launches(unsigned long long *count, int reset)
+{
+    if (count) *count = g_upconv_ride_launches.load();
+    if (reset) g_upconv_ride_launches.store(0);
     return ELO_OK;
 }
 static std::atomic<unsigned long long> g_sv_ride_launches;
@@ -2756,6 +2793,16 @@
     return cols;
 }
 
+static bool mlp_chain_regime(long rows, bool pair, int batch_hint, int mode)
+{
+#ifdef ELO_DENSE_F32
+    (void)rows; (void)pair; (void)batch_hint; (void)mode;
+    return false;
+#else
+    return (mode == MODE_SPLIT || mode == MODE_HALF) && cv1_rr_on() && rows * (pair ? 2 : 1) >= mlp_rr_rows(batch_hint);
+#endif
+}
+
 struct MlpPlan { int S, mode, C; bool t16, chain; int sv_tiles; };
 
 static int plan_mlp(const elo_mlp_args *a, const elo_mlp_args *b, MlpPlan *p, const char *who)
@@ -2787,16 +2834,15 @@
     p->C = a->n_sources == 2 ? a->src_width[1] : 0;
 #ifndef ELO_DENSE_F32
     {
-        const long min_rows = mlp_rr_rows(a->batch_hint);
         const int C = p->C;
         const bool aligned = ((uintptr_t)a->src[0] | (uintptr_t)a->src[1] | (uintptr_t)a->before | (uintptr_t)a->after | (uintptr_t)a->out |
                               (uintptr_t)a->out2) % 16 == 0 &&
                              (!b || ((uintptr_t)b->src[0] | (uintptr_t)b->src[1] | (uintptr_t)b->before | (uintptr_t)b->after | (uintptr_t)b->out |
                                      (uintptr_t)b->out2) % 16 == 0);
-        p->chain = (p->mode == MODE_SPLIT || p->mode == MODE_HALF) && cv1_rr_on() && a->n_sources == 2 && a->src_width[0] == 64 &&
+        p->chain = a->n_sources == 2 && a->src_width[0] == 64 &&
                    (C == 16 || C == 32 || C == 64) && a->n_layers == 2 && a->layers[0].N == 128 && a->layers[1].N == 64 && a->n_layers2 == 2 &&
                    a->layers2[0].N == 128 && a->layers2[1].N == 64 && a->w_before == C && a->w_after == 64 && aligned &&
-                   a->rows * (b ? 2 : 1) >= min_rows;
+                   mlp_chain_regime(a->rows, b != nullptr, a->batch_hint, p->mode);
     }
 #endif
     p->sv_tiles = 0;
@@ -3082,9 +3128,8 @@
 #endif
 }
 
-extern "C" int elo_cv_stage2_fused(const elo_cv2_args *a, elo_stream_t stream)
-{
-    const char *who = "elo_cv_stage2_fused";
+static int plan_cv2(const elo_cv2_args *a, TilePlan *p, const char *who)
+{
     ELO_REQUIRE(a, who, "null argument block");
     ELO_REQUIRE(a->batch >= 0 && a->npoints > 0 && a->K > 0 && a->H > 0 && a->W > 0 && a->C > 0, who, "bad sizes");
     ELO_REQUIRE(a->npoints == a->H * a->W, who, "npoints must equal H*W (every pixel is a centre)");
@@ -3099,21 +3144,33 @@
     if (int rc = check_dense(a->sum_cost1, 128, 64, who, "sum_cost_volume_1")) return rc;
     const long points = (long)a->batch * a->npoints;
     if (points >= 0x7fffffffL) return fail(ELO_ERR_LIMIT, "%s: batch * npoints beyond 2^31", who);
+    p->units = 0;
     if (points == 0) return ELO_OK;
-    const int S = row_stride(208);
+    p->S = row_stride(208);
     const int P32 = 32 / a->K, P16 = a->K <= 16 ? 16 / a->K : 1;
     const long u32 = (points + P32 - 1) / P32, u16 = (points + P16 - 1) / P16;
-    int mode = 0;
-    if (int rc = products_mode(who, &mode, a->xyz_enc, a->sum_cost0, a->sum_cost1)) return rc;
-    const bool t16 = small_tile(u32, a->K);
+    if (int rc = products_mode(who, &p->mode, a->xyz_enc, a->sum_cost0, a->sum_cost1)) return rc;
+    p->t16 = small_tile(u32, a->K);
+    p->units = p->t16 ? u16 : u32;
     const int KT = a->group.random_hw ? a->group.kernel_h * a->group.kernel_w : 0;
-    const size_t lds = tile_lds_bytes(t16 ? 16 : 32, S, KT, false);
-    if (int rc = check_group(a->group, a->H, a->W, lds, who)) return rc;
+    p->lds = tile_lds_bytes(p->t16 ? 16 : 32, p->S, KT, false);
+    return check_group(a->group, a->H, a->W, p->lds, who);
+}
+
+extern "C" int elo_cv_stage2_fused(const elo_cv2_args *a, elo_stream_t stream)
+{
+    const char *who = "elo_cv_stage2_fused";
+    TilePlan plan;
+    if (int rc = plan_cv2(a, &plan, who)) return rc;
+    if (plan.units == 0) return ELO_OK;
+    const int S = plan.S, mode = plan.mode;
+    const bool t16 = plan.t16;
+    const size_t lds = plan.lds;
     hipStream_t s = (hipStream_t)stream;
 #ifndef ELO_DENSE_F32
     if (!a->group.random_hw && cv_chain(a->C, mode)) {
         const int P = RR_ROWS / a->K;
-        const dim3 rgrid((unsigned)((points + P - 1) / P));
+        const dim3 rgrid((unsigned)(((long)a->batch * a->npoints + P - 1) / P));
         const bool f16 = a->feat_dtype == ELO_F16;
 #define RR(CC)                                                                                                           \
         do {                                                                                                             \
@@ -3130,9 +3187,64 @@
         return check_launch(who);
     }
 #endif
-    const dim3 grid((unsigned)(t16 ? u16 : u32));
+    const dim3 grid((unsigned)plan.units);
 #define CALL(k) hipLaunchKernelGGL(k, grid, dim3(FUSED_BLOCK), lds, s, *a, S)
     ELO_PICK(cv2_kernel, t16, mode, CALL);
 #undef CALL
     return check_launch(who);
 }
+
+static int upconv_ride_plan(const elo_cv2_args *a, const elo_mlp_args *ja, const elo_mlp_args *jb, TilePlan *pc, MlpPlan *pm,
+                            const char *who)
+{
+    if (int rc = plan_cv2(a, pc, who)) return rc;
+    ELO_REQUIRE(ja && jb, who, "two set-upconv jobs");
+    if (int rc = plan_mlp(ja, jb, pm, who)) return rc;
+    if (pc->units == 0 || ja->rows == 0) return fail(ELO_ERR_ARG, "%s: empty cost volume or jobs (call the separate entry points)", who);
+    for (const elo_mlp_args *j : {ja, jb})
+        if (j->n_layers2 != 0 || j->clear_scratch || j->sv_scratch)
+            return fail(ELO_ERR_ARG, "%s: the set-upconv jobs are one-stage MLPs without side jobs", who);
+    if (pm->mode != pc->mode) return fail(ELO_ERR_ARG, "%s: the cost volume and the MLP jobs must share one products mode", who);
+#ifndef ELO_DENSE_F32
+    if (!a->group.random_hw && cv_chain(a->C, pc->mode)) return fail(ELO_ERR_ARG, "%s: the cost volume takes its chain form", who);
+#endif
+    if (mlp_chain_regime(ja->rows, true, ja->batch_hint, pm->mode))
+        return fail(ELO_ERR_ARG, "%s: the set-upconv / predictor pair is in the chain kernel's regime", who);
+    return ELO_OK;
+}
+
+extern "C" int elo_cv_stage2_upconv_form(const elo_cv2_args *a, const elo_mlp_args *ja, const elo_mlp_args *jb)
+{
+    TilePlan pc;
+    MlpPlan pm;
+    return upconv_ride_plan(a, ja, jb, &pc, &pm, "elo_cv_stage2_upconv_form") == ELO_OK ? 1 : 0;
+}
+
+extern "C" int elo_cv_stage2_upconv_fused(const elo_cv2_args *a, const elo_mlp_args *ja, const elo_mlp_args *jb, elo_stream_t stream)
+{
+    const char *who = "elo_cv_stage2_upconv_fused";
+    TilePlan pc;
+    MlpPlan pm;
+    if (int rc = upconv_ride_plan(a, ja, jb, &pc, &pm, who)) return rc;
+    MlpSideJobs side;
+    side.job[0] = *ja;
+    side.job[1] = *jb;
+    side.S = pm.S;
+    const int tm = pm.t16 ? 16 : 32;
+    side.blocks_per_job = (int)((ja->rows + tm - 1) / tm);
+    const unsigned n_cv = (unsigned)pc.units;
+    const dim3 grid(n_cv + 2u * (unsigned)side.blocks_per_job);
+    const size_t lm = tile_lds_bytes(tm, pm.S), lds = pc.lds > lm ? pc.lds : lm;
+    const int S = pc.S;
+    hipStream_t s = (hipStream_t)stream;
+#define CALL_T(M) do {                                                                                                  \
+        if (pc.t16 && pm.t16) hipLaunchKernelGGL((cv2_upconv_kernel<16, 16, M>), grid, dim3(FUSED_BLOCK), lds, s, *a, S, n_cv, side);      \
+        else if (pc.t16) hipLaunchKernelGGL((cv2_upconv_kernel<16, 32, M>), grid, dim3(FUSED_BLOCK), lds, s, *a, S, n_cv, side);           \
+        else if (pm.t16) hipLaunchKernelGGL((cv2_upconv_kernel<32, 16, M>), grid, dim3(FUSED_BLOCK), lds, s, *a, S, n_cv, side);           \
+        else hipLaunchKernelGGL((cv2_upconv_kernel<32, 32, M>), grid, dim3(FUSED_BLOCK), lds, s, *a, S, n_cv, side);                        \
+    } while (0)
+    ELO_PICK_MODE(pc.mode, CALL_T);
+#undef CALL_T
+    ++g_upconv_ride_launches;
+    return check_launch(who);
+}
diff --git a/efficientlo-net_amd/fused.py b/efficientlo-net_amd/fused.py
--- a/efficientlo-net_amd/fused.py
+++ b/efficientlo-net_amd/fused.py
@@ -306,9 +306,11 @@
     return out.reshape(sources[0].shape[:-1] + (layers[-1].N,))
 
 
-def mlp_pair(sources_a, layers_a, sources_b, layers_b):
+def mlp_pair(sources_a, layers_a, sources_b, layers_b, clear=None, sv=None):
     a, out_a, _ka = _mlp_args(sources_a, layers_a)
     b, out_b, _kb = _mlp_args(sources_b, layers_b)
+    if _ride_sv(a, b, sv, out_a.dtype) or sv is None:
+        _ride_clear(a, clear, out_a.dtype)
     L.call2("elo_mlp_fused2", a, b, out_a)
     lead = sources_a[0].shape[:-1]
     return out_a.reshape(lead + (layers_a[-1].N,)), out_b.reshape(lead + (layers_b[-1].N,))
@@ -472,10 +474,10 @@
         _RECORD = keep
 
 
-def cv_stage2(xyz1_proj, feat1_proj, cost_proj, idx, mask, xyz_enc, sum_cost0, sum_cost1, group=None, K=None):
+def cv_stage2(xyz1_proj, feat1_proj, cost_proj, idx, mask, xyz_enc, sum_cost0, sum_cost1, group=None, K=None, side=None):
     L.require_gpu(xyz1_proj, feat1_proj, cost_proj, idx, mask)
     if _RECORD is not None:
-        _record(2, (xyz1_proj, feat1_proj, cost_proj, idx, mask, xyz_enc, sum_cost0, sum_cost1), dict(group=group, K=K))
+        _record(2, (xyz1_proj, feat1_proj, cost_proj, idx, mask, xyz_enc, sum_cost0, sum_cost1), dict(group=group, K=K, side=side))
     xyz1_proj = _f32c(xyz1_proj)
     (feat1_proj, cost_proj), dt, code = _features(feat1_proj, cost_proj)
     B, H, W, C = feat1_proj.shape
@@ -491,5 +493,13 @@
     a = L.Cv2Args(B, N, K, H, W, C, xyz1_proj.data_ptr(), feat1_proj.data_ptr(), cost_proj.data_ptr(), ptr(idx),
                   ptr(mask), xyz_enc.struct(), sum_cost0.struct(), sum_cost1.struct(), out.data_ptr(),
                   group.struct(B, N, K, xyz1_proj.device) if group is not None else _NO_GROUP, code)
+    if side:
+        if B < THROUGHPUT_BATCH:
+            jobs = [_mlp_args(**job) for job in side]
+            if L.lib().elo_cv_stage2_upconv_form(ctypes.byref(a), ctypes.byref(jobs[0][0]), ctypes.byref(jobs[1][0])) == 1:
+                L.call3("elo_cv_stage2_upconv_fused", a, jobs[0][0], jobs[1][0], out)
+                return out, [j[1].reshape(job["sources"][0].shape[:-1] + (j[1].shape[-1],)) for j, job in zip(jobs, side)]
+        L.call("elo_cv_stage2_fused", a, out)
+        return out, None
     L.call("elo_cv_stage2_fused", a, out)
     return out
diff --git a/efficientlo-net_amd/pointnet_util.py b/efficientlo-net_amd/pointnet_util.py
--- a/efficientlo-net_amd/pointnet_util.py
+++ b/efficientlo-net_amd/pointnet_util.py
@@ -104,7 +104,7 @@
 @_storage_boundary("points1_proj", "points2_proj")
 def cost_volume(warped_xyz1_proj, xyz2_proj, points1_proj, points2_proj, kernel_size1, kernel_size2, nsample,
                 nsample_q, distance, mlp1, mlp2, is_training, bn_decay, scope, bn=True, pooling='max', knn=True,
-                corr_func='elementwise_product', side_jobs=None, side_chain=False):
+                corr_func='elementwise_product', side_jobs=None, side_chain=False, upconv=None):
     with tf_util.variable_scope(scope):
         B, H, W, _ = warped_xyz1_proj.shape
         N = H * W
@@ -129,13 +129,17 @@
             pi_feat1_new, side_out = stage1 if side_jobs else (stage1, None)
             pi_feat1_new = pi_feat1_new.reshape(B, H, W, -1)
             order = list(range(64 + C, 128 + C)) + list(range(64)) + list(range(64, 64 + C))
-            cost = fused.cv_stage2(warped_xyz1_proj, points1_proj, pi_feat1_new, None, None,
-                                   P('sum_xyz_encoding', 10, 64), P('sum_cost_volume_0', 128 + C, 128, row_order=order),
-                                   P('sum_cost_volume_1', 128, 64),
-                                   group=fused.Grouping(random_HW_p, kernel_size1, distance), K=nsample)
+            layers2 = (P('sum_xyz_encoding', 10, 64), P('sum_cost_volume_0', 128 + C, 128, row_order=order),
+                       P('sum_cost_volume_1', 128, 64))
+            up_jobs = upconv(side_out) if upconv is not None else None
+            cost = fused.cv_stage2(warped_xyz1_proj, points1_proj, pi_feat1_new, None, None, *layers2,
+                                   group=fused.Grouping(random_HW_p, kernel_size1, distance), K=nsample, side=up_jobs)
+            cost, up_out = cost if up_jobs else (cost, None)
+            if upconv is not None:
+                return cost, side_out, up_out
             return (cost, side_out) if side_jobs else cost
-        if side_jobs:
-            raise NotImplementedError("side_jobs ride on the fused cost-volume launch only")
+        if side_jobs or upconv is not None:
+            raise NotImplementedError("side_jobs / upconv ride on the fused cost-volume launches only")
 
         idx_hw = get_hw_idx(B, H, W, dev)
         qi_idx, _, _, valid_mask = fused_conv_select_k(
@@ -283,24 +287,49 @@
     return jobs
 
 
-def up_conv_predict_finish(up_a, up_b, fp_a, fp_b, up_a_pooled, up_b_pooled, clear=None, sv=None):
+def _up_stage2(up):
+    P = fused.packed_layer
+    with tf_util.variable_scope(up["scope"]):
+        feat1_proj, mlp, mlp2 = up["feat1_proj"], up["mlp"], up["mlp2"]
+        B, H, W, _ = up["xyz1_proj"].shape
+        points1 = feat1_proj.reshape(B, H * W, -1)
+        w2 = [mlp[-1] + points1.shape[-1]] + list(mlp2)
+        return points1, [P('up_2_%d' % i, w2[i], w2[i + 1]) for i in range(len(mlp2))]
+
+
+def _predictor(up, fp, w_after=None):
+    P = fused.packed_layer
+    with tf_util.variable_scope(fp["scope"]):
+        before, after = fp["points_f1"], fp.get("cost_volume")
+        w_before = before.shape[-1] if before is not None else 0
+        w_after = after.shape[-1] if after is not None else (w_after or 0)
+        wp = [w_before + w_after + up["mlp2"][-1]] + list(fp["mlp"])
+        return before, after, [P('conv_predictor%d' % i, wp[i], wp[i + 1], bn=fp.get("bn", True),
+                                 row_order=fused.stage2_row_order(w_before, up["mlp2"][-1], w_after) if i == 0 else None)
+                               for i in range(len(fp["mlp"]))]
+
+
+def up_conv_stage2_jobs(up_a, up_b, fp_a, fp_b, up_a_pooled, up_b_pooled, w_cost):
+    jobs = []
+    for up, fp, pooled in ((up_a, fp_a, up_a_pooled), (up_b, fp_b, up_b_pooled)):
+        points1, layers = _up_stage2(up)
+        _predictor(up, fp, w_after=w_cost)
+        jobs.append(dict(sources=[pooled, points1], layers=layers))
+    return jobs
+
+
+def up_conv_predict_finish(up_a, up_b, fp_a, fp_b, up_a_pooled, up_b_pooled, clear=None, sv=None, up_out=None):
+    if up_out is not None:
+        specs = []
+        for up, fp, out in ((up_a, fp_a, up_out[0]), (up_b, fp_b, up_out[1])):
+            before, after, layers2 = _predictor(up, fp)
+            specs.append(([p for p in (out, before, after) if p is not None], layers2))
+        pred_a, pred_b = fused.mlp_pair(specs[0][0], specs[0][1], specs[1][0], specs[1][1], clear=clear, sv=sv)
+        return up_out[0], pred_a, up_out[1], pred_b
     stage2 = []
     for up, fp, pooled in ((up_a, fp_a, up_a_pooled), (up_b, fp_b, up_b_pooled)):
-        P = fused.packed_layer
-        with tf_util.variable_scope(up["scope"]):
-            feat1_proj, mlp, mlp2 = up["feat1_proj"], up["mlp"], up["mlp2"]
-            B, H, W, _ = up["xyz1_proj"].shape
-            points1 = feat1_proj.reshape(B, H * W, -1)
-            w2 = [mlp[-1] + points1.shape[-1]] + list(mlp2)
-            layers = [P('up_2_%d' % i, w2[i], w2[i + 1]) for i in range(len(mlp2))]
-        with tf_util.variable_scope(fp["scope"]):
-            before, after = fp["points_f1"], fp["cost_volume"]
-            wp = [sum(p.shape[-1] for p in (before, after) if p is not None) + mlp2[-1]] + list(fp["mlp"])
-            w_before = before.shape[-1] if before is not None else 0
-            w_after = after.shape[-1] if after is not None else 0
-            layers2 = [P('conv_predictor%d' % i, wp[i], wp[i + 1], bn=fp.get("bn", True),
-                         row_order=fused.stage2_row_order(w_before, mlp2[-1], w_after) if i == 0 else None)
-                       for i in range(len(fp["mlp"]))]
+        points1, layers = _up_stage2(up)
+        before, after, layers2 = _predictor(up, fp)
         stage2.append(dict(sources=[pooled, points1], layers=layers, before=before, after=after, layers2=layers2))
     (out_a, pred_a), (out_b, pred_b) = fused.mlp2_pair(stage2[0], stage2[1], clear=clear, sv=sv)
     return out_a, pred_a, out_b, pred_b
diff --git a/efficientlo-net_amd/pwclo_model.py b/efficientlo-net_amd/pwclo_model.py
--- a/efficientlo-net_amd/pwclo_model.py
+++ b/efficientlo-net_amd/pwclo_model.py
@@ -8,7 +8,7 @@
 from .model_util import (PreProcess, ProjectPC2SphericalRing, input_stage, preprocess_gt, get_selected_idx, inv_q, mul_point_q, mul_q_point,
                          softmax_valid, warp_and_project)
 from .pointnet_util import (cost_volume, down_conv, down_conv_job, flow_predictor, fused_pairs_available, merge_branches,
-                            up_conv, up_conv_predict_finish, up_conv_stage1_jobs)
+                            up_conv, up_conv_predict_finish, up_conv_stage1_jobs, up_conv_stage2_jobs)
 
 Down_conv_dis = [0.5, 3.0, 6.0, 12.0]
 Up_conv_dis = [3.0, 6.0, 9.0]
@@ -290,13 +290,14 @@
         xyz_warp_f1 = xyz_warp_proj_f1.reshape(batch_size, -1, 3)
         points_warp_f1 = points_warp_proj_f1.reshape(batch_size, out_h_list[g] * out_w_list[g], -1)
 
-        def branch_cost(side_jobs=None, side_chain=False):
+        def branch_cost(side_jobs=None, side_chain=False, upconv=None):
             return cost_volume(xyz_warp_proj_f1, xyz_proj_f2[level], points_warp_proj_f1, pts_proj_f2[level],
                                kernel_size1=[3, 5], kernel_size2=cv_kernel2[level], nsample=4, nsample_q=6,
                                distance=Cost_volume_dis[level], mlp1=[128, 64, 64], mlp2=[128, 64],
                                is_training=is_training, bn_decay=bn_decay, scope='flow_embedding_l%d' % level,
                                bn=True, pooling='max', knn=True, corr_func='concat', side_jobs=side_jobs,
-                               **({"side_chain": True} if side_chain else {}))
+                               **({"side_chain": True} if side_chain else {}),
+                               **({"upconv": upconv} if upconv is not None else {}))
 
         def branch_up(kind, coarse_feat_proj):
             return up_conv(xyz_warp_proj_f1, coarse_xyz_proj, points_warp_proj_f1, coarse_feat_proj,
@@ -312,17 +313,30 @@
             up_w = dict(up, feat2_proj=coarse_w_proj, scope='up_sa_layer_layer_l%dw' % level)
             up_c = dict(up, feat2_proj=coarse_predict_proj, scope='up_sa_layer_layer_l%dcostvolume' % level)
             jobs = up_conv_stage1_jobs(up_w, up_c)
+            fp = dict(points_f1=points_warp_f1, mlp=[128, 64])
+            fp_w, fp_c = dict(fp, scope='l%d_w_predict' % level), dict(fp, scope='l%d_costvolume_predict' % level)
+            sv = sv_ride(xyz_warp_f1)
+            upconv = None
+            if sv is not None and tuning.get("upconv_ride"):
+                upconv = tf_util.in_current_scope(
+                    lambda side: None if side is None else up_conv_stage2_jobs(up_w, up_c, fp_w, fp_c, side[0][0], side[1][0], 64))
+            up_out = None
             if merge_branches(is_training, finest_points, batch_size * out_h_list[g] * out_w_list[g]):
-                cost, ((up_w_pooled, _), (up_c_pooled, _)) = branch_cost(side_jobs=jobs)
+                got = branch_cost(side_jobs=jobs, upconv=upconv)
+                cost, ((up_w_pooled, _), (up_c_pooled, _)) = got[:2]
+                up_out = got[2] if upconv is not None else None
             else:
                 pair = tuning.get("chain_pair") and finest_points <= tuning.get("merge_points")
-                cost, sides = branch_cost(side_jobs=jobs, side_chain=True) if pair else (branch_cost(), None)
+                if pair:
+                    got = branch_cost(side_jobs=jobs, side_chain=True, upconv=upconv)
+                    cost, sides = got[:2]
+                    up_out = got[2] if upconv is not None else None
+                else:
+                    cost, sides = branch_cost(), None
                 (up_w_pooled, _), (up_c_pooled, _) = sides if sides is not None else fused.setconv_pair(jobs[0], jobs[1])
-            fp = dict(points_f1=points_warp_f1, cost_volume=cost, mlp=[128, 64])
-            sv = sv_ride(xyz_warp_f1)
             w_up_sample, weight, cost_up_sample, predict = up_conv_predict_finish(
-                up_w, up_c, dict(fp, scope='l%d_w_predict' % level), dict(fp, scope='l%d_costvolume_predict' % level),
-                up_w_pooled, up_c_pooled, clear=next_buffers if sv is not None else None, sv=sv)
+                up_w, up_c, dict(fp_w, cost_volume=cost), dict(fp_c, cost_volume=cost),
+                up_w_pooled, up_c_pooled, clear=next_buffers if sv is not None else None, sv=sv, up_out=up_out)
         else:
             cost, w_up_sample, cost_up_sample = _parallel([branch_cost, lambda: branch_up('w', coarse_w_proj),
                                                            lambda: branch_up('costvolume', coarse_predict_proj)], is_training)
diff --git a/efficientlo-net_amd/tf_util.py b/efficientlo-net_amd/tf_util.py
--- a/efficientlo-net_amd/tf_util.py
+++ b/efficientlo-net_amd/tf_util.py
@@ -116,6 +116,19 @@
 
 def variable_scope(name):
     return get_store().variable_scope(name)
+
+
+def in_current_scope(fn):
+    store = get_store()
+    names = list(store._scope)
+
+    def call(*args, **kw):
+        saved, store._scope = store._scope, list(names)
+        try:
+            return fn(*args, **kw)
+        finally:
+            store._scope = saved
+    return call
 
 
 def scope_name():
diff --git a/efficientlo-net_amd/tuning.py b/efficientlo-net_amd/tuning.py
--- a/efficientlo-net_amd/tuning.py
+++ b/efficientlo-net_amd/tuning.py
@@ -16,6 +16,7 @@
     "chain_pair": ("ELO_CHAIN_PAIR", lambda v: v != "0", True),
     "native_submit": ("ELO_NATIVE_SUBMIT", lambda v: v != "0", True),
     "sv_ride": ("ELO_SV_RIDE", lambda v: v != "0", True),
+    "upconv_ride": ("ELO_UPCONV_RIDE", lambda v: v != "0", True),
     "train_kernels": ("ELO_TRAIN_KERNELS", lambda v: v != "0", True),
     "train_dense": ("ELO_TRAIN_DENSE", lambda v: v != "0", True),
     "train_dense_rows": ("ELO_TRAIN_DENSE_ROWS", int, 25000),
diff --git a/include/elo.h b/include/elo.h
--- a/include/elo.h
+++ b/include/elo.h
@@ -495,6 +495,7 @@
 int elo_debug_rr_launches(unsigned long long *counts4, int reset);
 int elo_debug_sv_ride_launches(unsigned long long *count, int reset);
 int elo_debug_chain_pair_launches(unsigned long long *count, int reset);
+int elo_debug_upconv_ride_launches(unsigned long long *count, int reset);
 int elo_debug_narrow_mfma(int on);
 int elo_debug_narrow_launches(unsigned long long *counts2, int reset);
 int elo_cv_stage1_setconv_fused(const elo_cv1_args *a, const elo_setconv_args *ja, const elo_setconv_args *jb, elo_stream_t stream);
@@ -516,6 +517,8 @@
     unsigned long long *range_counter;
 } elo_cv2_args;
 int elo_cv_stage2_fused(const elo_cv2_args *a, elo_stream_t stream);
+int elo_cv_stage2_upconv_form(const elo_cv2_args *a, const elo_mlp_args *ja, const elo_mlp_args *jb);
+int elo_cv_stage2_upconv_fused(const elo_cv2_args *a, const elo_mlp_args *ja, const elo_mlp_args *jb, elo_stream_t stream);
 
 #ifdef __cplusplus
 }
```

New measurement: 12720, median of 6. 1.06x the previous value.
